# JunweiLiang/Object_Detection_Tracking

Hardware: AMD Instinct MI355X
Metric: detector FPS @1920x1080 b=8 per MI355X (higher is better)
Workload: dtype f32

## Files before the change

### include/odt.h

```cpp
#ifndef ODT_H_
#define ODT_H_

#include <stddef.h>
#include <stdint.h>

#ifdef __cplusplus
extern "C" {
#endif

typedef struct odt_model* odt_handle;

#define ODT_DTYPE_U8 0
#define ODT_DTYPE_F32 1

#define ODT_GRAPH_SINGLE 0
#define ODT_GRAPH_MULTI 1
#define ODT_GRAPH_EFFNET 2

typedef struct odt_config {
  int32_t graph;
  int32_t batch;
  int32_t height, width;
  int32_t num_class;
  int32_t num_blocks[4];
// ... 56 lines not shown
int odt_set_source_size(odt_handle h, int src_height, int src_width);

int odt_forward_serial(odt_handle h, int64_t* serial);

typedef struct odt_rle_result {
  int32_t n;
  int32_t height, width;
  const char* strings;
  const int64_t* offsets;
  const int32_t* lengths;
  const uint32_t* counts;
  const int64_t* count_offsets;
} odt_rle_result;
int odt_mask_rle(odt_handle h, int64_t serial, int height, int width, double scale, int want_counts, odt_rle_result* out);

#define ODT_WANT_FEATS  1
#define ODT_WANT_POOLED 2
#define ODT_WANT_MASKS  4
#define ODT_WANT_ALL    7
int odt_submit(odt_handle h, const void* frames, int dtype, int* ticket);
int odt_submit_ex(odt_handle h, const void* frames, int dtype, int want, int* ticket);
int odt_collect(odt_handle h, int ticket, odt_outputs* out);
int odt_ingest_buffer(odt_handle h, int dtype, void** buffer, size_t* bytes);

int odt_describe(odt_handle h, char* buf, int cap);

int odt_tap(odt_handle h, const char* name, float* dst, size_t cap_elems,
            int64_t* shape_out, int* rank_out);

int odt_range_health(odt_handle h, int rebase, double* worst_growth, char* tensor, int tensor_cap, double* tensor_amax,
                     long long* tensors_seen);

int odt_profile_enable(odt_handle h, int enable);
int odt_profile_read(odt_handle h, double* conv_ms, double* conv_flops,
                     int* conv_launches, double* total_ms);
int odt_profile_layer(odt_handle h, int index, char* name, int name_cap,
                      double* flops, double* ms, int64_t* mnk, int* count);

int odt_probe_mfma_bf16(int device, double warm_ms, double min_ms, int lds_reads, double* tflops_bf16,
                        double* clock_ghz, double* measured_ms, int* launches);

int odt_nn_cosine(int device, const float* gallery, const int32_t* seg_offsets,
                  int T, const float* dets, int N, int D, double* cost);

typedef struct odt_tracker* odt_tracker_handle;
int odt_tracker_create(double max_cosine_distance, int nn_budget, double max_iou_distance,
                       int max_age, int n_init, int device, odt_tracker_handle* out);
int odt_tracker_destroy(odt_tracker_handle t);
int odt_tracker_predict(odt_tracker_handle t);
int odt_tracker_update(odt_tracker_handle t, const double* tlwh, const double* conf,
                       const float* feats, int N, int D);
int odt_tracker_tracks(odt_tracker_handle t, int cap, int32_t* ids, int32_t* state,
                       int32_t* time_since_update, int32_t* hits, int32_t* age, double* mean,
                       double* covariance, int* n);
int odt_lsap(const double* cost, int nr, int nc, int32_t* rows, int32_t* cols, int* n);
int odt_tracker_nms(const double* boxes_xywh, const double* scores, const int32_t* order, int n, double max_overlap, int32_t* pick,
                    int* npick);

typedef struct odt_tmot* odt_tmot_handle;
int odt_tmot_create(double conf_thres, double track_max_second_lost, double emb_max_dist, double iou_max_dist1,
                    double iou_max_dist2, double emb_smooth_alpha, double frame_gap, double frame_rate,
                    odt_tmot_handle* out);
int odt_tmot_destroy(odt_tmot_handle t);
int odt_tmot_reset(odt_tmot_handle t);
int odt_tmot_update(odt_tmot_handle t, const double* tlwh, const double* conf, const float* feats, int n, int dim,
                    int* id_counter, int* n_out);
int odt_tmot_tracks(odt_tmot_handle t, int which, int cap, int32_t* ids, int32_t* state, int32_t* activated,
                    double* tlwh, double* det_tlwh, double* det_conf, double* score, int32_t* tracklet_len,
                    int32_t* start_frame, int32_t* frame_id, int* n);


int odt_op_conv2d(int device, const float* in, int B, int H, int W, int Cin,
                  const float* wt, const float* bias, int kh, int kw, int Cout,
                  int stride, int dil, int pad_t, int pad_l, int Ho, int Wo,
                  int oy, int ox, const float* res, int res_mode, int relu,
                  float* out);

int odt_op_conv2d_cat(int device, const float* a, int B, int Ho, int Wo, int Ca, const float* b2, int Hb,
                      int Wb, int Cb, int stride_b, const float* wa, const float* wb, const float* bias,
                      int Cout, int relu, float* out);
int odt_op_bottleneck_tail(int device, const float* in, int B, int H, int W, int C, const float* w2,
                           const float* b2, int dil, const float* w3, const float* b3, int C3,
                           const float* res, int relu3, int fuse, float* out);
int odt_op_stem(int device, const float* frame_pad, int B, int Hp, int Wp, const float* w_hwio, const float* bias,
                int fuse, int grid, float* out);
#define ODT_CONV_CHOICE_SHAPE 18
#define ODT_CONV_CHOICE_OUT 11
int odt_op_conv_choice(const int* shape, int conv_arith, int conv_split_family, int* out, char* name, int name_cap);
int odt_op_preprocess(int device, const void* frames, int dtype, int B, int H,
                      int W, int pad_t, int pad_l, int Hp, int Wp, float* out);
int odt_op_maxpool(int device, const float* in, int B, int H, int W, int C,
                   float* out);
int odt_op_topk(int device, const float* scores, int n, int k, int32_t* idx_out);
int odt_op_nms(int device, const float* boxes, const float* scores, int n,
               int max_out, float iou_thresh, int32_t* idx_out, int* n_out);
int odt_op_proposals(int device, int graph, int B, int L, const int* hs,
                     const int* ws, const int* fields, const float* const* rpn,
                     const float* const* anchors, int img_h, int img_w, int K,
                     float nms_thresh, float decode_clip, float* props,
                     int32_t* nprops);
int odt_op_roi_align(int device, int B, int C, const int* hs, const int* ws,
                     const float* const* feats, const float* strides,
                     const float* boxes, const int32_t* box_ind, int R,
                     float* out_nchw, float* pooled);
int odt_op_detections(int device, int graph, int B, int K, int C,
                      const float* cls_logits, const float* box_logits,
                      const float* props, const int32_t* nprops, int img_h,
                      int img_w, const float* reg_weights, float decode_clip,
                      float score_thresh, float nms_thresh, int per_im,
                      float* boxes, float* probs, int32_t* labels,
                      int32_t* valid);

int odt_op_class_nms(int device, int graph, int B, int N, int C, const float* boxes_in,
                     const float* scores_in, const int32_t* ncand, float score_thresh,
                     float nms_thresh, int per_im, float* boxes, float* scores,
                     int32_t* labels, int32_t* valid);


int odt_op_dwconv(int device, const float* in, int B, int H, int W, int ldc, const float* wt, const float* bias, int k,
                  int stride, int pad_t, int pad_l, int Ho, int Wo, int act, int nmaps, const int32_t* map_hw, int se,
                  int mid, const float* w1, const float* b1, const float* w2t, const float* b2, float* out, float* mean,
                  float* gate, int32_t* info);
int odt_op_se_gate(int device, const float* x, int B, int HW, int ldc, int mid, int se, const float* w1, const float* b1,
                   const float* w2t, const float* b2, float* mean, float* gate, float* scaled, int32_t* info);
int odt_op_rse_gate(int device, const float* t2, int B, int HW, int ch, int r, int cout, const float* w1, const float* b1,
                    const float* w2t, const float* b2, float* mean, float* gate);
int odt_op_rse_apply(int device, const float* y, const float* gate, const float* shortcut, int B, int HW, int C, int ldc,
                     int in_place, float* out, float* amax);
int odt_op_se_tail(int device, const float* t2, int B, int H, int W, int ch, const float* w3, const float* b3, const float* w1,
                   const float* b1, const float* w2t, const float* b2, const float* shortcut, float* out, float* gate,
                   float* amax);
int odt_op_bifpn_fuse(int device, int n, const float* const* ins, const int32_t* in_hw, const int32_t* mode,
                      const int32_t* pads, const float* wsm, int act, int B, int h, int w, int ldc, float* out);
int odt_op_mbconv_expand_dw(int device, const float* x, int B, int H, int W, int in_ldc, const float* e_wt,
                            const float* e_bias, int mid, int lmid, const float* dw_wt, const float* dw_bias, int k,
                            int stride, int pad_t, int pad_l, int Ho, int Wo, int se, const float* w1, const float* b1,
                            const float* w2t, const float* b2, float* out, float* mean, float* gate, int32_t* info);
int odt_op_effdet_post(int device, int B, int ncls, const int32_t* npix, int ldc_cls, int ldc_box,
                       const float* const* cls, const float* const* box, const float* anchors, int k, int max_out,
                       float score_thresh, float iou_thresh, float image_scale, int32_t* cand_idx, float* cand_boxes,
                       float* cand_scores, int32_t* cand_cls, int32_t* cand_lvl, float* boxes, float* scores,
                       int32_t* labels, int32_t* levels, int32_t* valid);
int odt_op_preprocess_rgb(int device, const void* frames, int dtype, int B, int Hs, int Ws, int Hr, int Wr, int pad_t,
                          int pad_l, int Hp, int Wp, int resize, float* out);

int odt_op_mask_rle(int device, const float* masks, const float* boxes, int n, int on_device, int height, int width,
                    double scale, int want_counts, odt_rle_result* out);

#ifdef __cplusplus
}
#endif
#endif
```

### object_detection_tracking_amd/_lib.py

```python
from __future__ import annotations

import copy
import ctypes as C
import json
import os

import numpy as np

HERE = os.path.dirname(os.path.abspath(__file__))
LIB_HIP_PATH = os.path.join(HERE, "libodt_hip.so")

c_float_p = C.POINTER(C.c_float)
c_int_p = C.POINTER(C.c_int32)
c_i64_p = C.POINTER(C.c_int64)
c_double_p = C.POINTER(C.c_double)

ODT_DTYPE_U8, ODT_DTYPE_F32 = 0, 1
ODT_ARITH_DEFAULT, ODT_ARITH_F32, ODT_ARITH_BF16X3 = 0, 1, 2
ODT_GRAPH_SINGLE, ODT_GRAPH_MULTI, ODT_GRAPH_EFFNET = 0, 1, 2
RPN_CH = 16


class OdtConfig(C.Structure):
  _fields_ = [
      ("graph", C.c_int32), ("batch", C.c_int32), ("height", C.c_int32),
      ("width", C.c_int32), ("num_class", C.c_int32),
      ("num_blocks", C.c_int32 * 4), ("use_dilations", C.c_int32),
      ("fpn_channels", C.c_int32), ("head_dim", C.c_int32),
      ("rpn_topk", C.c_int32), ("result_per_im", C.c_int32),
      ("anchor_field", C.c_int32), ("rpn_nms_thresh", C.c_float),
      ("rpn_decode_clip", C.c_float), ("head_decode_clip", C.c_float),
      ("bbox_reg_weights", C.c_float * 4), ("result_score_thresh", C.c_float),
      ("head_nms_thresh", C.c_float), ("add_mask", C.c_int32), ("mask_dim", C.c_int32),
      ("eff_backbone", C.c_int32), ("eff_det", C.c_int32), ("eff_topk", C.c_int32),
      ("eff_image_scale", C.c_float), ("conv_arith", C.c_int32), ("conv_split_family", C.c_int32),
      ("keep_taps", C.c_int32),
      ("tail_overlap", C.c_int32),
      ("use_se", C.c_int32),
  ]


class OdtOutputs(C.Structure):
  _fields_ = [("boxes", c_float_p), ("probs", c_float_p), ("labels", c_int_p),
              ("valid", c_int_p), ("feats", c_float_p), ("pooled", c_float_p),
              ("masks", c_float_p)]


class OdtRleResult(C.Structure):
  _fields_ = [("n", C.c_int32), ("height", C.c_int32), ("width", C.c_int32), ("strings", C.c_void_p),
              ("offsets", c_i64_p), ("lengths", c_int_p), ("counts", C.POINTER(C.c_uint32)), ("count_offsets", c_i64_p)]

  def rles(self):
    size = [int(self.height), int(self.width)]
    out = []
    for j in range(int(self.n)):
      s = C.string_at(self.strings + int(self.offsets[j]), int(self.lengths[j])) if self.lengths[j] else b""
      out.append({"size": list(size), "counts": s.decode("ascii")})
    return out

  def count_lists(self):
    if not self.counts:
      return None
    total = int(self.count_offsets[int(self.n)])
    flat = np.ctypeslib.as_array(self.counts, shape=(total,)).copy() if total else np.zeros(0, np.uint32)
    return [flat[int(self.count_offsets[j]):int(self.count_offsets[j + 1])] for j in range(int(self.n))]


def fptr(a):
  return a.ctypes.data_as(c_float_p)


def iptr(a):
  return a.ctypes.data_as(c_int_p)


def f32(a):
  return np.ascontiguousarray(a, dtype=np.float32)


def i32(a):
  return np.ascontiguousarray(a, dtype=np.int32)


class OdtError(RuntimeError):
  pass


class OdtLib(object):

  SYMBOLS = [
      "odt_last_error", "odt_device_count", "odt_create", "odt_destroy",
      "odt_load_tensor", "odt_finalize_weights", "odt_forward",
      "odt_forward_async", "odt_synchronize", "odt_read_outputs", "odt_describe", "odt_range_health", "odt_submit", "odt_submit_ex", "odt_collect",
      "odt_ingest_buffer", "odt_set_source_size", "odt_tap", "odt_profile_enable",
      "odt_profile_read", "odt_profile_layer", "odt_probe_mfma_bf16", "odt_nn_cosine", "odt_op_conv2d", "odt_op_conv2d_cat",
      "odt_op_bottleneck_tail", "odt_op_stem", "odt_op_conv_choice", "odt_op_preprocess",
      "odt_op_maxpool", "odt_op_topk", "odt_op_nms", "odt_op_proposals",
      "odt_op_roi_align", "odt_op_detections", "odt_op_class_nms",
      "odt_op_dwconv", "odt_op_se_gate", "odt_op_rse_gate", "odt_op_rse_apply", "odt_op_se_tail", "odt_op_bifpn_fuse", "odt_op_mbconv_expand_dw", "odt_op_effdet_post",
      "odt_op_preprocess_rgb", "odt_forward_serial", "odt_mask_rle", "odt_op_mask_rle", "odt_tracker_create", "odt_tracker_destroy",
      "odt_tracker_predict", "odt_tracker_update", "odt_tracker_tracks", "odt_lsap", "odt_tracker_nms",
      "odt_tmot_create", "odt_tmot_destroy", "odt_tmot_reset", "odt_tmot_update", "odt_tmot_tracks",
  ]

  def __init__(self, path):
    if not os.path.exists(path):
      raise OdtError("native library not found: %s (build it with "
                     "`python -m object_detection_tracking_amd.build`)" % path)
    self.path = path
    self.dll = C.CDLL(path)
    d = self.dll
    for s in self.SYMBOLS:
      if not hasattr(d, s):
        raise OdtError("%s does not export %s" % (path, s))
    d.odt_last_error.restype = C.c_char_p
    d.odt_create.argtypes = [C.POINTER(OdtConfig), C.c_int, C.POINTER(C.c_void_p)]
    d.odt_destroy.argtypes = [C.c_void_p]
    d.odt_load_tensor.argtypes = [C.c_void_p, C.c_char_p, c_float_p, c_i64_p, C.c_int]
    d.odt_finalize_weights.argtypes = [C.c_void_p]
    d.odt_forward.argtypes = [C.c_void_p, C.c_void_p, C.c_int, C.c_int, C.c_void_p,
                              C.POINTER(OdtOutputs)]
    d.odt_forward_async.argtypes = [C.c_void_p, C.c_void_p, C.c_int, C.c_int, C.c_void_p]
    d.odt_synchronize.argtypes = [C.c_void_p]
    d.odt_read_outputs.argtypes = [C.c_void_p, C.POINTER(OdtOutputs)]
    d.odt_submit.argtypes = [C.c_void_p, C.c_void_p, C.c_int, C.POINTER(C.c_int)]
    d.odt_describe.argtypes = [C.c_void_p, C.c_char_p, C.c_int]
    d.odt_range_health.argtypes = [C.c_void_p, C.c_int, C.POINTER(C.c_double), C.c_char_p, C.c_int, C.POINTER(C.c_double), C.POINTER(C.c_longlong)]
    d.odt_submit_ex.argtypes = [C.c_void_p, C.c_void_p, C.c_int, C.c_int, C.POINTER(C.c_int)]
    d.odt_collect.argtypes = [C.c_void_p, C.c_int, C.POINTER(OdtOutputs)]
    d.odt_set_source_size.argtypes = [C.c_void_p, C.c_int, C.c_int]
    d.odt_ingest_buffer.argtypes = [C.c_void_p, C.c_int, C.POINTER(C.c_void_p),
                                    C.POINTER(C.c_size_t)]
    d.odt_tap.argtypes = [C.c_void_p, C.c_char_p, c_float_p, C.c_size_t, c_i64_p,
                          C.POINTER(C.c_int)]
    d.odt_profile_enable.argtypes = [C.c_void_p, C.c_int]
    d.odt_profile_read.argtypes = [C.c_void_p, c_double_p, c_double_p,
                                   C.POINTER(C.c_int), c_double_p]
    d.odt_profile_layer.argtypes = [C.c_void_p, C.c_int, C.c_char_p, C.c_int, c_double_p,
                                    c_double_p, c_i64_p, C.POINTER(C.c_int)]
    d.odt_probe_mfma_bf16.argtypes = [C.c_int, C.c_double, C.c_double, C.c_int, c_double_p, c_double_p, c_double_p,
                                      C.POINTER(C.c_int)]
    d.odt_nn_cosine.argtypes = [C.c_int, c_float_p, c_int_p, C.c_int, c_float_p, C.c_int,
                                C.c_int, c_double_p]
    d.odt_op_conv2d.argtypes = [C.c_int, c_float_p] + [C.c_int] * 4 + [c_float_p, c_float_p] + \
        [C.c_int] * 11 + [c_float_p, C.c_int, C.c_int, c_float_p]
    d.odt_op_conv2d_cat.argtypes = [C.c_int, c_float_p] + [C.c_int] * 4 + [c_float_p] + [C.c_int] * 4 + \
        [c_float_p, c_float_p, c_float_p, C.c_int, C.c_int, c_float_p]
    d.odt_op_bottleneck_tail.argtypes = [C.c_int, c_float_p] + [C.c_int] * 4 + [c_float_p, c_float_p, C.c_int, c_float_p, c_float_p,
                                         C.c_int, c_float_p, C.c_int, C.c_int, c_float_p]
    d.odt_op_stem.argtypes = [C.c_int, c_float_p] + [C.c_int] * 3 + [c_float_p, c_float_p, C.c_int, C.c_int, c_float_p]
    d.odt_op_conv_choice.argtypes = [c_int_p, C.c_int, C.c_int, c_int_p, C.c_char_p, C.c_int]
    d.odt_op_preprocess.argtypes = [C.c_int, C.c_void_p] + [C.c_int] * 8 + [c_float_p]
    d.odt_op_maxpool.argtypes = [C.c_int, c_float_p] + [C.c_int] * 4 + [c_float_p]
    d.odt_op_topk.argtypes = [C.c_int, c_float_p, C.c_int, C.c_int, c_int_p]
    d.odt_op_nms.argtypes = [C.c_int, c_float_p, c_float_p, C.c_int, C.c_int, C.c_float,
                             c_int_p, C.POINTER(C.c_int)]
    d.odt_op_proposals.argtypes = [C.c_int, C.c_int, C.c_int, C.c_int, c_int_p, c_int_p, c_int_p,
                                   C.POINTER(c_float_p), C.POINTER(c_float_p), C.c_int, C.c_int,
                                   C.c_int, C.c_float, C.c_float, c_float_p, c_int_p]
    d.odt_op_roi_align.argtypes = [C.c_int, C.c_int, C.c_int, c_int_p, c_int_p,
                                   C.POINTER(c_float_p), c_float_p, c_float_p, c_int_p, C.c_int,
                                   c_float_p, c_float_p]
    d.odt_tracker_create.argtypes = [C.c_double, C.c_int, C.c_double, C.c_int, C.c_int, C.c_int,
                                     C.POINTER(C.c_void_p)]
    d.odt_tracker_destroy.argtypes = [C.c_void_p]
    d.odt_tracker_predict.argtypes = [C.c_void_p]
    d.odt_tracker_update.argtypes = [C.c_void_p, c_double_p, c_double_p, c_float_p, C.c_int, C.c_int]
    d.odt_tracker_tracks.argtypes = [C.c_void_p, C.c_int, c_int_p, c_int_p, c_int_p, c_int_p, c_int_p,
                                     c_double_p, c_double_p, C.POINTER(C.c_int)]
    d.odt_lsap.argtypes = [c_double_p, C.c_int, C.c_int, c_int_p, c_int_p, C.POINTER(C.c_int)]
    d.odt_tracker_nms.argtypes = [c_double_p, c_double_p, c_int_p, C.c_int, C.c_double, c_int_p, C.POINTER(C.c_int)]
    d.odt_tmot_create.argtypes = [C.c_double] * 8 + [C.POINTER(C.c_void_p)]
    d.odt_tmot_destroy.argtypes = [C.c_void_p]
    d.odt_tmot_reset.argtypes = [C.c_void_p]
    d.odt_tmot_update.argtypes = [C.c_void_p, c_double_p, c_double_p, c_float_p, C.c_int, C.c_int,
                                  C.POINTER(C.c_int), C.POINTER(C.c_int)]
    d.odt_tmot_tracks.argtypes = [C.c_void_p, C.c_int, C.c_int, c_int_p, c_int_p, c_int_p, c_double_p,
                                  c_double_p, c_double_p, c_double_p, c_int_p, c_int_p, c_int_p,
                                  C.POINTER(C.c_int)]
    d.odt_op_detections.argtypes = [C.c_int] * 5 + [c_float_p, c_float_p, c_float_p, c_int_p,
                                                    C.c_int, C.c_int, c_float_p, C.c_float,
                                                    C.c_float, C.c_float, C.c_int, c_float_p,
                                                    c_float_p, c_int_p, c_int_p]
    d.odt_op_class_nms.argtypes = [C.c_int] * 5 + [c_float_p, c_float_p, c_int_p, C.c_float, C.c_float, C.c_int,
                                                   c_float_p, c_float_p, c_int_p, c_int_p]

    d.odt_op_dwconv.argtypes = [C.c_int, c_float_p] + [C.c_int] * 4 + [c_float_p, c_float_p] + [C.c_int] * 8 + \
        [c_int_p, C.c_int, C.c_int] + [c_float_p] * 7 + [c_int_p]
    d.odt_op_se_gate.argtypes = [C.c_int, c_float_p] + [C.c_int] * 5 + [c_float_p] * 7 + [c_int_p]
    d.odt_op_rse_gate.argtypes = [C.c_int, c_float_p] + [C.c_int] * 5 + [c_float_p] * 6
    d.odt_op_rse_apply.argtypes = [C.c_int, c_float_p, c_float_p, c_float_p] + [C.c_int] * 5 + [c_float_p, c_float_p]
    d.odt_op_se_tail.argtypes = [C.c_int, c_float_p] + [C.c_int] * 4 + [c_float_p] * 10
    d.odt_op_bifpn_fuse.argtypes = [C.c_int, C.c_int, C.POINTER(c_float_p), c_int_p, c_int_p, c_int_p, c_float_p] + \
        [C.c_int] * 5 + [c_float_p]
    d.odt_op_mbconv_expand_dw.argtypes = [C.c_int, c_float_p] + [C.c_int] * 4 + [c_float_p] * 2 + [C.c_int] * 2 + \
        [c_float_p] * 2 + [C.c_int] * 7 + [c_float_p] * 7 + [c_int_p]
    d.odt_op_effdet_post.argtypes = [C.c_int] * 3 + [c_int_p, C.c_int, C.c_int, C.POINTER(c_float_p), C.POINTER(c_float_p),
                                     c_float_p, C.c_int, C.c_int, C.c_float, C.c_float, C.c_float, c_int_p, c_float_p,
                                     c_float_p, c_int_p, c_int_p, c_float_p, c_float_p, c_int_p, c_int_p, c_int_p]
    d.odt_op_preprocess_rgb.argtypes = [C.c_int, C.c_void_p] + [C.c_int] * 11 + [c_float_p]
    d.odt_forward_serial.argtypes = [C.c_void_p, c_i64_p]
    d.odt_mask_rle.argtypes = [C.c_void_p, C.c_int64, C.c_int, C.c_int, C.c_double, C.c_int, C.POINTER(OdtRleResult)]
    d.odt_op_mask_rle.argtypes = [C.c_int, C.c_void_p, C.c_void_p, C.c_int, C.c_int, C.c_int, C.c_int, C.c_double, C.c_int,
                                  C.POINTER(OdtRleResult)]

  def check(self, rc):
    if rc != 0:
      msg = self.dll.odt_last_error()
      raise OdtError(msg.decode("utf-8", "replace") if msg else "odt error %d" % rc)

  def device_count(self):
    n = C.c_int(0)
    self.check(self.dll.odt_device_count(C.byref(n)))
    return n.value


_LIB = None


def get_lib():
  global _LIB
  if _LIB is None:
    lib = OdtLib(LIB_HIP_PATH)
    if lib.device_count() < 1:
      raise OdtError("libodt_hip.so loaded but no HIP device is visible")
    _LIB = lib
  return _LIB


def as_frames(frames):
  fr = np.ascontiguousarray(frames)
  if fr.dtype == np.uint8:
# ... 94 lines not shown
```

### object_detection_tracking_amd/csrc/conv_h2.hip

```cpp
#include "conv_split_epilogue.hpp"

namespace odt {

namespace {

#define ODT_MFMA_F16(a, b, c) __builtin_amdgcn_mfma_f32_32x32x16_f16(a, b, c, 0, 0, 0)

template <int TN, int WM, int WN = 2>
struct H2Cfg {
  static constexpr int BM = 64 * WM, BN = 32 * TN * WN;
  static constexpr int NWV = WN * WM, NTHR = 64 * NWV;
  static constexpr int AKG = BM * 16 + 32, APL = 4 * AKG, ASTG = 2 * APL;
  static constexpr int BKG = BN * 16, BPL = 4 * BKG, STAGE_B = 2 * BPL;
  static constexpr int BOFF = 2 * ASTG;
  static constexpr int RING = BOFF + 2 * STAGE_B;
  static constexpr int CTILE = (BM < 128 ? BM : 128) * (BN + 4) * 4;
  static constexpr int LDS = RING > CTILE ? RING : CTILE;
  static constexpr int NW = STAGE_B / 1024 / NWV;
  static constexpr int RA = BM * 8 / NTHR;
  static_assert(LDS <= 160 * 1024 && STAGE_B % (1024 * NWV) == 0, "LDS ring");
};

template <int TN, int WM, bool TRACE = false, int WN = 2>
__global__ void __launch_bounds__(64 * WN * WM, 2) conv_h2_kernel(const ConvParams* __restrict__ pp) {
// ... 231 lines not shown
      }
      ODT_FENCE();
      ODT_MF(kst, 0, 0, j, bsel); ODT_FENCE();
    }
    { const int t = a_cur; a_cur = a_nxt; a_nxt = t; }
    { const int t = b_cur; b_cur = b_nxt; b_nxt = t; }
  };
  {
    int c = 0;
    for (; c + 2 < nsteps; ++c) step(std::true_type{}, std::true_type{});
    if (c + 1 < nsteps) { step(std::true_type{}, std::false_type{}); ++c; }
    step(std::false_type{}, std::false_type{});
  }
  stamp(2);
  split3_epilogue<WM, WN, TN, G::LDS, TRACE, G::NTHR>(p, acc, lds, m0, n0, M, HoWo, ks, splitk, tid, wm, wn, fr, fg, h2_inv);
  stamp(5);
}

#undef ODT_MF
#undef ODT_FENCE

__global__ void __launch_bounds__(256) h2_rowscale_kernel(const float* __restrict__ wt, int Cout, int K, float* __restrict__ chinv) {
  __shared__ float red[4];
  const int n = (int)blockIdx.x;
  float m = 0.f;
  if (n < Cout)
    for (int k = (int)threadIdx.x; k < K; k += 256) m = fmaxf(m, fabsf(wt[(size_t)n * K + k]));
#pragma unroll
  for (int d = 32; d >= 1; d >>= 1) m = fmaxf(m, __shfl_xor(m, d));
  if ((threadIdx.x & 63) == 0) red[threadIdx.x >> 6] = m;
  __syncthreads();
  if (threadIdx.x == 0) {
    m = fmaxf(fmaxf(red[0], red[1]), fmaxf(red[2], red[3]));
    chinv[n] = pow2f(-h2_scale_exp(__float_as_uint(m)));
  }
}

__global__ void split_weights_h2_kernel(const float* __restrict__ wt, int Cout, int K, int SBN, int ntaps, int Cin,
                                        unsigned short* __restrict__ img, const float* __restrict__ chinv) {
  const int nst = K >> 5, nst1 = ntaps * (Cin >> 5);
  const long idx = (long)blockIdx.x * blockDim.x + threadIdx.x;
  const long total = (long)cout_padded(Cout) * nst * 4;
  if (idx >= total) return;
  const int n = (int)(idx / (nst * 4)), rem = (int)(idx - (long)n * (nst * 4)), st = rem >> 2, kg = rem & 3;
  int k0;
  if (st < nst1) { const int cs = st / ntaps, tap = st - cs * ntaps; k0 = tap * Cin + cs * 32; }
  else k0 = ntaps * Cin + (st - nst1) * 32;
  k0 += kg * 8;
  const int tn = n / SBN, nn = n - tn * SBN;
  const float s = 1.0f / chinv[n];
  for (int e = 0; e < 8; e += 2) {
    unsigned piece[2];
    const float w0 = n < Cout ? wt[(size_t)n * K + k0 + e] : 0.f, w1 = n < Cout ? wt[(size_t)n * K + k0 + e + 1] : 0.f;
    split2h(w0, w1, s, piece[0], piece[1]);
    for (int q = 0; q < 2; ++q) {
      const size_t at = ((((size_t)(tn * nst + st) * 2 + q) * 4 + kg) * SBN + nn) * 8 + e;
      img[at] = (unsigned short)(piece[q] & 0xffffu);
      img[at + 1] = (unsigned short)(piece[q] >> 16);
    }
  }
}

__global__ void split_weights_h2f_kernel(const float* __restrict__ wt, int Cout, int K, unsigned short* __restrict__ img,
                                         const float* __restrict__ chinv) {
  const int KH = K >> 1, NS = KH >> 4;
  const long idx = (long)blockIdx.x * blockDim.x + threadIdx.x;
  const long total = (long)Cout * 2 * NS * 2;
  if (idx >= total) return;
  const int fg = (int)(idx & 1), s = (int)((idx >> 1) % NS), wn = (int)((idx / (2 * NS)) & 1), n = (int)(idx / (4 * NS));
  const int c = n >> 5, fr = n & 31;
  const float sc = 1.0f / chinv[n];
  for (int e = 0; e < 8; e += 2) {
    const int k0 = wn * KH + (s >> 1) * 32 + (s & 1) * 16 + (e & 3) + 8 * (e >> 2) + 4 * fg;
    unsigned piece[2];
    split2h(wt[(size_t)n * K + k0], wt[(size_t)n * K + k0 + 1], sc, piece[0], piece[1]);
    for (int q = 0; q < 2; ++q) {
      const size_t at = ((((((size_t)c * 2 + q) * 2 + wn) * NS + s) * 2 + fg) * 32 + fr) * 8 + e;
      img[at] = (unsigned short)(piece[q] & 0xffffu);
      img[at + 1] = (unsigned short)(piece[q] >> 16);
    }
  }
}

__global__ void __launch_bounds__(256) tensor_amax_kernel(const float* __restrict__ x, size_t n, unsigned* __restrict__ slot) {
  float m = 0.f;
  for (size_t i = (size_t)blockIdx.x * 256 + threadIdx.x; i < n; i += (size_t)gridDim.x * 256) m = fmaxf(m, fabsf(x[i]));
  publish_amax(slot, m, (int)threadIdx.x);
}

}

size_t conv_h2_weight_bytes(int Cout, int K) { return (size_t)cout_padded(Cout) * K * 4 + (size_t)cout_padded(Cout) * 4; }

const float* conv_h2_chinv(const void* img, int Cout, int K) {
  return reinterpret_cast<const float*>(reinterpret_cast<const char*>(img) + (size_t)cout_padded(Cout) * K * 4);
}

int conv_make_h2_weights(const ConvParams& p, void* img_dev, hipStream_t stream) {
  const int K = p.kh * p.kw * p.Cin + (p.in2 != nullptr ? p.Cin2 : 0);
  const int bn = conv_variant_row(p.variant).bn;
  ODT_CHECK((bn == 256 || bn == 128 || bn == 64) && p.Cin % 32 == 0 && (p.in2 == nullptr || p.Cin2 % 32 == 0) && cout_padded(p.Cout) % bn == 0,
            "conv_make_h2_weights: 256- / 128- / 64-wide n-tiles and 32-channel slices required");
  float* chinv = const_cast<float*>(conv_h2_chinv(img_dev, p.Cout, K));
  hipLaunchKernelGGL(h2_rowscale_kernel, dim3((unsigned)cout_padded(p.Cout)), dim3(256), 0, stream, p.wt, p.Cout, K, chinv);
  const long total = (long)cout_padded(p.Cout) * (K >> 5) * 4;
  hipLaunchKernelGGL(split_weights_h2_kernel, dim3((unsigned)((total + 255) / 256)), dim3(256), 0, stream, p.wt, p.Cout, K,
                     bn, p.kh * p.kw, p.Cin, (unsigned short*)img_dev, chinv);
  ODT_HIP(hipGetLastError());
  return 0;
}

size_t conv_h2f_weight_bytes(int Cout, int K) { return (size_t)Cout * K * 4 + (size_t)Cout * 4; }
const float* conv_h2f_chinv(const void* img, int Cout, int K) {
  return reinterpret_cast<const float*>(reinterpret_cast<const char*>(img) + (size_t)Cout * K * 4);
}
int conv_make_h2f_weights(const float* wt, int Cout, int K, void* img_dev, hipStream_t stream) {
  ODT_CHECK((K == 256 || K == 128 || K == 64) && Cout % 32 == 0 && Cout > 0, "conv_make_h2f_weights: K = 64 / 128 / 256 and Cout % 32 == 0 required");
  float* chinv = const_cast<float*>(conv_h2f_chinv(img_dev, Cout, K));
  hipLaunchKernelGGL(h2_rowscale_kernel, dim3((unsigned)Cout), dim3(256), 0, stream, wt, Cout, K, chinv);
  const long total = (long)Cout * (K >> 3);
  hipLaunchKernelGGL(split_weights_h2f_kernel, dim3((unsigned)((total + 255) / 256)), dim3(256), 0, stream, wt, Cout, K,
                     (unsigned short*)img_dev, chinv);
  ODT_HIP(hipGetLastError());
  return 0;
}

bool conv_h2f_fusable(const ConvParams& a, const ConvParams& b) {
  const ConvKernelRow& fa = conv_variant_row(conv_variant_fused_tail(a.variant));
  const bool a_ok = a.wt_split != nullptr && fa.launch != nullptr && fa.bn == a.Cout && a.splitk <= 1 && a.head_wt == nullptr &&
                    a.res_mode == 0 && a.in2 == nullptr && a.relu <= 1 && a.nlvl <= 1 && a.out_oy == 0 && a.out_ox == 0 &&
                    a.out_H == a.Ho && a.out_W == a.Wo && a.f_wt == nullptr;
  const bool b_ok = b.in == a.out && b.kh == 1 && b.kw == 1 && b.stride == 1 && b.pad_t == 0 && b.pad_l == 0 && b.Cin == a.Cout &&
                    b.in_ldc == a.out_ldc && b.in2 == nullptr && b.B == a.B && b.H == a.Ho && b.W == a.Wo && b.Ho == a.Ho &&
                    b.Wo == a.Wo && b.in_Ha == a.out_H && b.in_Wa == a.out_W && b.Cout % 32 == 0 && b.out_oy == 0 && b.out_ox == 0 &&
                    b.out_H == b.Ho && b.out_W == b.Wo && b.out_ldc % 4 == 0 && b.out_ldc >= b.Cout &&
                    (b.res_mode == 0 || (b.res_mode == 1 && b.res_H == b.Ho && b.res_W == b.Wo && b.res_ldc % 4 == 0)) &&
                    b.relu <= 1 && b.nlvl <= 1 && b.head_wt == nullptr && b.splitk <= 1 && b.wt_split != nullptr && conv_variant_row(b.variant).family == CF_H2 &&
                    b.f_wt == nullptr && (double)b.B * b.Ho * b.Wo * b.out_ldc * 4.0 < 2147483648.0;
  return a_ok && b_ok;
}

int launch_tensor_amax(const float* x, size_t n, unsigned* slot, hipStream_t stream) {
  const unsigned blocks = (unsigned)std::min<size_t>((n + 255) / 256, 2048);
  hipLaunchKernelGGL(tensor_amax_kernel, dim3(blocks ? blocks : 1), dim3(256), 0, stream, x, n, slot);
  ODT_HIP(hipGetLastError());
  return 0;
}

void conv_rows_h2(ConvKernelRow* t) {
  ODT_CONV_ROW(t, H2_64x64, CF_H2, 64, 64, 128, 0, (conv_h2_kernel<1, 1, false>));
  ODT_CONV_ROW(t, H2_64x128, CF_H2, 64, 128, 128, 0, (conv_h2_kernel<2, 1, false>));
  ODT_CONV_ROW(t, H2_512x64, CF_H2, 512, 64, 512, 0, (conv_h2_kernel<2, 8, false, 1>));
  ODT_CONV_ROW(t, H2_128x64, CF_H2, 128, 64, 256, 0, (conv_h2_kernel<1, 2, false>));
  ODT_CONV_ROW_T(t, H2_256x256, CF_H2, 256, 256, 512, 0, (conv_h2_kernel<4, 4, false>), (conv_h2_kernel<4, 4, true>));
  ODT_CONV_ROW(t, H2_256x128, CF_H2, 256, 128, 512, 0, (conv_h2_kernel<2, 4, false>));
  ODT_CONV_ROW_T(t, H2_128x128, CF_H2, 128, 128, 256, 0, (conv_h2_kernel<2, 2, false>), (conv_h2_kernel<2, 2, true>));
}

}
```

### object_detection_tracking_amd/csrc/conv_h2k.hip

```cpp
#include "conv_split_epilogue.hpp"

namespace odt {

namespace {

#define ODT_MFMA_F16(a, b, c) __builtin_amdgcn_mfma_f32_32x32x16_f16(a, b, c, 0, 0, 0)
#define ODT_MF(kst, qa, qb, j, bsel) { if constexpr (FUSE) {                                                   \
                                          acc[0][j] = ODT_MFMA_F16(fb[bsel][qb], fa[kst][qa][0], acc[0][j]);   \
                                          acc[1][j] = ODT_MFMA_F16(fb[bsel][qb], fa[kst][qa][1], acc[1][j]);   \
                                        } else {                                                                \
                                          acc[0][j] = ODT_MFMA_F16(fa[kst][qa][0], fb[bsel][qb], acc[0][j]);   \
                                          acc[1][j] = ODT_MFMA_F16(fa[kst][qa][1], fb[bsel][qb], acc[1][j]); } }
#define ODT_FENCE() __builtin_amdgcn_sched_barrier(0)

template <int TN, bool FUSE = false, int WN = 2>
struct H2kCfg {
  static constexpr int WM = 8 / WN;
  static constexpr int BM = 64 * WM, BN = 32 * TN * WN;
  static constexpr int PR = BM + 16;
  static constexpr int ZR = PR - 1;
  static constexpr int AKG = PR * 16 + 32, APL = 4 * AKG, ABUF = 2 * APL;
  static constexpr int BKG = BN * 16, BPL = 4 * BKG, STAGE_B = 2 * BPL;
  static constexpr int BOFF = 2 * ABUF;
  static constexpr int RING = BOFF + 2 * STAGE_B;
  static constexpr int CTILE = 128 * (BN + 4) * 4;
  static constexpr int F_WCH = 2 * 2 * (2 * TN) * 1024, F_CS = 36, F_COFF = 2 * F_WCH, F_CEND = F_COFF + 2 * 256 * F_CS * 4;
  static constexpr int LDS0 = RING > CTILE ? RING : CTILE;
  static constexpr int F_KOFF = F_CEND > LDS0 ? F_CEND : LDS0;
  static constexpr int F_K3OFF = F_KOFF + 2048;
  static constexpr int LDS = FUSE ? F_K3OFF + 8192 : LDS0;
  static constexpr int NW = STAGE_B / 1024 / 8;
  static constexpr int RA = (PR + 63) / 64;
  static_assert(LDS <= 160 * 1024 && STAGE_B % 8192 == 0 && (!FUSE || WN == 2), "LDS");
};

template <int TN, bool TRACE>
__device__ __forceinline__ void h2f_tail(const ConvParams& p, f32x16 (&acc)[2][TN], unsigned char* lds, int m0, int M,
                                         int wave, int wm, int wn, float h2_inv) {
  using G = H2kCfg<TN, true>;
  constexpr int NS = 2 * TN, WCH = G::F_WCH, CS = G::F_CS, COFF = G::F_COFF, CBUF = 256 * CS * 4;
  ODT_FENCE();
  const int lane = ODT_LANE_ID();
  const int tid = wave * 64 + lane, fr = lane & 31, fg = lane >> 5;
  const int nch = p.f_cout >> 5;

  const float* kc = reinterpret_cast<const float*>(lds + G::F_KOFF);
  const float act2_lo = p.relu == 1 ? 0.f : -__builtin_huge_valf();
  float mx[2] = {0.f, 0.f};
#pragma unroll
  for (int j = 0; j < TN; ++j)
#pragma unroll
    for (int g = 0; g < 4; ++g) {
      const int col = wn * 32 * TN + j * 32 + 8 * g + 4 * fg;
      const f32x4 sc = *reinterpret_cast<const f32x4*>(kc + col), bs = *reinterpret_cast<const f32x4*>(kc + 256 + col);
#pragma unroll
      for (int i = 0; i < 2; ++i)
#pragma unroll
        for (int e = 0; e < 4; ++e) {
          float v = acc[i][j][4 * g + e] * sc[e];
          v += bs[e];
          mx[i] = fmaxf(mx[i], fabsf(fmaxf(v, act2_lo)));
        }
      if (g & 1) ODT_FENCE();
    }
  ODT_PIN2(mx[0], mx[1]);
  asm volatile("" ::: "memory");
  constexpr int XS = 8 * 2 * NS * 1024;
  float* xs = reinterpret_cast<float*>(lds + XS);
#pragma unroll
  for (int i = 0; i < 2; ++i) {
    mx[i] = fmaxf(mx[i], __shfl_xor(mx[i], 32));
    xs[wave * 128 + i * 64 + lane] = mx[i];
  }
  ODT_BARRIER_LDS();
  float ys[2], yinv[2];
#pragma unroll
  for (int i = 0; i < 2; ++i) {
    const float m = fmaxf(mx[i], xs[(wave ^ 1) * 128 + i * 64 + lane]);
    const int be = (int)((__float_as_uint(m) >> 23) & 0xffu);
    int e = 14 - (be - 127);
    e = e > 100 ? 100 : (e < -100 ? -100 : e);
    e = (be == 0) | (be == 255) ? 0 : e;
    ys[i] = pow2f(e); yinv[i] = pow2f(-e);
  }
  ODT_PIN2(ys[0], ys[1]);
  u32x4 yq[2][2][NS];
#pragma unroll
  for (int j = 0; j < TN; ++j)
#pragma unroll
    for (int h = 0; h < 2; ++h) {
      const int col = wn * 32 * TN + j * 32 + 16 * h + 4 * fg;
      const f32x4 sc0 = *reinterpret_cast<const f32x4*>(kc + col), bs0 = *reinterpret_cast<const f32x4*>(kc + 256 + col);
      const f32x4 sc1 = *reinterpret_cast<const f32x4*>(kc + col + 8), bs1 = *reinterpret_cast<const f32x4*>(kc + 256 + col + 8);
#pragma unroll
      for (int i = 0; i < 2; ++i) {
        float v[8];
#pragma unroll
        for (int e = 0; e < 4; ++e) {
          float t0 = acc[i][j][8 * h + e] * sc0[e], t1 = acc[i][j][8 * h + 4 + e] * sc1[e];
          t0 += bs0[e]; t1 += bs1[e];
          v[e] = fmaxf(t0, act2_lo); v[4 + e] = fmaxf(t1, act2_lo);
        }
        u32x4 hq, lq;
#pragma unroll
        for (int t = 0; t < 4; ++t) {
          unsigned a, b;
          split2h(v[2 * t], v[2 * t + 1], ys[i], a, b);
          hq[t] = a; lq[t] = b;
        }
        ODT_PIN2(hq, lq);
        yq[i][0][2 * j + h] = hq; yq[i][1][2 * j + h] = lq;
      }
      ODT_FENCE();
    }
  ODT_STAMP(3);

  constexpr int XW = 2 * NS * 1024;
  static_assert(XS == 8 * XW && XS + 8 * 512 <= G::F_KOFF, "exchange area");
  u32x4 yo[2][NS], yr[2][NS];
  const float yinv_k = wn == 0 ? yinv[0] : yinv[1];
  {
    unsigned char* xw = lds + wave * XW + lane * 16;
    const unsigned char* xr = lds + (wave ^ 1) * XW + lane * 16;
    auto give = [&](auto IC) {
      constexpr int ig = decltype(IC)::value;
#pragma unroll
      for (int q = 0; q < 2; ++q)
#pragma unroll
        for (int t = 0; t < NS; ++t) {
          *reinterpret_cast<u32x4*>(xw + (q * NS + t) * 1024) = yq[ig][q][t];
          yo[q][t] = yq[1 - ig][q][t];
        }
    };
    if (wn == 0) give(std::integral_constant<int, 1>{}); else give(std::integral_constant<int, 0>{});
    ODT_BARRIER_LDS();
#pragma unroll
    for (int q = 0; q < 2; ++q)
#pragma unroll
      for (int t = 0; t < NS; ++t) yr[q][t] = *reinterpret_cast<const u32x4*>(xr + (q * NS + t) * 1024);
    ODT_BARRIER_LDS();
  }
  const __amdgpu_buffer_rsrc_t rs_w = __builtin_amdgcn_make_buffer_rsrc((void*)p.f_wt, 0, (int)((unsigned)nch * (unsigned)WCH), 0x00020000);
  const int rot = (p.debug & 0x100) == 0 ? (m0 / G::BM) % nch : 0;
  auto ce = [&](int c) { return c < nch ? (c + rot >= nch ? c + rot - nch : c + rot) : c; };
  auto dma_w = [&](int cs, int buf) {
    const int c = ce(cs);
#pragma unroll
    for (int i = 0; i < WCH / 8192; ++i)
      __builtin_amdgcn_raw_ptr_buffer_load_lds(rs_w, ODT_LDS_PTR(lds + buf * WCH + (i * 8 + wave) * 1024), 16,
                                               c < nch ? lane * 16 + (i * 8 + wave) * 1024 : (int)kOOB, c < nch ? c * WCH : 0, 0, 0);
  };
  dma_w(0, 0);
  dma_w(1, 1);

  const unsigned mrows = (unsigned)M;
  const __amdgpu_buffer_rsrc_t rs_res = __builtin_amdgcn_make_buffer_rsrc(
      (void*)(p.f_res != nullptr ? p.f_res : p.f_bias), 0, (int)(p.f_res != nullptr ? mrows * (unsigned)p.f_res_ldc * 4u : 0u), 0x00020000);
  const __amdgpu_buffer_rsrc_t rs_out = __builtin_amdgcn_make_buffer_rsrc((void*)p.f_out, 0, (int)(mrows * (unsigned)p.f_out_ldc * 4u), 0x00020000);
  const int c4 = tid & 7, row0 = tid >> 3;
  const unsigned m_first = (unsigned)(m0 + row0);
  const unsigned roff0 = (m_first * (unsigned)p.f_res_ldc + c4 * 4u) * 4u, rstep = 64u * (unsigned)p.f_res_ldc * 4u;
  const unsigned ooff0 = (m_first * (unsigned)p.f_out_ldc + c4 * 4u) * 4u, ostep = 64u * (unsigned)p.f_out_ldc * 4u;
  const bool has_res = p.f_res != nullptr;
  const float act_lo = p.f_relu == 1 ? 0.f : -__builtin_huge_valf();
  const float* k3 = reinterpret_cast<const float*>(lds + G::F_K3OFF);
  auto fetch_res = [&](int cs, int s2) -> f32x4 {
    const int c = ce(cs);
    const unsigned off = has_res && c < nch && m_first + 64u * s2 < mrows ? roff0 + s2 * rstep : kOOB;
    return (f32x4)__builtin_amdgcn_raw_buffer_load_b128(rs_res, (int)off, c * 128, 2);
  };
  f32x4 ra[4], rb[4];
#pragma unroll
  for (int s2 = 0; s2 < 4; ++s2) ra[s2] = fetch_res(0, s2);
#pragma unroll
  for (int s2 = 0; s2 < 4; ++s2) rb[s2] = fetch_res(1, s2);
  const unsigned char* wrd = lds + lane * 16;
  float* Cst = reinterpret_cast<float*>(lds + COFF);
  const int cw_at = (wm * 64 + wn * 32 + fr) * CS + 4 * fg;
  const int cr_at = row0 * CS + c4 * 4;
  float vmax = 0.f;
  auto row_item = [&](int cs, int s2, f32x4& rr) {
    const int c = ce(cs);
    const float* Cb = Cst + (cs & 1) * (CBUF / 4);
    f32x4 v = *reinterpret_cast<const f32x4*>(Cb + cr_at + 64 * s2 * CS);
    const f32x4 sc3 = *reinterpret_cast<const f32x4*>(k3 + c * 32 + c4 * 4), b3 = *reinterpret_cast<const f32x4*>(k3 + 1024 + c * 32 + c4 * 4);
    v = v * sc3;
    v += b3;
    v += rr;
#pragma unroll
    for (int e = 0; e < 4; ++e) v[e] = fmaxf(v[e], act_lo);
    const float vm = fmaxf(fmaxf(fabsf(v[0]), fabsf(v[1])), fmaxf(fabsf(v[2]), fabsf(v[3])));
    const bool ok = m_first + 64u * s2 < mrows;
    vmax = fmaxf(vmax, ok ? vm : 0.f);
    __builtin_amdgcn_raw_buffer_store_b128((u32x4)v, rs_out, (int)(ok ? ooff0 + s2 * ostep : kOOB), c * 128, 0);
    rr = fetch_res(cs + 2, s2);
  };
  ODT_WAIT_VM_LGKM0(8);
  __builtin_amdgcn_s_barrier();
  auto chunk = [&](int c, f32x4 (&rprev)[4], auto HP) {
    constexpr bool has_prev = decltype(HP)::value;
    const int buf = c & 1;
    const unsigned char* wo = wrd + buf * WCH + wn * NS * 1024;
    const unsigned char* wr = wrd + buf * WCH + (1 - wn) * NS * 1024;
    f32x16 co;
#pragma unroll
    for (int r = 0; r < 16; ++r) co[r] = 0.f;
    f16x8 wf[2][2];
    wf[0][0] = *reinterpret_cast<const f16x8*>(wo);
    wf[0][1] = *reinterpret_cast<const f16x8*>(wo + 2 * NS * 1024);
#pragma unroll
    for (int u = 0; u < 2 * NS; ++u) {
      if (u + 1 < 2 * NS) {
        const unsigned char* w = ((u + 1) & 1 ? wr : wo) + ((u + 1) >> 1) * 1024;
        wf[(u + 1) & 1][0] = *reinterpret_cast<const f16x8*>(w);
        wf[(u + 1) & 1][1] = *reinterpret_cast<const f16x8*>(w + 2 * NS * 1024);
      }
      f16x8 yhh, yll;
      if (u & 1) { __builtin_memcpy(&yhh, &yr[0][u >> 1], 16); __builtin_memcpy(&yll, &yr[1][u >> 1], 16); }
      else { __builtin_memcpy(&yhh, &yo[0][u >> 1], 16); __builtin_memcpy(&yll, &yo[1][u >> 1], 16); }
      ODT_FENCE();
      co = ODT_MFMA_F16(wf[u & 1][1], yhh, co);
      co = ODT_MFMA_F16(wf[u & 1][0], yll, co);
      co = ODT_MFMA_F16(wf[u & 1][0], yhh, co);
      ODT_FENCE();
      if constexpr (has_prev) {
        if constexpr (NS >= 4) { if ((u & 1) && u < 8) row_item(c - 1, u >> 1, rprev[u >> 1]); }
        else row_item(c - 1, u, rprev[u]);
      }
    }
    float* Cb = Cst + buf * (CBUF / 4) + cw_at;
#pragma unroll
    for (int g = 0; g < 4; ++g) {
      f32x4 a = {co[4 * g], co[4 * g + 1], co[4 * g + 2], co[4 * g + 3]};
      a = a * yinv_k;
      *reinterpret_cast<f32x4*>(Cb + 8 * g) = a;
    }
    if constexpr (has_prev) ODT_WAIT_VM_LGKM0(8); else ODT_WAIT_VM_LGKM0(0);
    __builtin_amdgcn_s_barrier();
    ODT_FENCE();
    dma_w(c + 2, buf);
    ODT_FENCE();
  };
  chunk(0, ra, std::false_type{});
  int c = 1;
#pragma unroll 1
  for (; c + 1 < nch; c += 2) {
    chunk(c, ra, std::true_type{});
    chunk(c + 1, rb, std::true_type{});
  }
  if (c < nch) {
    chunk(c, ra, std::true_type{});
#pragma unroll
    for (int s2 = 0; s2 < 4; ++s2) row_item(c, s2, rb[s2]);
  } else {
#pragma unroll
    for (int s2 = 0; s2 < 4; ++s2) row_item(c - 1, s2, ra[s2]);
  }
  publish_amax_wg<512>(p.f_out_amax, vmax, tid, lds);
}

template <int TN, bool TRACE = false, bool FUSE = false, int WN = 2>
__global__ void __launch_bounds__(512, 2) conv_h2k_kernel(const ConvParams* __restrict__ pp) {
  using G = H2kCfg<TN, FUSE, WN>;
  constexpr int WM = G::WM, KW = 3;
  constexpr int BM = G::BM, BN = G::BN, AKG = G::AKG, APL = G::APL, ABUF = G::ABUF, BKG = G::BKG, BPL = G::BPL;
  constexpr int STAGE_B = G::STAGE_B, BOFF = G::BOFF, NW = G::NW, ZR = G::ZR, RA = G::RA;
  const ConvParams p = *pp;
  __shared__ __attribute__((aligned(16))) unsigned char lds[G::LDS];

  const int tid = threadIdx.x, lane = tid & 63;
  const int wave = __builtin_amdgcn_readfirstlane(tid >> 6);
  const int wm = wave / WN, wn = wave % WN;
  auto stamp = [&](int i) {
    if constexpr (TRACE) {
      if (tid == 0) p.trace[(size_t)blockIdx.x * 16 + i] = wall_clock64();
    }
  };
  stamp(0);
  if constexpr (TRACE) {
    if (tid == 0) {
      p.trace[(size_t)blockIdx.x * 16 + 8] = __builtin_amdgcn_s_getreg((31 << 11) | 4);
      p.trace[(size_t)blockIdx.x * 16 + 9] = __builtin_amdgcn_s_getreg((31 << 11) | 20);
    }
  }
  const int ntn = cout_padded(p.Cout) / BN;
  int wg = (int)blockIdx.x;
  {
    const int nwg = (int)gridDim.x, xcd = wg & 7, q = nwg >> 3, r = nwg & 7;
    wg = (xcd < r ? xcd * (q + 1) : r * (q + 1) + (xcd - r) * q) + (wg >> 3);
  }
  const int splitk = p.splitk > 1 ? p.splitk : 1;
  const int ks = wg % splitk;
  wg /= splitk;
  const int mt = wg / ntn, nt = wg - mt * ntn;
  const int m0 = mt * BM, n0 = nt * BN;
  const int HoWo = p.Ho * p.Wo;
  const int M = p.B * HoWo;
  const int cpt = p.Cin >> 5;
  const int nsteps = p.kh * KW * cpt, ngroups_all = p.kh * cpt;
  const int g_begin = (int)(((long)ngroups_all * ks) / splitk);
  const int ngroups = (int)(((long)ngroups_all * (ks + 1)) / splitk) - g_begin;
  const int halo = (KW - 1) * p.dil;
  const int sexp = h2_in_scale_exp(p);
  const float a_scale = pow2f(sexp), h2_inv = pow2f(-sexp);

  const __amdgpu_buffer_rsrc_t rs_in = __builtin_amdgcn_make_buffer_rsrc(
      (void*)p.in, 0, (int)((unsigned)p.B * p.in_Ha * p.in_Wa * p.in_ldc * 4u), 0x00020000);
  const __amdgpu_buffer_rsrc_t rs_wt = __builtin_amdgcn_make_buffer_rsrc(
      (void*)p.wt_split, 0, (int)((unsigned)ntn * nsteps * (unsigned)STAGE_B), 0x00020000);

  unsigned l_b = ((unsigned)nt * (unsigned)nsteps + (unsigned)(g_begin * KW)) * (unsigned)STAGE_B;
  auto dma_b = [&](int boff) {
#pragma unroll
    for (int i = 0; i < NW; ++i)
      __builtin_amdgcn_raw_ptr_buffer_load_lds(rs_wt, ODT_LDS_PTR(lds + boff + (i * 8 + wave) * 1024), 16,
                                               lane * 16 + (i * 8 + wave) * 1024, (int)l_b, 0, 0);
    l_b += (unsigned)STAGE_B;
  };
  dma_b(BOFF);

  const int pix_bytes = p.in_ldc * 4;
  const int n_first = sfast_div(m0, p.div_howo_mul, p.div_howo_sh), r_img = m0 - n_first * HoWo;
  const int len0 = HoWo - r_img < BM ? HoWo - r_img : BM;
  const int pix0 = (n_first * p.in_Ha - p.pad_t) * p.in_Wa + r_img - p.pad_l;
  const int pix1 = ((n_first + 1) * p.in_Ha - p.pad_t) * p.in_Wa - p.pad_l;
  const int a_c = tid & 7, a_r = tid >> 3;
  int a_base[RA];
#pragma unroll
  for (int j = 0; j < RA; ++j) {
    const int pr = a_r + 64 * j;
    const int pix = pr < len0 + halo ? pix0 + pr : pix1 + (pr - len0 - halo);
    a_base[j] = pr < BM + 2 * halo ? pix * pix_bytes + a_c * 16 : (int)kOOB;
  }
  int l_cs = g_begin / p.kh, l_kh = g_begin - (g_begin / p.kh) * p.kh;
  f32x4 ga[RA];
  auto load_group = [&]() {
    const int khoff = l_kh * p.dil * p.in_Wa * pix_bytes;
#pragma unroll
    for (int j = 0; j < RA; ++j) {
      const unsigned v = (unsigned)a_base[j] == kOOB ? kOOB : (unsigned)(a_base[j] + khoff);
      ga[j] = (f32x4)__builtin_amdgcn_raw_buffer_load_b128(rs_in, (int)v, l_cs * 128, 0);
    }
    if (++l_kh == p.kh) { l_kh = 0; ++l_cs; }
  };
  auto store_slot = [&](int abuf, int j) {
    const int pr = a_r + 64 * j;
    if (pr < BM + 2 * halo) {
      unsigned h0, l0, h1, l1;
      split2h(ga[j][0], ga[j][1], a_scale, h0, l0);
      split2h(ga[j][2], ga[j][3], a_scale, h1, l1);
      unsigned char* d = lds + abuf + (a_c >> 1) * AKG + pr * 16 + (a_c & 1) * 8;
// ... 80 lines not shown
    for (int t = 0; t < 2; ++t) fa[kst][q][t] = *reinterpret_cast<const f16x8*>(lds + q * APL + kst * 2 * AKG + fa_addr[t]);
  };
  auto rdA_n = [&](int q) {
#pragma unroll
    for (int t = 0; t < 2; ++t) fa[0][q][t] = *reinterpret_cast<const f16x8*>(lds + q * APL + fa_addr_n[t]);
  };
  auto rdB = [&](int bbuf, int kst, int j, int dst) {
#pragma unroll
    for (int q = 0; q < 2; ++q) fb[dst][q] = *reinterpret_cast<const f16x8*>(lds + bbuf + q * BPL + kst * 2 * BKG + b_rd + j * 512);
  };
  int a_cur = 0, a_nxt = ABUF;
  int b_cur = BOFF, b_nxt = BOFF + STAGE_B;
  tap_addr(a_cur, c_kh, 0);
  rdA(0, 1); rdA(0, 0);
  rdB(b_cur, 0, 0, 0);

  auto step = [&](auto KWIC, auto NEXT, auto PRE, auto GNC) {
    constexpr int KWI = decltype(KWIC)::value;
    constexpr bool next = decltype(NEXT)::value, pre = decltype(PRE)::value, gn = decltype(GNC)::value;
    constexpr int NG = 2 * TN;
    ODT_FENCE();
#pragma unroll
    for (int g = 0; g < NG; ++g) {
      const int kst = g / TN, j = g % TN, bsel = g & 1;
      const bool last = g == NG - 1;
      if (last) {
        if constexpr (KWI == 0 && gn) ODT_WAIT_VM_LGKM0(RA); else ODT_WAIT_VM_LGKM0(0);
        __builtin_amdgcn_s_barrier();
        ODT_FENCE();
        if constexpr (pre) dma_b(b_cur);
        if constexpr (next) {
          if constexpr (KWI + 1 < KW) tap_addr_n(a_cur, c_kh, KWI + 1);
          else tap_addr_n(a_nxt, c_kh + 1 == p.kh ? 0 : c_kh + 1, 0);
          rdB(b_nxt, 0, 0, bsel ^ 1);
        }
      } else {
        rdB(b_cur, (g + 1) / TN, (g + 1) % TN, bsel ^ 1);
        if (TN == 1) { rdA(1, 1); rdA(1, 0); }
      }
      ODT_FENCE();
      ODT_MF(kst, 1, 0, j, bsel); ODT_FENCE();
      if (last) {
        if constexpr (next) rdA_n(1);
      } else {
        if constexpr (gn && KWI == 2) {
          if (TN > 1) {
            constexpr int SPG = (RA + NG - 2) / (NG - 1);
#pragma unroll
            for (int q = 0; q < SPG; ++q)
              if (g * SPG + q < RA) store_slot(a_nxt, g * SPG + q);
          } else { store_slot(a_nxt, 0); store_slot(a_nxt, 1); store_slot(a_nxt, 2); }
        }
        if constexpr (gn && KWI == 0) { if (g == (TN == 1 ? 0 : 1)) load_group(); }
      }
      ODT_FENCE();
      ODT_MF(kst, 0, 1, j, bsel); ODT_FENCE();
      if (last) {
        if constexpr (next) rdA_n(0);
      } else {
        if (TN > 1 && g == TN - 2) rdA(1, 1);
        if (TN > 1 && g == TN - 1) rdA(1, 0);
        if constexpr (gn && KWI == 2) { if (TN == 1) { store_slot(a_nxt, 3); store_slot(a_nxt, 4); } }
      }
      ODT_FENCE();
      ODT_MF(kst, 0, 0, j, bsel); ODT_FENCE();
    }
    fa_addr[0] = fa_addr_n[0]; fa_addr[1] = fa_addr_n[1];
    { const int t = b_cur; b_cur = b_nxt; b_nxt = t; }
    if constexpr (KWI == KW - 1) {
      const int u = a_cur; a_cur = a_nxt; a_nxt = u;
      if (++c_kh == p.kh) c_kh = 0;
    }
  };
  {
    using T = std::true_type; using F = std::false_type;
    using K0 = std::integral_constant<int, 0>; using K1 = std::integral_constant<int, 1>; using K2 = std::integral_constant<int, 2>;
    for (int g = 0; g + 1 < ngroups; ++g) { step(K0{}, T{}, T{}, T{}); step(K1{}, T{}, T{}, T{}); step(K2{}, T{}, T{}, T{}); }
    step(K0{}, T{}, T{}, F{});
    step(K1{}, T{}, F{}, F{});
    step(K2{}, F{}, F{}, F{});
  }
#undef ODT_MF
  stamp(2);
  if constexpr (FUSE) h2f_tail<TN, TRACE>(p, acc, lds, m0, M, wave, wm, wn, h2_inv);
  else split3_epilogue<WM, WN, TN, G::LDS, TRACE>(p, acc, lds, m0, n0, M, HoWo, ks, splitk, tid, wm, wn, fr, fg, h2_inv);
  stamp(5);
}
#undef ODT_FENCE

}

void conv_rows_h2k(ConvKernelRow* t) {
  ODT_CONV_ROW(t, H2KF_256x64, CF_H2, 256, 64, 512, CVF_KWR | CVF_FTAIL, (conv_h2k_kernel<1, false, true>));
  ODT_CONV_ROW(t, H2KF_256x128, CF_H2, 256, 128, 512, CVF_KWR | CVF_FTAIL, (conv_h2k_kernel<2, false, true>));
  ODT_CONV_ROW_T(t, H2KF_256x256, CF_H2, 256, 256, 512, CVF_KWR | CVF_FTAIL, (conv_h2k_kernel<4, false, true>), (conv_h2k_kernel<4, true, true>));
  ODT_CONV_ROW_T(t, H2K_256x256, CF_H2, 256, 256, 512, CVF_KWR, (conv_h2k_kernel<4, false>), (conv_h2k_kernel<4, true>));
  ODT_CONV_ROW(t, H2K_256x128, CF_H2, 256, 128, 512, CVF_KWR, (conv_h2k_kernel<2, false>));
  ODT_CONV_ROW(t, H2K_512x64, CF_H2, 512, 64, 512, CVF_KWR, (conv_h2k_kernel<2, false, false, 1>));
  ODT_CONV_ROW(t, H2K_256x64, CF_H2, 256, 64, 512, CVF_KWR, (conv_h2k_kernel<1, false>));
}

}
```

### object_detection_tracking_amd/csrc/conv_igemm.hip

```cpp
#include <cstdlib>
#include <type_traits>

#include "odt_common.hpp"

namespace odt {

namespace {

constexpr int LS = 36;

typedef unsigned int u32x4 __attribute__((vector_size(16)));

__device__ __forceinline__ int fast_div(int n, unsigned mul, unsigned sh) {
  return mul ? (int)(__umulhi((unsigned)n, mul) >> sh) : n;
}
constexpr unsigned kOOB = 0x80000000u;

template <int WM, int WN, int TM, int TN, int ST, bool FINE>
__global__ void __launch_bounds__(256, ST == 1 ? 3 : 2) conv_igemm_kernel(const ConvParams* __restrict__ pp) {
  const ConvParams p = *pp;
  constexpr int BM = WM * TM * 32, BN = WN * TN * 32;
  constexpr int RA = BM / 32, RB = BN / 32;
  static_assert(WM * WN == 4, "4 waves");
  __shared__ __attribute__((aligned(16))) float lds[ST][(BM + BN) * LS];
// ... 428 lines not shown
        if (pass == 0) stamp(4);
      }
    };
    if (p.relu == 1) run(std::integral_constant<int, 1>{});
    else if (p.relu == 2) run(std::integral_constant<int, 2>{});
    else if (p.relu == 3) run(std::integral_constant<int, 3>{});
    else run(std::integral_constant<int, 0>{});
  } else {
    for (int pass = 0; pass < PASSES; ++pass) {
      stage_pass(pass);
      for (int s2 = 0; s2 < NCH; ++s2) {
        const int rl = row0 + s2 * (256 / C4);
        const int m = m0 + pass * RP + rl;
        int nv = p.Cout - col;
        nv = nv > 4 ? 4 : nv;
        if (m >= M || nv <= 0) continue;
        size_t opix, rpix = 0;
        if (dense_io) {
          opix = (size_t)m;
          rpix = (size_t)m;
        } else {
          const int n = fast_div(m, p.div_howo_mul, p.div_howo_sh), rr = m - n * HoWo;
          const int ho = fast_div(rr, p.div_wo_mul, p.div_wo_sh), wo = rr - ho * p.Wo;
          opix = ((size_t)n * p.out_H + ho + p.out_oy) * p.out_W + wo + p.out_ox;
          if (p.res_mode != 0)
            rpix = p.res_mode == 1 ? ((size_t)n * p.res_H + ho) * p.res_W + wo
                                   : ((size_t)n * p.res_H + (ho >> 1)) * p.res_W + (wo >> 1);
        }
        f32x4 v = *reinterpret_cast<const f32x4*>(&Ct[rl * CS + c4 * 4]);
        v += bias4;
        if (p.res_mode != 0) {
          const float* rp = p.res + rpix * p.res_ldc + col;
          for (int e = 0; e < nv; ++e) v[e] += rp[e];
        }
#pragma unroll
        for (int e = 0; e < 4; ++e) {
          if (p.relu == 1) v[e] = fmaxf(v[e], 0.f);
          else if (p.relu == 2) v[e] = v[e] * (1.0f / (1.0f + expf(-v[e])));
          else if (p.relu == 3) v[e] = 1.0f / (1.0f + expf(-v[e]));
        }
        float* op = p.out + opix * p.out_ldc + col;
        for (int e = 0; e < nv; ++e) op[e] = v[e];
      }
    }
  }
  stamp(5);
}

}

void conv_rows_f32(ConvKernelRow* t) {
  ODT_CONV_ROW(t, F32_128x64_S1_FINE, CF_F32, 128, 64, 256, CVF_FINE, (conv_igemm_kernel<4, 1, 1, 2, 1, true>));
  ODT_CONV_ROW(t, F32_128x64_S1, CF_F32, 128, 64, 256, 0, (conv_igemm_kernel<4, 1, 1, 2, 1, false>));
  ODT_CONV_ROW(t, F32_64x64_S1_FINE, CF_F32, 64, 64, 256, CVF_FINE, (conv_igemm_kernel<2, 2, 1, 1, 1, true>));
  ODT_CONV_ROW(t, F32_64x64_S1, CF_F32, 64, 64, 256, 0, (conv_igemm_kernel<2, 2, 1, 1, 1, false>));
  ODT_CONV_ROW(t, F32_128x128_S1_FINE, CF_F32, 128, 128, 256, CVF_FINE, (conv_igemm_kernel<2, 2, 2, 2, 1, true>));
  ODT_CONV_ROW(t, F32_128x128_S1, CF_F32, 128, 128, 256, 0, (conv_igemm_kernel<2, 2, 2, 2, 1, false>));
  ODT_CONV_ROW(t, F32_128x64_S2_FINE, CF_F32, 128, 64, 256, CVF_ST2 | CVF_FINE, (conv_igemm_kernel<4, 1, 1, 2, 2, true>));
  ODT_CONV_ROW(t, F32_128x64_S2, CF_F32, 128, 64, 256, CVF_ST2, (conv_igemm_kernel<4, 1, 1, 2, 2, false>));
  ODT_CONV_ROW(t, F32_64x64_S2_FINE, CF_F32, 64, 64, 256, CVF_ST2 | CVF_FINE, (conv_igemm_kernel<2, 2, 1, 1, 2, true>));
  ODT_CONV_ROW(t, F32_64x64_S2, CF_F32, 64, 64, 256, CVF_ST2, (conv_igemm_kernel<2, 2, 1, 1, 2, false>));
  ODT_CONV_ROW(t, F32_128x128_S2_FINE, CF_F32, 128, 128, 256, CVF_ST2 | CVF_FINE, (conv_igemm_kernel<2, 2, 2, 2, 2, true>));
  ODT_CONV_ROW(t, F32_128x128_S2, CF_F32, 128, 128, 256, CVF_ST2, (conv_igemm_kernel<2, 2, 2, 2, 2, false>));
}

static void make_div(unsigned d, unsigned* mul, unsigned* sh) {
  if (d <= 1) { *mul = 0; *sh = 0; return; }
  unsigned l = 0;
  while ((1ull << l) < d) ++l;
  const unsigned pbits = 31 + l;
  *mul = (unsigned)(((1ull << pbits) + d - 1) / d);
  *sh = pbits - 32;
}

void conv_prepare(ConvParams& p) {
  make_div((unsigned)(p.Ho * p.Wo), &p.div_howo_mul, &p.div_howo_sh);
  make_div((unsigned)p.Wo, &p.div_wo_mul, &p.div_wo_sh);
}

double conv_flops(const ConvParams& p) {
  return 2.0 * (double)p.B * p.Ho * p.Wo * (double)p.Cout *
             (double)(p.kh * p.kw * p.Cin + (p.in2 != nullptr ? p.Cin2 : 0)) +
         (p.head_wt != nullptr ? 2.0 * (double)p.B * p.Ho * p.Wo * (double)p.Cout * 15.0 : 0.0) +
         (p.f_wt != nullptr ? 2.0 * (double)p.B * p.Ho * p.Wo * (double)p.Cout * (double)p.f_cout : 0.0);
}

int conv_check(const ConvParams& p) {
  ODT_CHECK(p.Cin % 32 == 0, "conv: Cin must be a multiple of 32");
  ODT_CHECK(p.in_ldc % 4 == 0, "conv: input pixel stride must be a multiple of 4 floats");
  ODT_CHECK(p.B > 0 && p.Ho > 0 && p.Wo > 0 && p.Cout > 0, "conv: empty problem");
  ODT_CHECK(p.in2 == nullptr || (p.kh == 1 && p.kw == 1 && p.Cin2 % 32 == 0 && p.in2_ldc % 4 == 0 &&
                                 (double)p.B * p.in2_Ha * p.in2_Wa * p.in2_ldc * 4.0 < 2147483648.0),
            "conv: a second A source needs a 1x1 conv, Cin2 % 32 == 0 and a tensor below 2 GiB");
  ODT_CHECK((long)p.Ho * p.stride + (long)p.kh * p.dil < 32000 && (long)p.Wo * p.stride + (long)p.kw * p.dil < 32000 &&
            p.pad_t < 32000 && p.pad_l < 32000, "conv: spatial extent must fit 16-bit tap coordinates");
  ODT_CHECK((double)p.B * p.in_Ha * p.in_Wa * p.in_ldc * 4.0 < 2147483648.0 &&
            (double)p.Cout * (p.kh * p.kw * p.Cin + p.Cin2) * 4.0 < 2147483648.0,
            "conv: operand tensors must be smaller than 2 GiB (32-bit buffer offsets)");
  ODT_CHECK((double)p.B * p.out_H * p.out_W * p.out_ldc * 4.0 < 2147483648.0 &&
            (p.res_mode == 0 || (double)p.B * p.res_H * p.res_W * p.res_ldc * 4.0 < 2147483648.0),
            "conv: output / residual tensors must be smaller than 2 GiB (32-bit buffer offsets)");
  return conv_check_variant(p);
}

}
```

### object_detection_tracking_amd/csrc/conv_split.hip

```cpp
#include <array>

#include "conv_split_common.hpp"

namespace odt {

namespace {

__global__ void split_weights_kernel(const float* __restrict__ wt, int Cout, int K, int SBN, int bk, unsigned short* __restrict__ img,
                                     const float* __restrict__ kscale) {
  const int nsl = K / bk, kgs = bk >> 3;
  const long idx = (long)blockIdx.x * blockDim.x + threadIdx.x;
  const long total = (long)cout_padded(Cout) * (K >> 3);
  if (idx >= total) return;
  const int n = (int)(idx / (K >> 3)), k8 = (int)(idx - (long)n * (K >> 3));
  const int tn = n / SBN, nn = n - tn * SBN, sl = k8 / kgs, kg = k8 - sl * kgs;
  for (int e = 0; e < 8; e += 2) {
    unsigned piece[3];
    float w0 = n < Cout ? wt[(size_t)n * K + k8 * 8 + e] : 0.f, w1 = n < Cout ? wt[(size_t)n * K + k8 * 8 + e + 1] : 0.f;
    if (kscale != nullptr) { w0 = w0 * kscale[k8 * 8 + e]; w1 = w1 * kscale[k8 * 8 + e + 1]; }
    split2(w0, w1, piece[0], piece[1], piece[2]);
    for (int q = 0; q < 3; ++q) {
      const size_t at = ((((size_t)(tn * nsl + sl) * 3 + q) * kgs + kg) * SBN + nn) * 8 + e;
      img[at] = (unsigned short)(piece[q] & 0xffffu);
      img[at + 1] = (unsigned short)(piece[q] >> 16);
// ... 243 lines not shown
      conv_tiles(p, 128, 64) < q.min_tiles) return false;
  return TILE(CF_H2, s.np == 64 && q.h2_n64_bm512 == 2 ? 512 : 128, 64, 0, 1);
}
bool rule_split1(const Sel& s, Tile& t) { return TILE(CF_SPLIT1, conv_split_bm(s.p.Cout), s.bn0, 0, 1); }
#undef TILE

const Rule kRules[] = {rule_exact_f32_outside_policy, rule_exact_f32_too_few_tiles, rule_h2_n64_forced,     rule_h2_256_rows,
                       rule_h2k_few_rows,             rule_h2_dense_few_rows,       rule_h2_64_rows,        rule_h2_128_rows,
                       rule_split3,                   rule_h2_n64_small_tiles,      rule_split1};

int select_exact_f32(const ConvParams& p, const Knobs& k) {
  const long M = (long)p.B * p.Ho * p.Wo;
  const long tiles128 = ((M + 127) / 128) * ((p.Cout + 127) / 128);
  int tile = (int)k.get_long(K_CONV_TILE, 0);
  const bool smallk = !k.off(K_CONV_SMALLK);
  const int Kfull = conv_k(p);
  if (tile == 0) tile = p.Cout <= 64 ? 1 : ((tiles128 < 384 || (smallk && Kfull <= 384)) ? 2 : 3);
  int stages = (tile == 3 && p.kh * p.kw == 1 && p.Cin >= 1024) ? 2 : 1;
  if (k.get(K_CONV_STAGES).i == 1 || k.get(K_CONV_STAGES).i == 2) stages = (int)k.get(K_CONV_STAGES).i;
  const int BMt = tile == 2 ? 64 : 128, BNt = tile == 3 ? 128 : 64;
  const long tiles = ((M + BMt - 1) / BMt) * ((p.Cout + BNt - 1) / BNt);
  const long slots = 256L * (stages == 2 ? 2 : (tile == 3 ? 3 : 4));
  bool fine = stages == 2 || (tile != 2 && (tiles <= slots || tile == 1 || (Kfull >= 1024 && tiles >= 2 * slots)));
  if (tile == 2) fine = tiles >= 384 && tiles <= slots;
  if (k.get(K_CONV_FINE).c0 == '0' || k.get(K_CONV_FINE).c0 == '1') fine = k.get(K_CONV_FINE).c0 == '1';
  return conv_variant_find(CF_F32, BMt, BNt, (stages == 2 ? CVF_ST2 : 0u) | (fine ? CVF_FINE : 0u));
}

}

ConvChoice conv_select(const ConvParams& p, const ConvPolicy& q, const Knobs& k) {
  Sel s{p, q, (long)p.B * p.Ho * p.Wo, conv_k(p), cout_padded(p.Cout), conv_split_bn(p.Cout), false, 0, 0, 1, false, false};
  split3_fit(s);
  s.kwr3 = s.fit && q.kw_reuse && s.b3 == 256 && s.k3 == 1 && (s.n3 >= 128 || q.kwr_n64) && conv_kwr_pays(p);
  s.h2 = s.fit && q.family == 2 && (s.n3 >= 128 || q.h2_n64) && conv_h2_sources_ok(p) && p.lvl_scale == nullptr && p.head_wt == nullptr;
  Tile t{CF_F32, 0, 0, 0, 0};
  for (const Rule rule : kRules)
    if (rule(s, t)) break;
  if (t.family == CF_F32) return ConvChoice{select_exact_f32(p, k), 0, 0};
  if (t.family == CF_H2 && t.bm == 64 && t.splitk == 1 && conv_h2d_fits(p) && !k.off(K_CONV_H2_BK64)) t.flags |= CVF_DSTAGE;
  const long capv = k.get_long(K_SPLIT_REDUCE_BLOCKS, 512L);
  return ConvChoice{conv_variant_find(t.family, t.bm, t.bn, t.flags), t.splitk, capv > 0 ? (int)capv : 512};
}

int conv_finish(ConvParams& p, const Knobs& k) {
  conv_prepare(p);
  if (k.get(K_CONV_DEBUG).i != 0) p.debug = (int)k.get(K_CONV_DEBUG).i;
  if (p.wt_split == nullptr) conv_use_variant(p, select_exact_f32(p, k), 0);
  return conv_check(p);
}

int conv_check_variant(const ConvParams& p) {
  const ConvKernelRow& r = conv_variant_row(p.variant);
  const bool split3 = p.wt_split != nullptr && r.family == CF_SPLIT3;
  ODT_CHECK(p.nlvl <= 1 || (split3 && p.splitk <= 1 && p.nlvl <= 5 && p.head_wt == nullptr),
            "conv: per-row-range epilogue constants need a conv_split3 kernel without split-K");
  if (p.wt_split == nullptr) {
    ODT_CHECK(p.variant == CV_NONE || r.family == CF_F32, "conv: a split-kernel row without a weight image");
    return 0;
  }
  ODT_CHECK(r.launch != nullptr && r.family != CF_F32, "conv: the record's variant names no split-kernel row of the table");
  ODT_CHECK(cout_padded(p.Cout) % r.bn == 0, "conv: the row's n-tile does not divide the padded channel count");
  const long M = (long)p.B * p.Ho * p.Wo;
  const int sk = p.splitk > 1 ? p.splitk : 1;
  const bool kwr = (r.flags & CVF_KWR) != 0;
  ODT_CHECK(sk == 1 || p.reduce_blocks > 0, "conv: split-K without a combine-pass grid");
  if (r.flags & CVF_STEM) {
    ODT_CHECK(conv_stem_fits(p) && p.out != nullptr && p.out_H == (p.Ho + 1 - 3) / 2 + 1 && p.out_W == (p.Wo + 1 - 3) / 2 + 1 &&
              p.out_oy == 0 && p.out_ox == 0, "conv stem: unsupported shape");
  } else if (r.family == CF_H2) {
    ODT_CHECK((r.bm != 512 || !kwr || p.Ho * p.Wo >= 512) && conv_h2_sources_ok(p) && p.h2_chinv != nullptr &&
              (!(r.flags & CVF_DSTAGE) || (sk == 1 && conv_h2d_fits(p))),
              "conv h2: unsupported tile / shape, or no recorded input range");
    ODT_CHECK(sk == 1 || (p.partial != nullptr && p.in2 == nullptr && p.head_wt == nullptr && (p.kh * p.kw * p.Cin >> 5) >= sk),
              "conv h2: split-K needs a partial buffer, a single source and at least one stage per range");
    ODT_CHECK((p.f_wt != nullptr) == ((r.flags & CVF_FTAIL) != 0), "conv h2: a fused 1x1 tail needs the kw-reuse kernel");
    if (kwr) {
      ODT_CHECK(conv_kwr_fits(p) && (sk == 1 || (r.bm == 256 && r.bn >= 128 && p.f_wt == nullptr && p.kh * (p.Cin >> 5) >= sk)), "conv h2k: unsupported shape");
      ODT_CHECK(p.f_wt == nullptr || (r.bn == p.Cout && p.head_wt == nullptr && p.res_mode == 0 && p.relu <= 1 && p.f_cout % 32 == 0 &&
                                      p.f_cout > 0 && p.f_cout <= 1024 && p.f_out != nullptr && p.f_chinv != nullptr && p.f_bias != nullptr && p.f_out_ldc % 4 == 0 &&
                                      (p.f_res == nullptr || p.f_res_ldc % 4 == 0) && (double)M * p.f_out_ldc * 4.0 < 2147483648.0 &&
                                      (p.f_res == nullptr || (double)M * p.f_res_ldc * 4.0 < 2147483648.0)),
                "conv h2k: unsupported fused 1x1 tail");
    }
  } else if (r.family == CF_SPLIT3) {
    ODT_CHECK(p.Cin % 16 == 0 && p.kh * p.kw <= 32, "conv split3: unsupported tile / shape");
    ODT_CHECK(sk == 1 || (p.partial != nullptr && p.in2 == nullptr && (p.kh * p.kw * p.Cin >> 4) >= sk),
              "conv split3: split-K needs a partial buffer, a single source and at least one stage per range");
    ODT_CHECK(!kwr || (sk == 1 && conv_kwr_fits(p)), "conv split3k: unsupported shape");
  } else {
    ODT_CHECK(sk == 1 && r.bm == conv_split_bm(p.Cout) && r.bn == conv_split_bn(p.Cout), "conv split1: the tile follows from the channel count");
  }
  return 0;
}

int launch_conv(const ConvParams& p, const ConvParams* dev, hipStream_t stream) {
  const ConvKernelRow& r = conv_variant_row(p.variant);
  ODT_CHECK(r.launch != nullptr, "conv: launch of a record without a kernel variant");
  const int sk = p.splitk > 1 ? p.splitk : 1;
  unsigned grid;
  if (r.flags & CVF_STEM) {
    if (conv_stem_grid(p, &grid)) return 1;
  } else {
    const long M = (long)p.B * p.Ho * p.Wo;
    const int ntiles = r.family == CF_F32 ? (p.Cout + r.bn - 1) / r.bn : cout_padded(p.Cout) / r.bn;
    grid = (unsigned)(((M + r.bm - 1) / r.bm) * ntiles * sk);
  }
  (p.trace != nullptr && r.launch_traced != nullptr ? r.launch_traced : r.launch)(dev, grid, stream);
  if (sk > 1) launch_split_reduce(p, dev, stream);
  ODT_HIP(hipGetLastError());
  return 0;
}

size_t conv_split_partial_bytes(const ConvParams& p) {
  const int fam = conv_variant_row(p.variant).family;
  return (fam == CF_SPLIT3 || fam == CF_H2) && p.splitk > 1 ? (size_t)p.splitk * p.B * p.Ho * p.Wo * cout_padded(p.Cout) * sizeof(float) : 0;
}

__global__ void __launch_bounds__(256) scale_weights_kernel(const float* __restrict__ wt, const float* __restrict__ kscale, long total, int K,
                                                            float* __restrict__ out) {
  const long i = (long)blockIdx.x * blockDim.x + threadIdx.x;
  if (i < total) out[i] = wt[i] * kscale[(int)(i % K)];
}

int conv_scale_weights(const float* wt, const float* kscale, int Cout, int K, float* out, hipStream_t stream) {
  const long total = (long)Cout * K;
  hipLaunchKernelGGL(scale_weights_kernel, dim3((unsigned)((total + 255) / 256)), dim3(256), 0, stream, wt, kscale, total, K, out);
  ODT_HIP(hipGetLastError());
  return 0;
}

int conv_make_split_weights(const ConvParams& p, void* img_dev, hipStream_t stream, const float* wt_src, const float* kscale) {
  const float* src = wt_src != nullptr ? wt_src : p.wt;
  ODT_CHECK(kscale == nullptr || (p.kh == 1 && p.kw == 1 && p.in2 == nullptr), "conv_make_split_weights: a folded gate belongs to a single-source 1x1 conv");
  const ConvKernelRow& r = conv_variant_row(p.variant);
  const int bn = r.bn;
  const int K = p.kh * p.kw * p.Cin + (p.in2 != nullptr ? p.Cin2 : 0);
  ODT_CHECK(r.launch != nullptr && r.family != CF_F32 && K % 32 == 0,
            "conv_make_split_weights: Cout % 64 == 0, K % 32 == 0 and a chosen kernel family required");
  if (r.family == CF_H2) {
    ODT_CHECK(kscale == nullptr && wt_src == nullptr, "conv_make_split_weights: the fp16x2 image takes the conv's own weights");
    return conv_make_h2_weights(p, img_dev, stream);
  }
  if (r.family == CF_SPLIT3) {
    const long total = (long)cout_padded(p.Cout) * (K >> 4) * 2;
    hipLaunchKernelGGL(split_weights3_kernel, dim3((unsigned)((total + 255) / 256)), dim3(256), 0, stream, src, p.Cout, K,
                       bn, p.kh * p.kw, p.Cin, (unsigned short*)img_dev, kscale);
  } else {
    const long total = (long)cout_padded(p.Cout) * (K >> 3);
    hipLaunchKernelGGL(split_weights_kernel, dim3((unsigned)((total + 255) / 256)), dim3(256), 0, stream, src, p.Cout, K,
                       bn, 32, (unsigned short*)img_dev, kscale);
  }
  ODT_HIP(hipGetLastError());
  return 0;
}

}
```

### object_detection_tracking_amd/csrc/knobs.hpp

```cpp
#pragma once
#include <string>
#include <vector>

namespace odt {

#define ODT_KNOB_LIST(X)                                                                                                          \
  X(CONV_SPLIT) X(CONV_SPLIT_PIPE) X(CONV_SPLIT_MINTILES) X(CONV_SPLIT3_MINTILES) X(CONV_SPLIT_MINK) X(CONV_SPLIT_MINBN)          \
  X(CONV_H2S_MAXK) X(CONV_H2_FEW_TILES) X(CONV_H2_N64) X(CONV_H2_N64_BM512) X(CONV_H2_BM64) X(CONV_H2K_SPLITK) X(CONV_H2K_FEWROWS) X(CONV_H2_BK64)    \
  X(CONV_H2_ROT) X(CONV_SPLIT3_FILLDIV) X(CONV_SPLIT3_BM) X(CONV_SPLIT3_SPLITK) X(CONV_SPLIT3_KWR) X(CONV_SPLIT3_KWR_N64)         \
  X(CONV_SPLIT3_FORCE_SPLITK) X(CONV_SPLIT_SRC2) X(CONV_SPLIT_RES2) X(SPLIT_REDUCE_BLOCKS) X(CONV_NT) X(AMAX_PER_WAVE) X(ROI_AMAX)            \
  X(CONV_CHUNK_BYTES) X(CONV_TILE) X(CONV_DEBUG) X(CONV_SMALLK) X(CONV_STAGES) X(CONV_FINE) X(CONV_TRACE)                         \
  X(FUSE_SHORTCUT) X(FUSE_RPN_HEAD) X(FUSE_BOTTLENECK) X(FUSE_ROT) X(FUSE_STEM) X(STEM_GRID) X(TAIL_OVERLAP)                      \
  X(SIDE_STREAM_PRIORITY) X(COSINE_STREAM_PRIORITY) X(TRACKER_TIMING)                                                             \
  X(EFFDET_SPLIT) X(EFFDET_FUSE_MB) X(EFFDET_FUSE_MB_MIN) X(EFFDET_WSCALE) X(EFFDET_MERGE_LEVELS) X(DW_PX) X(DW_SUMCAP) X(DW_XCD)

enum Knob : int {
#define ODT_KNOB_ENUM(n) K_##n,
  ODT_KNOB_LIST(ODT_KNOB_ENUM)
#undef ODT_KNOB_ENUM
  K_COUNT
};

struct KnobVal {
  bool set = false;
  long i = 0;
  double d = 0.0;
  char c0 = 0;
};

struct Knobs {
  KnobVal v[K_COUNT];
  std::string text[K_COUNT];
  const KnobVal& get(Knob k) const { return v[k]; }
  bool off(Knob k) const { return v[k].set && v[k].c0 == '0'; }
  long get_long(Knob k, long dflt) const { return v[k].set ? v[k].i : dflt; }
  std::vector<std::string> active() const;
};
Knobs knobs_read();

}
```

### object_detection_tracking_amd/csrc/odt_common.hpp

```cpp
#pragma once
#include <hip/hip_runtime.h>
#include <vector>

#include <cstddef>
#include <cstdint>
#include <cstdio>
#include <functional>
#include <string>

#include "knobs.hpp"

namespace odt {

void set_error(const std::string& msg);

#define ODT_HIP(expr)                                                          \
  do {                                                                         \
    hipError_t odt_e_ = (expr);                                                \
    if (odt_e_ != hipSuccess) {                                                \
      ::odt::set_error(std::string(#expr) + ": " + hipGetErrorString(odt_e_)); \
      return 1;                                                                \
    }                                                                          \
  } while (0)

#define ODT_CHECK(cond, msg)                 \
  do {                                       \
    if (!(cond)) {                           \
      ::odt::set_error(std::string(msg));    \
      return 1;                              \
    }                                        \
  } while (0)

typedef float f32x4 __attribute__((vector_size(16)));
typedef float f32x16 __attribute__((vector_size(64)));

constexpr int kMaxTopK = 1024;
constexpr int kMaxTopKBig = 4096;
#ifndef ODT_AMAX_WAYS
#define ODT_AMAX_WAYS 1
#endif
constexpr int kAmaxWays = ODT_AMAX_WAYS;
constexpr int kRangeSlots = 1024;
constexpr int kRoiOut = 7;
constexpr int kRpnCh = 16;
constexpr int kSelChunk = 32768;
int proposal_total_chunks(const struct ProposalParams& p);

struct ConvParams {
  const float* in;
  const float* wt;
  const float* bias;
  const float* res;
  float* out;
  int B, H, W, Cin, in_ldc;
  int in_Ha, in_Wa;
  int Ho, Wo, Cout;
  int kh, kw, stride, dil, pad_t, pad_l;
  int out_H, out_W, out_oy, out_ox, out_ldc;
  int res_mode;
  int res_H, res_W, res_ldc;
  int relu;
  const float* in2;
  int Cin2, in2_ldc, in2_Ha, in2_Wa, in2_stride;
  unsigned div_howo_mul, div_howo_sh, div_wo_mul, div_wo_sh;
  int debug;
  unsigned long long* trace;
  const void* wt_split;
  int variant;
  int host_unused0_[3];
  int splitk;
  float* partial;
  int nlvl;
  int lvl_start[5];
  int lvl_stride;
  const float* lvl_scale;
  const unsigned* in_amax;
  const unsigned* in2_amax;
  unsigned* out_amax;
  const float* h2_chinv;
  const float* head_wt;
  const float* head_bias;
  float* head_out;
  int head_ldc;
  const void* f_wt;
  const float* f_chinv;
  const float* f_bias;
  const float* f_res;
  float* f_out;
  unsigned* f_out_amax;
  int f_cout, f_out_ldc, f_res_ldc, f_relu;
  int host_unused1_[5];
  int reduce_blocks;
};
static_assert(sizeof(ConvParams) == 432 && offsetof(ConvParams, variant) == 208 && offsetof(ConvParams, splitk) == 224 &&
              offsetof(ConvParams, nlvl) == 240 && offsetof(ConvParams, reduce_blocks) == 428, "ConvParams layout");
void conv_prepare(ConvParams& p);
double conv_flops(const ConvParams& p);

enum ConvFamily : int { CF_F32 = 0, CF_SPLIT1 = 1, CF_H2 = 2, CF_SPLIT3 = 3 };
enum ConvVariantFlag : unsigned {
  CVF_KWR = 1u,
  CVF_DSTAGE = 2u,
  CVF_FTAIL = 4u,
  CVF_STEM = 8u,
  CVF_ST2 = 16u,
  CVF_FINE = 32u,
};
#define ODT_CONV_VARIANT_LIST(X)                                                                                                   \
  X(F32_128x64_S1) X(F32_128x64_S1_FINE) X(F32_128x64_S2) X(F32_128x64_S2_FINE) X(F32_64x64_S1) X(F32_64x64_S1_FINE)              \
  X(F32_64x64_S2) X(F32_64x64_S2_FINE) X(F32_128x128_S1) X(F32_128x128_S1_FINE) X(F32_128x128_S2) X(F32_128x128_S2_FINE)          \
  X(SPLIT1_128x256) X(SPLIT1_256x128) X(SPLIT1_256x64)                                                                            \
  X(SPLIT3_256x256) X(SPLIT3_256x128) X(SPLIT3_256x64) X(SPLIT3_128x256) X(SPLIT3_128x128)                                        \
  X(SPLIT3K_256x256) X(SPLIT3K_256x128) X(SPLIT3K_256x64)                                                                         \
  X(H2_64x64) X(H2_64x128) X(H2_512x64) X(H2_128x64) X(H2_256x256) X(H2_256x128) X(H2_128x128) X(H2D_64x64) X(H2D_64x128)         \
  X(H2K_256x256) X(H2K_256x128) X(H2K_512x64) X(H2K_256x64) X(H2KF_256x64) X(H2KF_256x128) X(H2KF_256x256) X(H2_STEM)
enum ConvVariant : int {
  CV_NONE = 0,
#define ODT_CONV_VARIANT_ENUM(n) CV_##n,
  ODT_CONV_VARIANT_LIST(ODT_CONV_VARIANT_ENUM)
#undef ODT_CONV_VARIANT_ENUM
  CV_COUNT
};
typedef void (*ConvLaunchFn)(const ConvParams* dev, unsigned grid, hipStream_t stream);
struct ConvKernelRow {
  const char* name;
  int family;
  int bm, bn, threads;
  unsigned flags;
  ConvLaunchFn launch;
  ConvLaunchFn launch_traced;
};
#define ODT_CONV_THUNK(threads, kern) \
  [](const ConvParams* dev, unsigned grid, hipStream_t st) { hipLaunchKernelGGL(kern, dim3(grid), dim3(threads), 0, st, dev); }
#define ODT_CONV_ROW(t, id, fam, bm, bn, threads, flags, kern) \
  t[CV_##id] = ConvKernelRow{#id, fam, bm, bn, threads, flags, ODT_CONV_THUNK(threads, kern), nullptr}
#define ODT_CONV_ROW_T(t, id, fam, bm, bn, threads, flags, kern, kern_traced) \
  t[CV_##id] = ConvKernelRow{#id, fam, bm, bn, threads, flags, ODT_CONV_THUNK(threads, kern), ODT_CONV_THUNK(threads, kern_traced)}
const ConvKernelRow& conv_variant_row(int variant);
int conv_variant_find(int family, int bm, int bn, unsigned flags);
int conv_variant_fused_tail(int variant);
void conv_use_variant(ConvParams& p, int variant, int splitk = 1, int reduce_blocks = 0);
void conv_rows_f32(ConvKernelRow* t);
void conv_rows_split1(ConvKernelRow* t);
void conv_rows_split3(ConvKernelRow* t);
void conv_rows_h2(ConvKernelRow* t);
void conv_rows_h2d(ConvKernelRow* t);
void conv_rows_h2k(ConvKernelRow* t);
void conv_rows_stem(ConvKernelRow* t);

struct ConvPolicy {
  int arith;
  int family;
  long min_tiles;
  long min_tiles3;
  int min_k, min_bn;
  int h2s_maxk;
  bool h2_few_tiles;
  bool h2_n64;
  bool h2k_splitk;
  int h2k_fewrows;
  int fill_div;
  int h2_bm64;
  int h2_n64_bm512;
  int force_bm3;
  int splitk_max;
  bool kw_reuse;
  bool kwr_n64;
  int force_splitk;
  bool src2, res2;
};
ConvPolicy conv_policy_default();
ConvPolicy conv_policy_with_knobs(ConvPolicy q, const Knobs& k);
bool conv_split_supported(const ConvParams& p);
struct ConvChoice {
  int variant, splitk, reduce_blocks;
};
ConvChoice conv_select(const ConvParams& p, const ConvPolicy& q, const Knobs& k);
int conv_finish(ConvParams& p, const Knobs& k);
int conv_check(const ConvParams& p);
int conv_check_variant(const ConvParams& p);
int launch_conv(const ConvParams& p, const ConvParams* dev, hipStream_t stream);
bool conv_kwr_fits(const ConvParams& p);
bool conv_h2_sources_ok(const ConvParams& p);
bool conv_h2d_fits(const ConvParams& p);
bool conv_stem_fits(const ConvParams& p);
int conv_stem_grid(const ConvParams& p, unsigned* grid);
size_t conv_split_weight_bytes(int Cout, int K);
int conv_split_bn(int Cout);
int conv_split_bm(int Cout);
int conv_make_split_weights(const ConvParams& p, void* img_dev, hipStream_t stream, const float* wt_src = nullptr,
                            const float* kscale = nullptr);
int conv_scale_weights(const float* wt, const float* kscale, int Cout, int K, float* out, hipStream_t stream);
const float* conv_h2_chinv(const void* img, int Cout, int K);
int conv_make_h2_weights(const ConvParams& p, void* img_dev, hipStream_t stream);
int launch_tensor_amax(const float* x, size_t n, unsigned* slot, hipStream_t stream);
size_t conv_h2f_weight_bytes(int Cout, int K);
const float* conv_h2f_chinv(const void* img, int Cout, int K);
int conv_make_h2f_weights(const float* wt, int Cout, int K, void* img_dev, hipStream_t stream);
bool conv_h2f_fusable(const ConvParams& a, const ConvParams& b);
size_t conv_split_partial_bytes(const ConvParams& p);

int launch_preprocess(const void* frames, int dtype, int B, int H, int W, int pad_t, int pad_l,
                      int Hp, int Wp, float* out, hipStream_t stream, unsigned* amax = nullptr);
int launch_preprocess_resize(const void* frames, int dtype, int B, int Hs, int Ws, int H, int W, int pad_t,
                             int pad_l, int Hp, int Wp, float* out, hipStream_t stream, unsigned* amax = nullptr);
int launch_maxpool3x3s2(const float* in, int B, int H, int W, int C, float* out, int Ho, int Wo,
                        hipStream_t stream);

struct DwConvParams {
  const float* in;
  const float* wt;
  const float* bias;
  float* out;
  int B, H, W, Ho, Wo, ldc, k, stride, pad_t, pad_l;
  int act;
  float* sum_part;
  int cqn, nsplit;
  int xcd_bands;
  int nlvl;
  const float* lin[5];
  float* lout[5];
  int lH[5], lW[5];
  int px;
};
int dwconv_plan(DwConvParams& p, bool squeeze, const Knobs& k);
int launch_dwconv(const DwConvParams& p, hipStream_t stream);
struct MbExpandDwParams {
  const float* x;
  int B, H, W, in_ldc;
  const void* w_img;
  const float* e_bias;
  int mid, lmid;
  const float* dw_wt;
  const float* dw_bias;
  float* out;
  int Ho, Wo, k, stride, pad_t, pad_l;
  float* sum_part;
  int nsplit;
  int tiles_y, tiles_x;
};
int launch_mbconv_expand_dw(const MbExpandDwParams& p, hipStream_t stream);
int mbconv_expand_dw_splits(const MbExpandDwParams& p);
size_t mbconv_expand_weight_bytes(int lmid, int in_ldc);
struct FuseParams {
  const float* in[3];
  int ih[3], iw[3], mode[3];
  float sy[3], sx[3];
  int pt[3], pl[3];
  float wgt[3], denom;
  int n, weighted, act;
  int B, h, w, ldc;
  float* out;
};
int launch_bifpn_fuse(const FuseParams& p, hipStream_t stream);
int launch_preprocess_rgb(const void* frames, int dtype, int B, int H, int W, int pad_t, int pad_l, int Hp, int Wp,
                          float* out, hipStream_t stream);
int channel_mean_splits(int HW, int ldc, int B);
int launch_preprocess_rgb_resize(const void* frames, int dtype, int B, int Hs, int Ws, int Hr, int Wr, int pad_t,
                                 int pad_l, int Hp, int Wp, float* out, hipStream_t stream);
int launch_channel_mean(const float* in, int B, int HW, int ldc, float* scratch, float* out, hipStream_t stream);
int launch_channel_scale(float* x, const float* s, int B, int HW, int ldc, hipStream_t stream);
struct SeGateParams {
  const float* part; int nsplit;
  int HW, ldc, mid, se;
  const float* w1;
  const float* b1;
  const float* w2t;
  const float* b2;
  float* gate;
  float* r;
  float* mean;
};
int launch_se_gate(const float* in, const SeGateParams& p, int B, float* scratch, hipStream_t stream);
int launch_se_gate_from_parts(const SeGateParams& p, int B, hipStream_t stream);

struct ResSeParams {
  const float* t2;
  int B, HW, ch, r, cout;
  const float* w1;
  const float* b1;
  const float* w2t;
  const float* b2;
// ... 163 lines not shown
```

### object_detection_tracking_amd/csrc/odt_model.hpp

```cpp
#pragma once
#include "../../include/odt.h"

#include <algorithm>
#include <cmath>
#include <cstdlib>
#include <cstring>
#include <map>
#include <memory>
#include <mutex>
#include <set>
#include <string>
#include <type_traits>
#include <vector>

#include "odt_common.hpp"

namespace odt {

std::string& last_error();
int launch_subsample2(const float* in, int B, int H, int W, int C, float* out, int Ho, int Wo,
                      hipStream_t stream);

struct DevBuf {
  void* p = nullptr;
  size_t bytes = 0;
  int alloc(size_t n) {
    bytes = n;
    if (n == 0) n = 256;
    ODT_HIP(hipMalloc(&p, n));
    return 0;
  }
  void release() { if (p) (void)hipFree(p); p = nullptr; bytes = 0; }
  ~DevBuf() { release(); }
  DevBuf() = default;
  DevBuf(const DevBuf&) = delete;
  DevBuf& operator=(const DevBuf&) = delete;
};

struct Tensor {
  float* d = nullptr;
  int B = 0, H = 0, W = 0, C = 0;
  int h = 0, w = 0, c = 0;
  size_t elems() const { return (size_t)B * H * W * C; }
};

struct HostTensor {
  std::vector<float> data;
  std::vector<int64_t> shape;
};

struct ConvOp {
  ConvParams p;
  std::string name;
};

enum OpKind { OP_PRE, OP_CONV, OP_POOL, OP_SUB2, OP_PROPOSALS, OP_ROI_HEAD, OP_DETECT, OP_ROI_FINAL,
              OP_ROI_MASK, OP_MASK_SELECT, OP_PRE_RGB, OP_DW, OP_CMEAN, OP_CSCALE, OP_FUSE, OP_EFF_POST, OP_ROI_EFF, OP_SE_GATE,
              OP_SE_GATE_MEAN, OP_WSCALE, OP_MB_EXPAND_DW, OP_RSE_GATE, OP_RSE_APPLY };
struct Op {
  OpKind kind;
  int conv = -1;
  Tensor in, out;
  DwConvParams dw{};
  MbExpandDwParams mb{};
  FuseParams fuse{};
  SeGateParams se{};
  ResSeParams rse{};
  ResSeApplyParams rsa{};
  float* aux = nullptr;
  const float* wt0 = nullptr;
  float* aux2 = nullptr;
  int pad_t = 0, pad_l = 0;
  bool skip = false;
};

}

using namespace odt;

struct odt_model {
  odt_config cfg;
  Knobs knobs;
  int device = 0;
  hipStream_t own_stream = nullptr;
  bool finalized = false;
  std::map<std::string, HostTensor> host_w;
  std::vector<std::unique_ptr<DevBuf>> bufs;
  std::map<std::string, Tensor> taps;
  std::vector<ConvOp> convs;
  std::vector<char> conv_fused;
  ConvParams* convs_dev = nullptr;
  std::vector<ConvParams> conv_recs;
  std::vector<int> conv_rec0, conv_nrec;
  int chunked_convs = 0;
  static constexpr int kAmaxSlots = 512;
  unsigned* amax_dev = nullptr;
  int amax_used[2] = {0, 0};
  unsigned* range_host = nullptr;
  std::vector<float> range_baseline;
  unsigned* range_host_dev = nullptr;
  std::vector<std::string> range_slot_name;
  int convs_h2 = 0;
  int stem_fused = 0;
  int convs_h2f = 0;
  unsigned* pre_amax = nullptr;
  std::vector<Op> ops;
  int Hp = 0, Wp = 0;
  ProposalParams prop{};
  RoiAlignParams roi_head{}, roi_final{}, roi_mask{};
  MaskSelectParams mask_sel{};
  EffPostParams eff_post{};
  RoiAlignParams roi_eff{};
  int eff_filters = 0;
  struct Slot;
  Slot* d2h_slot = nullptr; int d2h_want = 0;
  ConvPolicy policy{};
  int se_blocks = 0;
  int mb_fused = 0;
  int tail_overlap = -1;
  size_t op_first_fpn = 0, op_tail = 0;
  hipStream_t tail_stream = nullptr, done_stream = nullptr;
  hipEvent_t trunk_done = nullptr, tail_done = nullptr;
  bool tail_pending = false;
  unsigned long long forwards_enqueued = 0;
  int eff_scaled_h = 0, eff_scaled_w = 0;
  float* final_masks = nullptr;
  std::map<std::string, std::unique_ptr<DevBuf>> rle_bufs;
  MaskRleHost rle_host;
  DetectParams det{};
  Tensor image_pad, frames_dev;
  int src_h = 0, src_w = 0;
  DevBuf frames_src;
  float* anchors_dev[5] = {nullptr, nullptr, nullptr, nullptr, nullptr};
  float* final_feat = nullptr;
  float* final_pooled = nullptr;
  size_t frames_bytes = 0;
  struct Slot {
    void* pin_in = nullptr; size_t pin_in_bytes = 0;
    void* dev_in = nullptr; size_t dev_in_bytes = 0;
    float *pin_boxes = nullptr, *pin_probs = nullptr, *pin_feats = nullptr, *pin_pooled = nullptr;
    float* pin_masks = nullptr;
    int *pin_labels = nullptr, *pin_valid = nullptr;
    hipEvent_t h2d_done = nullptr, fwd_done = nullptr, d2h_done = nullptr;
    int ticket = -1;
    int ingest_armed = -1;
    int ingest_dtype = 0;
    int want = 0;
  } slot[2];
  hipStream_t copy_in = nullptr, copy_out = nullptr;
  int next_ticket = 0;
  hipEvent_t wait_before_detect = nullptr;
  bool profile = false;
  std::vector<hipEvent_t> ev;
  hipEvent_t ev_total[2] = {nullptr, nullptr};
  double prof_conv_ms = 0, prof_conv_flops = 0, prof_total_ms = 0;
  std::vector<double> prof_layer_ms;
  int prof_launches = 0;

  struct VTensor { size_t bytes = 0, voff = 0, off = 0; int first = 1 << 30, last = -1, region = 0; };
  static constexpr uintptr_t kVirtBase = 0x400000000000ull;
  bool arena_on = false;
  std::set<std::string> transient_taps;
  std::vector<VTensor> vt;
  size_t vnext = 0;
  float* arena[2] = {nullptr, nullptr};
  size_t arena_bytes[2] = {0, 0};
  size_t dedicated_tensor_bytes = 0, virtual_tensor_bytes = 0;
  bool is_virtual(const void* p) const {
    const uintptr_t a = (uintptr_t)p;
    return a >= kVirtBase && a < kVirtBase + vnext;
  }
  int vt_index(const void* p) const {
    const size_t o = (size_t)((uintptr_t)p - kVirtBase);
    size_t lo = 0, hi = vt.size();
    while (hi - lo > 1) { const size_t mid = (lo + hi) / 2; if (vt[mid].voff <= o) lo = mid; else hi = mid; }
    return (int)lo;
  }

  float* alloc_f(size_t elems, bool zero) {
    bufs.emplace_back(new DevBuf());
    if (bufs.back()->alloc(elems * sizeof(float))) return nullptr;
    if (zero && hipMemset(bufs.back()->p, 0, elems * sizeof(float)) != hipSuccess) return nullptr;
    return (float*)bufs.back()->p;
  }
};

namespace odt {

int ceil_div(int a, int b);
int make_tensor(odt_model* m, const std::string& name, int B, int H, int W, int C, Tensor* t, bool zero = false);
const HostTensor* find_w(odt_model* m, const std::string& name);
int upload_conv(odt_model* m, const std::string& scope, int kh, int kw, int cin, int cout, bool has_bn, const float** wt_out,
                const float** bias_out);
int upload_conv_cat(odt_model* m, const std::string& sa, int cin_a, const std::string& sb, int cin_b, int cout,
                    const float** wt_out, const float** bias_out);
int upload_raw(odt_model* m, const std::vector<float>& v, const float** out);
int upload_se_gate(odt_model* m, const std::string& pre, int ch, const float** w1, const float** b1, const float** w2t,
                   const float** b2);
int add_conv(odt_model* m, const std::string& name, const Tensor& in, int cin, const float* wt, const float* bias, int kh,
             int kw, int cout, int stride, int dil, int pad_t, int pad_l, int Ho, int Wo, int oy, int ox, const Tensor* res,
             int res_mode, bool relu, int out_ldc, Tensor* out, const std::string& tap);
int create_side_stream(hipStream_t* s, const Knobs& k);
ConvPolicy resolve_conv_policy(const odt_model* m);
int attach_split_weights(odt_model* m);
int fuse_rpn_heads(odt_model* m);
int fuse_bottleneck_tails(odt_model* m);
int fuse_stem(odt_model* m);
void find_overlap_points(odt_model* m);
int plan_arena(odt_model* m);
int upload_conv_records(odt_model* m);
int build_plan(odt_model* m);
int build_plan_effnet(odt_model* m);
int run_plan(odt_model* m, const void* frames, int dtype, int on_device, hipStream_t st);

inline void rle_fill(const MaskRleHost& h, odt_rle_result* r) {
  r->n = h.n; r->height = h.H0; r->width = h.W0;
  r->strings = h.str.data(); r->offsets = h.off.data(); r->lengths = h.len.data();
  r->counts = h.counts.empty() ? nullptr : h.counts.data();
  r->count_offsets = h.coff.data();
}

template <typename F>
void visit_op_ptrs(odt_model* m, size_t oi, F&& f) {
  Op& op = m->ops[oi];
  if (op.skip) return;
  auto roi = [&](RoiAlignParams& r) {
    for (auto& p : r.feat) f(p);
    f(r.boxes); f(r.out_nhwc); f(r.out_nchw); f(r.pooled);
  };
  f(op.in.d); f(op.out.d);
  switch (op.kind) {
    case OP_PRE: case OP_PRE_RGB: f(m->image_pad.d); break;
    case OP_CONV: { ConvParams& c = m->convs[op.conv].p; f(c.in); f(c.res); f(c.out); f(c.in2); f(c.head_out); f(c.f_res); f(c.f_out); break; }
    case OP_PROPOSALS: for (auto& l : m->prop.lvl) f(l.rpn); f(m->prop.props); break;
    case OP_ROI_HEAD: roi(m->roi_head); break;
    case OP_ROI_FINAL: roi(m->roi_final); break;
    case OP_ROI_MASK: roi(m->roi_mask); break;
    case OP_ROI_EFF: roi(m->roi_eff); break;
    case OP_DETECT: f(m->det.head_out); f(m->det.props); break;
    case OP_MASK_SELECT: f(m->mask_sel.logits); break;
    case OP_DW: f(op.dw.in); f(op.dw.out); for (auto& p : op.dw.lin) f(p); for (auto& p : op.dw.lout) f(p); break;
    case OP_MB_EXPAND_DW: f(op.mb.x); f(op.mb.out); break;
    case OP_RSE_GATE: f(op.rse.t2); f(op.rse.part); f(op.rse.mean); f(op.rse.rvec); f(op.rse.gate); break;
    case OP_RSE_APPLY: f(op.rsa.y); f(op.rsa.sc); f(op.rsa.gate); f(op.rsa.out); break;
    case OP_FUSE: for (auto& p : op.fuse.in) f(p); f(op.fuse.out); break;
    case OP_EFF_POST: for (auto& p : m->eff_post.cls) f(p); for (auto& p : m->eff_post.box) f(p); break;
    case OP_CMEAN: case OP_CSCALE: case OP_SE_GATE: case OP_SE_GATE_MEAN: case OP_WSCALE: case OP_POOL: case OP_SUB2: break;
  }
}

}
```

### object_detection_tracking_amd/csrc/op_shims.hip

```cpp
#include <functional>

#include "odt_model.hpp"

using namespace odt;
#define g_err (::odt::last_error())

namespace {

template <typename T>
struct Tmp {
  T* d = nullptr;
  size_t n = 0;
  int alloc(size_t count) { n = count; ODT_HIP(hipMalloc((void**)&d, (count ? count : 1) * sizeof(T))); return 0; }
  int put(const T* h) { ODT_HIP(hipMemcpy(d, h, n * sizeof(T), hipMemcpyHostToDevice)); return 0; }
  int get(T* h, size_t count) { ODT_HIP(hipMemcpy(h, d, count * sizeof(T), hipMemcpyDeviceToHost)); return 0; }
  int zero() { ODT_HIP(hipMemset(d, 0, (n ? n : 1) * sizeof(T))); return 0; }
  ~Tmp() { if (d) (void)hipFree(d); }
};

int set_dev(int device) {
  int n = 0;
  ODT_HIP(hipGetDeviceCount(&n));
  ODT_CHECK(device >= 0 && device < n, "no such device");
  ODT_HIP(hipSetDevice(device));
// ... 181 lines not shown
      double pa = 0, pb = 0, ma = 0, mb = 0; int na = 0, nb2 = 0;
      for (int b = 0; b < max_blocks; ++b) {
        const unsigned long long* q = &t[(size_t)b * 16];
        if (q[0] == 0) continue;
        double* sx = (q[0] - t0 < 500) ? sa : sb;
        sx[0] += (double)(q[6] - q[0]); sx[1] += (double)(q[7] - q[6]); sx[2] += (double)(q[1] - q[7]);
        if (q[0] - t0 < 500) { pa += (double)(q[1] - q[0]); ma += (double)(q[2] - q[1]); ++na; }
        else { pb += (double)(q[1] - q[0]); mb += (double)(q[2] - q[1]); ++nb2; }
      }
      printf("[conv trace] first wave (%d blocks): prologue %.2f us, mainloop %.2f us | later (%d blocks): prologue %.2f us, mainloop %.2f us\n",
             na, na ? pa / na / 100 : 0.0, na ? ma / na / 100 : 0.0, nb2, nb2 ? pb / nb2 / 100 : 0.0, nb2 ? mb / nb2 / 100 : 0.0);
      if (na && nb2)
        printf("[conv trace] prologue split (setup / first loads+lds / barrier): first wave %.2f / %.2f / %.2f us, later %.2f / %.2f / %.2f us\n",
               sa[0] / na / 100, sa[1] / na / 100, sa[2] / na / 100, sb[0] / nb2 / 100, sb[1] / nb2 / 100, sb[2] / nb2 / 100);
    }
    printf("[conv trace] at mid-launch: %d blocks in prologue, %d in main loop, %d in epilogue\n", in_pro, in_main, in_epi);
    {
      std::map<unsigned, std::vector<int>> cu_blocks;
      for (int b = 0; b < max_blocks; ++b) {
        const unsigned long long* q = &t[(size_t)b * 16];
        if (q[0] == 0) continue;
        const unsigned hw = (unsigned)q[8], xcc = (unsigned)q[9] & 0xf;
        const unsigned cu = (hw >> 8) & 0xf, sh = (hw >> 12) & 1, se = (hw >> 13) & 0x7;
        cu_blocks[(xcc << 12) | (se << 8) | (sh << 4) | cu].push_back(b);
      }
      double frac[4] = {0, 0, 0, 0}; double busy = 0;
      for (auto& kv : cu_blocks) {
        std::vector<std::pair<unsigned long long, int>> ev;
        unsigned long long lo = ~0ull, hi = 0;
        for (int b : kv.second) {
          const unsigned long long* q = &t[(size_t)b * 16];
          ev.push_back({q[1], +1}); ev.push_back({q[2], -1});
          if (q[0] < lo) lo = q[0]; if (q[5] > hi) hi = q[5];
        }
        std::sort(ev.begin(), ev.end());
        unsigned long long prev = lo; int n = 0;
        for (auto& e : ev) {
          frac[n > 3 ? 3 : n] += (double)(e.first - prev); prev = e.first; n += e.second;
        }
        frac[0] += (double)(hi - prev); busy += (double)(hi - lo);
      }
      printf("[conv trace] %zu CUs seen; time share per CU with k workgroups in the main loop: k=0 %.3f  k=1 %.3f  k=2 %.3f  k>=3 %.3f\n",
             cu_blocks.size(), frac[0] / busy, frac[1] / busy, frac[2] / busy, frac[3] / busy);
      printf("[conv trace] XCD0 first blocks -> (se,cu,tg): ");
      for (int b = 0; b < 8 * 40 && b < max_blocks; b += 8) {
        const unsigned long long* q = &t[(size_t)b * 16];
        if (q[0] == 0) break;
        const unsigned hw = (unsigned)q[8];
        printf("%u.%u.%u ", (hw >> 13) & 7, (hw >> 8) & 0xf, (hw >> 16) & 0xf);
      }
      printf("\n");
    }
    fflush(stdout);
  }
  return dout.get(out, nout);
}

int odt_op_conv2d_cat(int device, const float* a, int B, int Ho, int Wo, int Ca, const float* b2, int Hb,
                      int Wb, int Cb, int stride_b, const float* wa, const float* wb, const float* bias,
                      int Cout, int relu, float* out) {
  ODT_CHECK(a && b2 && wa && wb && out, "odt_op_conv2d_cat: null argument");
  ODT_CHECK((Ho - 1) * stride_b < Hb && (Wo - 1) * stride_b < Wb, "odt_op_conv2d_cat: second input too small");
  if (set_dev(device)) return 1;
  std::vector<float> w((size_t)Cout * (Ca + Cb)), bz(Cout, 0.f);
  for (int o = 0; o < Cout; ++o) {
    for (int i = 0; i < Ca; ++i) w[(size_t)o * (Ca + Cb) + i] = wa[(size_t)i * Cout + o];
    for (int i = 0; i < Cb; ++i) w[(size_t)o * (Ca + Cb) + Ca + i] = wb[(size_t)i * Cout + o];
  }
  Tmp<float> da, db2, dw, dbias, dout;
  const size_t na = (size_t)B * Ho * Wo * Ca, nb = (size_t)B * Hb * Wb * Cb, nout = (size_t)B * Ho * Wo * Cout;
  if (da.alloc(na) || db2.alloc(nb) || dw.alloc(w.size()) || dbias.alloc(Cout) || dout.alloc(nout) || dout.zero()) return 1;
  if (da.put(a) || db2.put(b2) || dw.put(w.data()) || dbias.put(bias ? bias : bz.data())) return 1;
  ConvParams p; std::memset(&p, 0, sizeof(p));
  p.in = da.d; p.wt = dw.d; p.bias = dbias.d; p.out = dout.d;
  p.B = B; p.H = Ho; p.W = Wo; p.Cin = Ca; p.in_ldc = Ca; p.in_Ha = Ho; p.in_Wa = Wo;
  p.Ho = Ho; p.Wo = Wo; p.Cout = Cout; p.kh = 1; p.kw = 1; p.stride = 1; p.dil = 1;
  p.out_H = Ho; p.out_W = Wo; p.out_ldc = Cout; p.relu = relu;
  p.in2 = db2.d; p.Cin2 = Cb; p.in2_ldc = Cb; p.in2_Ha = Hb; p.in2_Wa = Wb; p.in2_stride = stride_b;
  if (run_conv(p, knobs_read())) return 1;
  ODT_HIP(hipDeviceSynchronize());
  return dout.get(out, nout);
}

int odt_op_bottleneck_tail(int device, const float* in, int B, int H, int W, int C, const float* w2_hwio, const float* b2,
                           int dil, const float* w3_io, const float* b3, int C3, const float* res, int relu3, int fuse,
                           float* out) {
  ODT_CHECK(in && w2_hwio && b2 && w3_io && b3 && out, "odt_op_bottleneck_tail: null argument");
  ODT_CHECK((C == 256 || C == 128 || C == 64) && C3 % 64 == 0 && C3 > 0 && (dil == 1 || dil == 2), "odt_op_bottleneck_tail: C = 64 / 128 / 256, C3 % 64 == 0, dil 1 or 2");
  if (set_dev(device)) return 1;
  const size_t M = (size_t)B * H * W;
  std::vector<float> w2((size_t)C * 9 * C), w3((size_t)C3 * C);
  for (int y = 0; y < 3; ++y) for (int x = 0; x < 3; ++x) for (int i = 0; i < C; ++i) for (int o = 0; o < C; ++o)
    w2[(((size_t)o * 3 + y) * 3 + x) * C + i] = w2_hwio[(((size_t)y * 3 + x) * C + i) * C + o];
  for (int i = 0; i < C; ++i) for (int o = 0; o < C3; ++o) w3[(size_t)o * C + i] = w3_io[(size_t)i * C3 + o];
  Tmp<float> di, dw2, db2, dw3, db3, dres, dmid, dout, img2, img3, imgf;
  Tmp<unsigned> amax;
  if (di.alloc(M * C) || dw2.alloc(w2.size()) || db2.alloc(C) || dw3.alloc(w3.size()) || db3.alloc(C3) || dmid.alloc(M * C) ||
      dout.alloc(M * C3) || dout.zero() || amax.alloc(4 * kAmaxWays) || amax.zero()) return 1;
  if (di.put(in) || dw2.put(w2.data()) || db2.put(b2) || dw3.put(w3.data()) || db3.put(b3)) return 1;
  if (res) { if (dres.alloc(M * C3) || dres.put(res)) return 1; }
  if (launch_tensor_amax(di.d, M * C, amax.d, nullptr)) return 1;
  ConvParams a; std::memset(&a, 0, sizeof(a));
  a.in = di.d; a.wt = dw2.d; a.bias = db2.d; a.out = dmid.d;
  a.B = B; a.H = H; a.W = W; a.Cin = C; a.in_ldc = C; a.in_Ha = H; a.in_Wa = W; a.Ho = H; a.Wo = W; a.Cout = C;
  a.kh = 3; a.kw = 3; a.stride = 1; a.dil = dil; a.pad_t = dil; a.pad_l = dil;
  a.out_H = H; a.out_W = W; a.out_ldc = C; a.relu = 1;
  conv_use_variant(a, conv_variant_find(CF_H2, 256, C, CVF_KWR));
  a.in_amax = amax.d; a.out_amax = amax.d + kAmaxWays; a.debug = 0x400;
  conv_prepare(a);
  if (img2.alloc((conv_split_weight_bytes(C, 9 * C) + 3) / 4) || conv_make_split_weights(a, img2.d, nullptr)) return 1;
  a.wt_split = img2.d; a.h2_chinv = conv_h2_chinv(img2.d, C, 9 * C);
  ConvParams b; std::memset(&b, 0, sizeof(b));
  b.in = dmid.d; b.wt = dw3.d; b.bias = db3.d; b.out = dout.d; b.res = res ? dres.d : nullptr;
  b.B = B; b.H = H; b.W = W; b.Cin = C; b.in_ldc = C; b.in_Ha = H; b.in_Wa = W; b.Ho = H; b.Wo = W; b.Cout = C3;
  b.kh = 1; b.kw = 1; b.stride = 1; b.dil = 1;
  b.out_H = H; b.out_W = W; b.out_ldc = C3; b.relu = relu3 ? 1 : 0;
  b.res_mode = res ? 1 : 0; b.res_H = H; b.res_W = W; b.res_ldc = C3;
  conv_use_variant(b, C3 % 256 == 0 ? CV_H2_256x256 : (C3 % 128 == 0 ? CV_H2_256x128 : CV_H2_128x64));
  b.in_amax = amax.d + kAmaxWays; b.out_amax = amax.d + 2 * kAmaxWays; b.debug = 0x400;
  conv_prepare(b);
  if (img3.alloc((conv_split_weight_bytes(C3, C) + 3) / 4) || conv_make_split_weights(b, img3.d, nullptr)) return 1;
  b.wt_split = img3.d; b.h2_chinv = conv_h2_chinv(img3.d, C3, C);
  Tmp<ConvParams> rec;
  if (rec.alloc(2)) return 1;
  if (fuse) {
    ODT_CHECK(conv_h2f_fusable(a, b), "odt_op_bottleneck_tail: this pair is not fusable");
    conv_use_variant(a, conv_variant_fused_tail(a.variant));
    if (imgf.alloc((conv_h2f_weight_bytes(C3, C) + 3) / 4) || conv_make_h2f_weights(dw3.d, C3, C, imgf.d, nullptr)) return 1;
    a.f_wt = imgf.d; a.f_chinv = conv_h2f_chinv(imgf.d, C3, C); a.f_bias = db3.d; a.f_res = b.res; a.f_res_ldc = C3;
    a.f_out = dout.d; a.f_out_ldc = C3; a.f_cout = C3; a.f_relu = b.relu; a.f_out_amax = amax.d + 2 * kAmaxWays;
    a.out = nullptr; a.out_amax = nullptr;
    ConvParams recs[2] = {a, b};
    if (conv_check(a) || rec.put(recs)) return 1;
    if (launch_conv(a, rec.d, nullptr)) return 1;
  } else {
    ConvParams recs[2] = {a, b};
    if (conv_check(a) || conv_check(b) || rec.put(recs)) return 1;
    if (launch_conv(a, rec.d, nullptr) || launch_conv(b, rec.d + 1, nullptr)) return 1;
  }
  ODT_HIP(hipDeviceSynchronize());
  return dout.get(out, M * C3);
}

int odt_op_stem(int device, const float* frame_pad, int B, int Hp, int Wp, const float* w_hwio, const float* bias, int fuse,
                int grid, float* out) {
  ODT_CHECK(frame_pad && w_hwio && bias && out && B > 0 && Hp >= 11 && Wp >= 11, "odt_op_stem: null argument / frame too small");
  if (set_dev(device)) return 1;
  const int Ho0 = (Hp - 7) / 2 + 1, Wo0 = (Wp - 7) / 2 + 1, Wa = 2 * Wo0 + 8;
  const int Hq = (Ho0 + 1 - 3) / 2 + 1, Wq = (Wo0 + 1 - 3) / 2 + 1;
  std::vector<float> x((size_t)B * Hp * Wa * 4, 0.f), wv((size_t)64 * 7 * 32, 0.f);
  for (int b = 0; b < B; ++b) for (int y = 0; y < Hp; ++y) for (int xx = 0; xx < Wp; ++xx) for (int c = 0; c < 3; ++c)
    x[(((size_t)b * Hp + y) * Wa + xx) * 4 + c] = frame_pad[(((size_t)b * Hp + y) * Wp + xx) * 3 + c];
  for (int y = 0; y < 7; ++y) for (int xx = 0; xx < 7; ++xx) for (int c = 0; c < 3; ++c) for (int o = 0; o < 64; ++o)
    wv[((size_t)o * 7 + y) * 32 + xx * 4 + c] = w_hwio[(((size_t)y * 7 + xx) * 3 + c) * 64 + o];
  Tmp<float> di, dw, db, dmap, dout, img;
  Tmp<unsigned> amax;
  Tmp<ConvParams> rec;
  const size_t nmap = (size_t)B * Ho0 * Wo0 * 64, nout = (size_t)B * Hq * Wq * 64;
  if (di.alloc(x.size()) || dw.alloc(wv.size()) || db.alloc(64) || dmap.alloc(nmap) || dout.alloc(nout) || dout.zero() ||
      amax.alloc(4 * kAmaxWays) || amax.zero() || rec.alloc(1)) return 1;
  if (di.put(x.data()) || dw.put(wv.data()) || db.put(bias)) return 1;
  if (launch_tensor_amax(di.d, x.size(), amax.d, nullptr)) return 1;
  ConvParams p; std::memset(&p, 0, sizeof(p));
  p.in = di.d; p.wt = dw.d; p.bias = db.d; p.out = dmap.d;
  p.B = B; p.H = Hp; p.W = Wa; p.Cin = 32; p.in_ldc = 4; p.in_Ha = Hp; p.in_Wa = Wa; p.Ho = Ho0; p.Wo = Wo0; p.Cout = 64;
  p.kh = 7; p.kw = 1; p.stride = 2; p.dil = 1; p.out_H = Ho0; p.out_W = Wo0; p.out_ldc = 64; p.relu = 1;
  conv_use_variant(p, CV_H2_128x64);
  p.in_amax = amax.d; p.out_amax = amax.d + kAmaxWays;
  conv_prepare(p);
  if (img.alloc((conv_split_weight_bytes(64, 224) + 3) / 4) || conv_make_split_weights(p, img.d, nullptr)) return 1;
  p.wt_split = img.d; p.h2_chinv = conv_h2_chinv(img.d, 64, 224);
  if (fuse) {
    ODT_CHECK(conv_stem_fits(p), "odt_op_stem: shape not taken by the stem kernel");
    p.out = dout.d; p.out_H = Hq; p.out_W = Wq; conv_use_variant(p, CV_H2_STEM);
    if (grid > 0) p.debug |= (grid & 0x3ff) << 20;
    if (conv_check(p) || rec.put(&p) || launch_conv(p, rec.d, nullptr)) return 1;
  } else {
    if (conv_check(p) || rec.put(&p) || launch_conv(p, rec.d, nullptr)) return 1;
    if (launch_maxpool3x3s2(dmap.d, B, Ho0, Wo0, 64, dout.d, Hq, Wq, nullptr)) return 1;
  }
  ODT_HIP(hipDeviceSynchronize());
  return dout.get(out, nout);
}

int odt_op_conv_choice(const int* shape, int conv_arith, int conv_split_family, int* out, char* name, int name_cap) {
  ODT_CHECK(shape && out, "odt_op_conv_choice: null argument");
  static float ph_f[4]; static unsigned ph_u[4];
  for (int i = 0; i < ODT_CONV_CHOICE_OUT; ++i) out[i] = 0;
  if (name && name_cap > 0) name[0] = 0;
  const int* s = shape;
  ConvParams q; std::memset(&q, 0, sizeof(q));
  q.in = ph_f; q.wt = ph_f; q.bias = ph_f; q.out = ph_f;
  q.B = s[0]; q.H = s[1]; q.W = s[2]; q.Cin = s[3]; q.Cout = s[4]; q.kh = s[5]; q.kw = s[6]; q.stride = s[7]; q.dil = s[8];
  q.pad_t = s[9]; q.pad_l = s[9]; q.Ho = s[10]; q.Wo = s[11]; q.in_Wa = s[12]; q.in_Ha = q.H;
  q.in_ldc = s[16] > 0 ? s[16] : q.Cin; q.out_ldc = s[17] > 0 ? s[17] : q.Cout;
  q.out_H = q.Ho; q.out_W = q.Wo;
  if (s[13] > 0) { q.in2 = ph_f; q.Cin2 = s[13]; q.in2_ldc = s[13]; q.in2_Ha = q.Ho; q.in2_Wa = q.Wo; q.in2_stride = 1; }
  q.res_mode = s[14];
  if (q.res_mode != 0) {
    q.res = ph_f; q.res_ldc = q.out_ldc;
    q.res_H = q.res_mode == 2 ? (q.Ho + 1) / 2 : q.Ho; q.res_W = q.res_mode == 2 ? (q.Wo + 1) / 2 : q.Wo;
  }
  if (s[15]) { q.in_amax = ph_u; if (q.in2 != nullptr) q.in2_amax = ph_u; }
  const Knobs kn = knobs_read();
  if (conv_check(q)) { out[0] = 2; return 0; }
  ConvPolicy pol = conv_policy_default();
  if (conv_arith == ODT_ARITH_F32) pol.arith = 0;
  else if (conv_arith == ODT_ARITH_BF16X3) pol.arith = 1;
  if (conv_split_family >= 1 && conv_split_family <= 3) pol.family = conv_split_family;
  pol = conv_policy_with_knobs(pol, kn);
  const ConvChoice ch = conv_select(q, pol, kn);
  if (conv_variant_row(ch.variant).family != CF_F32) {
    conv_use_variant(q, ch.variant, ch.splitk, ch.reduce_blocks);
    q.wt_split = ph_f;
    if (conv_variant_row(q.variant).family == CF_H2) q.h2_chinv = ph_f;
    if (conv_split_partial_bytes(q) > 0) q.partial = ph_f;
  }
  if (conv_finish(q, kn)) { out[0] = 2; return 0; }
  const ConvKernelRow& r = conv_variant_row(q.variant);
  if (name && name_cap > 0) { std::strncpy(name, r.name, name_cap - 1); name[name_cap - 1] = 0; }
  if (r.family != CF_F32) {
    out[0] = 1; out[1] = r.family; out[2] = r.bm; out[3] = r.bn; out[4] = (r.flags & CVF_KWR) ? 1 : 0; out[5] = q.splitk;
    out[6] = (r.flags & CVF_DSTAGE) ? 1 : 0; out[10] = q.reduce_blocks;
  } else {
// ... 506 lines not shown
```

### object_detection_tracking_amd/csrc/plan_common.hip

```cpp
#include "odt_model.hpp"

#define g_err (::odt::last_error())

namespace odt {

int ceil_div(int a, int b) { return (a + b - 1) / b; }

int make_tensor(odt_model* m, const std::string& name, int B, int H, int W, int C, Tensor* t, bool zero) {
  t->B = B; t->H = H; t->W = W; t->C = C; t->h = H; t->w = W; t->c = C;
  if (m->arena_on && !zero) {
    odt_model::VTensor v;
    v.bytes = (t->elems() * sizeof(float) + 255) & ~(size_t)255;
    v.voff = m->vnext;
    m->vnext += v.bytes;
    m->vt.push_back(v);
    m->virtual_tensor_bytes += v.bytes;
    t->d = reinterpret_cast<float*>(odt_model::kVirtBase + v.voff);
    if (!name.empty()) m->taps[name] = *t;
    return 0;
  }
  t->d = m->alloc_f(t->elems(), zero);
  ODT_CHECK(t->d != nullptr, "device allocation failed for " + name + ": " + g_err);
  m->dedicated_tensor_bytes += t->elems() * sizeof(float);
  if (!name.empty()) m->taps[name] = *t;
// ... 313 lines not shown

int fuse_rpn_heads(odt_model* m) {
  m->conv_fused.assign(m->convs.size(), 0);
  if (m->knobs.off(K_FUSE_RPN_HEAD)) return 0;
  const HostTensor* W = find_w(m, "__rpnhead/W");
  const HostTensor* Bv = find_w(m, "__rpnhead/b");
  if (W == nullptr || Bv == nullptr) return 0;
  const float *hw = nullptr, *hb = nullptr;
  for (size_t oi = 0; oi + 1 < m->ops.size(); ++oi) {
    Op& oa = m->ops[oi]; Op& ob = m->ops[oi + 1];
    if (oa.kind != OP_CONV || ob.kind != OP_CONV) continue;
    ConvOp& a = m->convs[oa.conv]; ConvOp& b = m->convs[ob.conv];
    if (a.name.compare(0, 10, "rpn/conv0@") != 0 || b.name.compare(0, 9, "rpn/head@") != 0) continue;
    const ConvParams& bp = b.p;
    ConvParams& ap = a.p;
    const ConvKernelRow& ar = conv_variant_row(ap.variant);
    const bool ok = ap.wt_split != nullptr && (ar.family == CF_SPLIT3 || ar.family == CF_H2) && ar.bn == 256 && ap.Cout == 256 && ap.splitk <= 1 &&
                    ap.res_mode == 0 && ap.in2 == nullptr && ap.relu <= 1 && bp.in == ap.out && bp.kh == 1 && bp.kw == 1 &&
                    bp.Cin == 256 && bp.Cout == 15 && bp.out_ldc == 16 && bp.stride == 1 && bp.res_mode == 0 && bp.relu == 0 &&
                    bp.out_oy == 0 && bp.out_ox == 0 && bp.out_H == bp.Ho && bp.out_W == bp.Wo && bp.Ho == ap.Ho && bp.Wo == ap.Wo &&
                    ap.out_oy == 0 && ap.out_ox == 0 && ap.out_H == ap.Ho && ap.out_W == ap.Wo && (int)W->data.size() == 256 * 15;
    if (!ok) continue;
    if (hw == nullptr) {
      std::vector<float> v((size_t)256 * 16, 0.f), vb(16, 0.f);
      for (int c = 0; c < 256; ++c)
        for (int j = 0; j < 15; ++j) v[(size_t)c * 16 + j] = W->data[(size_t)c * 15 + j];
      for (int j = 0; j < 15; ++j) vb[j] = Bv->data[j];
      if (upload_raw(m, v, &hw) || upload_raw(m, vb, &hb)) return 1;
    }
    ap.head_wt = hw; ap.head_bias = hb; ap.head_out = bp.out; ap.head_ldc = bp.out_ldc;
    ap.out = nullptr;
    ap.out_amax = nullptr;
    ob.skip = true;
    m->conv_fused[ob.conv] = 1;
  }
  return 0;
}

int fuse_bottleneck_tails(odt_model* m) {
  if (m->conv_fused.size() < m->convs.size()) m->conv_fused.resize(m->convs.size(), 0);
  const char e0 = m->knobs.get(K_FUSE_BOTTLENECK).c0;
  if (e0 == '0') return 0;
  const int min_cout = e0 == '1' ? 256 : (e0 == '2' ? 128 : 64);
  if (m->policy.arith == 0 || m->policy.family != 2) return 0;
  if (m->cfg.use_se) return 0;
  std::map<const float*, const void*> made;
  for (size_t oi = 0; oi + 1 < m->ops.size(); ++oi) {
    Op& oa = m->ops[oi]; Op& ob = m->ops[oi + 1];
    if (oa.kind != OP_CONV || ob.kind != OP_CONV || oa.skip || ob.skip) continue;
    ConvOp& a = m->convs[oa.conv]; ConvOp& b = m->convs[ob.conv];
    if (a.p.Cout < min_cout) continue;
    if (!conv_h2f_fusable(a.p, b.p)) continue;
    bool other = false;
    for (size_t k = 0; k < m->ops.size() && !other; ++k) {
      if (k == oi || k == oi + 1) continue;
      visit_op_ptrs(m, k, [&](auto& ptr) { if ((const void*)ptr == (const void*)a.p.out) other = true; });
    }
    for (const auto& kv : m->taps) if (kv.second.d == a.p.out) other = true;
    if (other) continue;
    const int K = b.p.Cin;
    auto it = made.find(b.p.wt);
    if (it == made.end()) {
      float* img = m->alloc_f((conv_h2f_weight_bytes(b.p.Cout, K) + 3) / 4, false);
      ODT_CHECK(img != nullptr, "device allocation failed (fused 1x1 weights of " + b.name + ")");
      if (conv_make_h2f_weights(b.p.wt, b.p.Cout, K, img, 0)) return 1;
      it = made.emplace(b.p.wt, img).first;
    }
    ConvParams& ap = a.p;
    conv_use_variant(ap, conv_variant_fused_tail(ap.variant), ap.splitk, ap.reduce_blocks);
    ap.f_wt = it->second; ap.f_chinv = conv_h2f_chinv(it->second, b.p.Cout, K); ap.f_bias = b.p.bias;
    ap.f_res = b.p.res_mode != 0 ? b.p.res : nullptr; ap.f_res_ldc = b.p.res_ldc;
    ap.f_out = b.p.out; ap.f_out_ldc = b.p.out_ldc; ap.f_cout = b.p.Cout; ap.f_relu = b.p.relu; ap.f_out_amax = b.p.out_amax;
    ap.debug |= b.p.debug & 0x400;
    if (m->knobs.off(K_FUSE_ROT)) ap.debug |= 0x100;
    ap.out = nullptr; ap.out_amax = nullptr;
    ob.skip = true;
    m->conv_fused[ob.conv] = 2;
    ++m->convs_h2f;
  }
  ODT_HIP(hipDeviceSynchronize());
  return 0;
}

int fuse_stem(odt_model* m) {
  if (m->knobs.off(K_FUSE_STEM)) return 0;
  if (m->policy.arith == 0 || m->policy.family != 2) return 0;
  for (size_t oi = 0; oi + 1 < m->ops.size(); ++oi) {
    Op& oa = m->ops[oi]; Op& ob = m->ops[oi + 1];
    if (oa.kind != OP_CONV || ob.kind != OP_POOL || oa.skip || ob.skip) continue;
    ConvParams& ap = m->convs[oa.conv].p;
    if (ob.in.d != ap.out || ap.out == nullptr || !conv_stem_fits(ap) || ap.out_oy != 0 || ap.out_ox != 0 || ap.out_H != ap.Ho || ap.out_W != ap.Wo ||
        ob.in.h != ap.Ho || ob.in.w != ap.Wo || ob.in.C != 64 || ob.out.H != (ap.Ho + 1 - 3) / 2 + 1 || ob.out.W != (ap.Wo + 1 - 3) / 2 + 1 ||
        ob.out.C < 64 || (double)ap.B * ob.out.H * ob.out.W * ob.out.C * 4.0 >= 2147483648.0) continue;
    bool other = false;
    for (size_t k = 0; k < m->ops.size() && !other; ++k) {
      if (k == oi || k == oi + 1) continue;
      visit_op_ptrs(m, k, [&](auto& ptr) { if ((const void*)ptr == (const void*)ap.out) other = true; });
    }
    if (!m->arena_on) for (const auto& kv : m->taps) if (kv.second.d == ap.out) other = true;
    if (other) continue;
    for (auto it = m->taps.begin(); it != m->taps.end();) { if (it->second.d == ap.out) it = m->taps.erase(it); else ++it; }
    ap.out = ob.out.d; ap.out_H = ob.out.H; ap.out_W = ob.out.W; ap.out_ldc = ob.out.C;
    conv_use_variant(ap, CV_H2_STEM, ap.splitk, ap.reduce_blocks);
    if (m->knobs.get(K_STEM_GRID).set) ap.debug |= ((int)m->knobs.get(K_STEM_GRID).i & 0x3ff) << 20;
    ob.skip = true;
    m->stem_fused = 1;
  }
  return 0;
}

void find_overlap_points(odt_model* m) {
  m->op_first_fpn = m->op_tail = 0;
  if (m->cfg.graph == ODT_GRAPH_EFFNET) return;
  for (size_t i = 0; i < m->ops.size(); ++i) {
    if (m->ops[i].kind == OP_PROPOSALS) { m->op_tail = i; break; }
    if (m->op_first_fpn == 0 && m->ops[i].kind == OP_CONV && m->convs[m->ops[i].conv].name.compare(0, 4, "fpn/") == 0)
      m->op_first_fpn = i;
  }
  if (m->op_tail == 0 || m->op_first_fpn == 0 || m->op_first_fpn >= m->op_tail) m->op_first_fpn = m->op_tail = 0;
}

int plan_arena(odt_model* m) {
  if (!m->arena_on || m->vt.empty()) return 0;
  find_overlap_points(m);
  const int nops = (int)m->ops.size();
  for (int oi = 0; oi < nops; ++oi)
    visit_op_ptrs(m, (size_t)oi, [&](auto& p) {
      if (p == nullptr || !m->is_virtual((const void*)p)) return;
      odt_model::VTensor& v = m->vt[m->vt_index((const void*)p)];
      v.first = std::min(v.first, oi); v.last = std::max(v.last, oi);
    });
  const bool split = m->op_tail > 0;
  std::vector<char> tapped(m->vt.size(), 0);
  for (const auto& kv : m->taps)
    if (kv.second.d != nullptr && m->is_virtual(kv.second.d)) tapped[m->vt_index(kv.second.d)] = 1;
  for (size_t i = 0; i < m->vt.size(); ++i) {
    auto& v = m->vt[i];
    if (v.last < 0 && !tapped[i]) { v.bytes = 0; v.first = v.last = 0; }
    if (v.last < 0) { v.first = 0; v.last = nops - 1; }
    v.region = split && v.last >= (int)m->op_tail ? 1 : 0;
    ODT_CHECK(v.region == 0 || v.bytes == 0 || v.first >= (int)m->op_first_fpn || tapped[i],
              "activation arena: a tensor the tail ops read is produced before the FPN stage (tail overlap would race)");
    if (v.region == 1) v.last = nops - 1;
  }
  std::vector<int> order(m->vt.size());
  for (size_t i = 0; i < order.size(); ++i) order[i] = (int)i;
  std::sort(order.begin(), order.end(), [&](int a, int b) {
    return m->vt[a].bytes != m->vt[b].bytes ? m->vt[a].bytes > m->vt[b].bytes : a < b;
  });
  std::vector<int> placed;
  for (int id : order) {
    odt_model::VTensor& v = m->vt[id];
    std::vector<std::pair<size_t, size_t>> busy;
    for (int q : placed) {
      const odt_model::VTensor& u = m->vt[q];
      if (u.region == v.region && u.first <= v.last && v.first <= u.last) busy.emplace_back(u.off, u.off + u.bytes);
    }
    std::sort(busy.begin(), busy.end());
    size_t off = 0;
    for (const auto& b : busy) {
      if (off + v.bytes <= b.first) break;
      off = std::max(off, b.second);
    }
    v.off = off;
    m->arena_bytes[v.region] = std::max(m->arena_bytes[v.region], off + v.bytes);
    placed.push_back(id);
  }
  for (int r = 0; r < 2; ++r) {
    if (m->arena_bytes[r] == 0) continue;
    m->arena[r] = m->alloc_f(m->arena_bytes[r] / sizeof(float), false);
    ODT_CHECK(m->arena[r] != nullptr, "device allocation failed (activation arena): " + g_err);
  }
  auto fix = [&](auto& p) {
    if (p == nullptr || !m->is_virtual((const void*)p)) return;
    const odt_model::VTensor& v = m->vt[m->vt_index((const void*)p)];
    const size_t within = (size_t)((uintptr_t)p - odt_model::kVirtBase) - v.voff;
    p = reinterpret_cast<std::remove_reference_t<decltype(p)>>(reinterpret_cast<char*>(m->arena[v.region]) + v.off + within);
  };
  for (auto& kv : m->taps) {
    if (kv.second.d != nullptr && m->is_virtual(kv.second.d)) {
      const odt_model::VTensor& v = m->vt[m->vt_index(kv.second.d)];
      if (v.region == 0 && !(v.first == 0 && v.last == nops - 1)) m->transient_taps.insert(kv.first);
    }
    fix(kv.second.d);
  }
  for (size_t oi = 0; oi < m->ops.size(); ++oi) visit_op_ptrs(m, oi, fix);
  fix(m->image_pad.d);
  for (size_t oi = 0; oi < m->ops.size(); ++oi) {
    const Op& op = m->ops[oi];
    if (op.kind != OP_CONV || op.skip) continue;
    const ConvParams& c = m->convs[op.conv].p;
    for (const void* q : {(const void*)c.in, (const void*)c.res, (const void*)c.out, (const void*)c.in2, (const void*)c.head_out,
                          (const void*)c.f_res, (const void*)c.f_out})
      ODT_CHECK(q == nullptr || !m->is_virtual(q), "activation arena: unmapped pointer left in " + m->convs[op.conv].name);
  }
  return 0;
}

static int conv_batch_chunks(const ConvParams& p, double limit) {
  auto fits = [&](int n) {
    const double b = (double)(p.B / n);
    return b * p.in_Ha * p.in_Wa * p.in_ldc * 4.0 < limit && b * p.out_H * p.out_W * p.out_ldc * 4.0 < limit &&
           (p.res_mode == 0 || b * p.res_H * p.res_W * p.res_ldc * 4.0 < limit) &&
           (p.in2 == nullptr || b * p.in2_Ha * p.in2_Wa * p.in2_ldc * 4.0 < limit) &&
           (p.f_wt == nullptr || (b * p.Ho * p.Wo * p.f_out_ldc * 4.0 < limit && (p.f_res == nullptr || b * p.Ho * p.Wo * p.f_res_ldc * 4.0 < limit)));
  };
  for (int n = 1; n <= p.B; ++n)
    if (p.B % n == 0 && fits(n)) return n;
  return p.B;
}

int upload_conv_records(odt_model* m) {
  double limit = 2147483648.0;
  if (m->knobs.get(K_CONV_CHUNK_BYTES).d > 0) limit = m->knobs.get(K_CONV_CHUNK_BYTES).d;
  m->conv_recs.clear(); m->conv_rec0.clear(); m->conv_nrec.clear();
  std::vector<char> launched(m->convs.size(), 0);
  for (const Op& op : m->ops)
    if (op.kind == OP_CONV && !op.skip) launched[op.conv] = 1;
  for (size_t ci = 0; ci < m->convs.size(); ++ci) {
    const ConvOp& c = m->convs[ci];
    const ConvParams& p = c.p;
    const int n = conv_batch_chunks(p, limit), bc = p.B / n;
    m->conv_rec0.push_back((int)m->conv_recs.size());
    m->conv_nrec.push_back(n);
    for (int k = 0; k < n; ++k) {
      ConvParams q = p;
      const size_t b0 = (size_t)k * bc;
      q.B = bc;
      q.in = p.in + b0 * p.in_Ha * p.in_Wa * p.in_ldc;
      if (p.out != nullptr) q.out = p.out + b0 * p.out_H * p.out_W * p.out_ldc;
      if (p.res != nullptr) q.res = p.res + b0 * p.res_H * p.res_W * p.res_ldc;
      if (p.in2 != nullptr) q.in2 = p.in2 + b0 * p.in2_Ha * p.in2_Wa * p.in2_ldc;
      if (p.head_out != nullptr) q.head_out = p.head_out + b0 * p.Ho * p.Wo * p.head_ldc;
      if (p.f_out != nullptr) q.f_out = p.f_out + b0 * p.Ho * p.Wo * p.f_out_ldc;
      if (p.f_res != nullptr) q.f_res = p.f_res + b0 * p.Ho * p.Wo * p.f_res_ldc;
      if (launched[ci] && conv_finish(q, m->knobs)) { g_err = c.name + ": " + g_err; return 1; }
      m->conv_recs.push_back(q);
    }
    if (n > 1) ++m->chunked_convs;
  }
  m->bufs.emplace_back(new DevBuf());
  if (m->bufs.back()->alloc(m->conv_recs.size() * sizeof(ConvParams))) return 1;
  m->convs_dev = (ConvParams*)m->bufs.back()->p;
  ODT_HIP(hipMemcpy(m->convs_dev, m->conv_recs.data(), m->conv_recs.size() * sizeof(ConvParams), hipMemcpyHostToDevice));
  return 0;
}

}
```

### object_detection_tracking_amd/csrc/plan_fpn.hip

```cpp
#include "odt_model.hpp"

#define g_err (::odt::last_error())

namespace odt {

int build_plan(odt_model* m) {
  const odt_config& cfg = m->cfg;
  m->arena_on = cfg.keep_taps == 0;
  if (cfg.graph == ODT_GRAPH_EFFNET) return build_plan_effnet(m);
  const int B = cfg.batch, H = cfg.height, W = cfg.width;
  const int FC = cfg.fpn_channels;
  const int ph = ceil_div(H, 32) * 32 - H, pw = ceil_div(W, 32) * 32 - W;
  const int Hp = 3 + H + 2 + ph, Wpl = 3 + W + 2 + pw;
  const int Ho0 = (Hp - 7) / 2 + 1, Wo0 = (Wpl - 7) / 2 + 1;
  const int Wp = 2 * Wo0 + 8;
  m->Hp = Hp; m->Wp = Wp;
  if (make_tensor(m, "image_pad", B, Hp, Wp, 4, &m->image_pad)) return 1;
  m->frames_bytes = (size_t)B * H * W * 3 * sizeof(float);
  m->src_h = H; m->src_w = W;
  { m->bufs.emplace_back(new DevBuf()); if (m->bufs.back()->alloc(m->frames_bytes)) return 1;
    m->frames_dev.d = (float*)m->bufs.back()->p; }
  { Op op; op.kind = OP_PRE; m->ops.push_back(op); }

  const float *wt = nullptr, *bias = nullptr;
// ... 265 lines not shown
  dp.props = props.d; dp.nprops = pp.nprops; dp.img_h = H; dp.img_w = W;
  for (int i = 0; i < 4; ++i) dp.reg_w[i] = cfg.bbox_reg_weights[i];
  dp.decode_clip = cfg.head_decode_clip; dp.score_thresh = cfg.result_score_thresh;
  dp.nms_thresh = cfg.head_nms_thresh; dp.per_im = cfg.result_per_im;
  const int per_im = cfg.result_per_im;
  Tensor dec{}, prb{};
  if (make_tensor(m, "decoded_boxes", 1, B * K, C - 1, 4, &dec, true)) return 1;
  if (make_tensor(m, "label_probs", 1, 1, B * K, C, &prb, true)) return 1;
  dp.dec_boxes = dec.d; dp.probs = prb.d;
  dp.cls_keep = (int*)m->alloc_f((size_t)B * (C - 1) * per_im, true);
  dp.cls_count = (int*)m->alloc_f((size_t)B * (C - 1), true);
  dp.out_boxes = m->alloc_f((size_t)B * per_im * 4, true);
  dp.out_probs = m->alloc_f((size_t)B * per_im, true);
  dp.out_labels = (int*)m->alloc_f((size_t)B * per_im, true);
  dp.out_valid = (int*)m->alloc_f(B, true);
  ODT_CHECK(dp.cls_keep && dp.cls_count && dp.out_boxes && dp.out_probs && dp.out_labels && dp.out_valid,
            "device allocation failed (detections)");
  { Op op; op.kind = OP_DETECT; m->ops.push_back(op); }

  m->final_feat = m->alloc_f((size_t)B * per_im * FC * 49, true);
  m->final_pooled = m->alloc_f((size_t)B * per_im * FC, true);
  ODT_CHECK(m->final_feat && m->final_pooled, "device allocation failed (features)");
  RoiAlignParams& rf = m->roi_final;
  rf.boxes = dp.out_boxes; rf.per_image = per_im; rf.count = dp.out_valid; rf.R_cap = B * per_im;
  rf.out_nhwc = nullptr; rf.out_nchw = m->final_feat; rf.pooled = m->final_pooled;
  rf.pack_rows = 1;
  { Op op; op.kind = OP_ROI_FINAL; m->ops.push_back(op); }

  if (cfg.add_mask) {
    ODT_CHECK(cfg.graph == ODT_GRAPH_SINGLE, "add_mask: built for the single-image graph only");
    const int MD = cfg.mask_dim > 0 ? cfg.mask_dim : 256;
    ODT_CHECK(MD % 32 == 0, "add_mask: mrcnn_head_dim must be a multiple of 32");
    const int R = B * per_im;
    Tensor mroi{};
    if (make_tensor(m, "mask_roi", R, 14, 14, FC, &mroi, true)) return 1;
    m->roi_mask = m->roi_final;
    m->roi_mask.out_nhwc = mroi.d; m->roi_mask.out_nchw = nullptr; m->roi_mask.pooled = nullptr;
    m->roi_mask.out_size = 14;
    { Op op; op.kind = OP_ROI_MASK; m->ops.push_back(op); }
    Tensor cur = mroi;
    int cin = FC;
    for (int k = 0; k < 4; ++k) {
      const std::string sc = "maskrcnn/fcn" + std::to_string(k);
      if (upload_conv(m, sc, 3, 3, cin, MD, false, &wt, &bias)) return 1;
      Tensor nx{};
      if (add_conv(m, sc, cur, cin, wt, bias, 3, 3, MD, 1, 1, 1, 1, 14, 14, 0, 0, nullptr, 0, true, MD, &nx,
                   "mask_fcn" + std::to_string(k))) return 1;
      cur = nx; cin = MD;
    }
    {
      const HostTensor* wd = find_w(m, "maskrcnn/deconv/W"); const HostTensor* bd = find_w(m, "maskrcnn/deconv/b");
      ODT_CHECK(wd && bd, "missing maskrcnn/deconv variables");
      ODT_CHECK(wd->data.size() == (size_t)4 * MD * MD && bd->data.size() == (size_t)MD, "bad maskrcnn/deconv shapes");
      HostTensor v, vb; v.data.resize((size_t)MD * 4 * MD); vb.data.resize((size_t)4 * MD);
      for (int q = 0; q < 4; ++q)
        for (int co = 0; co < MD; ++co) {
          vb.data[(size_t)q * MD + co] = bd->data[co];
          for (int ci = 0; ci < MD; ++ci)
            v.data[(size_t)ci * 4 * MD + (size_t)q * MD + co] = wd->data[((size_t)q * MD + co) * MD + ci];
        }
      m->host_w["__maskdeconv/W"] = v; m->host_w["__maskdeconv/b"] = vb;
      if (upload_conv(m, "__maskdeconv", 1, 1, MD, 4 * MD, false, &wt, &bias)) return 1;
    }
    Tensor dc{};
    if (add_conv(m, "maskrcnn/deconv", cur, MD, wt, bias, 1, 1, 4 * MD, 1, 1, 0, 0, 14, 14, 0, 0, nullptr, 0, true,
                 4 * MD, &dc, "mask_deconv")) return 1;
    Tensor dv = dc;
    dv.W = dv.w = 56; dv.C = MD; dv.c = MD;
    if (upload_conv(m, "maskrcnn/conv", 1, 1, MD, C - 1, false, &wt, &bias)) return 1;
    Tensor ml{};
    const int mld = (C - 1 + 3) / 4 * 4;
    if (add_conv(m, "maskrcnn/conv", dv, MD, wt, bias, 1, 1, C - 1, 1, 1, 0, 0, 14, 56, 0, 0, nullptr, 0, false, mld,
                 &ml, "mask_logits")) return 1;
    m->final_masks = m->alloc_f((size_t)R * 784, true);
    ODT_CHECK(m->final_masks != nullptr, "device allocation failed (masks)");
    MaskSelectParams& ms = m->mask_sel;
    ms.logits = ml.d; ms.ld = ml.C; ms.labels = dp.out_labels; ms.valid = dp.out_valid; ms.B = B;
    ms.per_image = per_im; ms.masks = m->final_masks;
    { Op op; op.kind = OP_MASK_SELECT; m->ops.push_back(op); }
  }
  if (attach_split_weights(m)) return 1;
  if (fuse_rpn_heads(m)) return 1;
  if (fuse_bottleneck_tails(m)) return 1;
  if (fuse_stem(m)) return 1;
  if (plan_arena(m)) return 1;
  if (upload_conv_records(m)) return 1;
  return 0;
}

}
```

### object_detection_tracking_amd/csrc/runtime.hip

```cpp
#include <cmath>
#include <thread>

#include "odt_model.hpp"

namespace odt {

std::string& last_error() {
  static thread_local std::string err;
  return err;
}
void set_error(const std::string& msg) { last_error() = msg; }

}

using namespace odt;
#define g_err (::odt::last_error())

namespace odt {

static int run_ops(odt_model* m, const void* src, int dtype, hipStream_t st, size_t* ev_io, size_t begin = 0,
                   size_t end = (size_t)-1) {
  const odt_config& cfg = m->cfg;
  size_t ev_i = *ev_io;
  for (size_t oi = begin; oi < end && oi < m->ops.size(); ++oi) {
// ... 545 lines not shown
  if (want & ODT_WANT_POOLED)
    ODT_HIP(hipMemcpyAsync(sl.pin_pooled, h->final_pooled, B * per * FC * sizeof(float), hipMemcpyDeviceToHost, co));
  if ((want & ODT_WANT_MASKS) && h->final_masks)
    ODT_HIP(hipMemcpyAsync(sl.pin_masks, h->final_masks, B * per * 784 * sizeof(float), hipMemcpyDeviceToHost, co));
  ODT_HIP(hipEventRecord(sl.d2h_done, co));
  sl.ticket = t;
  *ticket = t;
  h->next_ticket = t + 1;
  return 0;
}

int odt_collect(odt_handle h, int ticket, odt_outputs* out) {
  ODT_CHECK(h && out, "odt_collect: null argument");
  odt_model::Slot& sl = h->slot[ticket & 1];
  ODT_CHECK(ticket >= 0 && sl.ticket == ticket, "odt_collect: unknown or already collected ticket");
  ODT_HIP(hipSetDevice(h->device));
  ODT_HIP(hipEventSynchronize(sl.d2h_done));
  const odt_config& cfg = h->cfg;
  const size_t B = cfg.batch, per = cfg.result_per_im, FC = cfg.fpn_channels;
  size_t total = 0;
  for (size_t b = 0; b < B; ++b) total += (size_t)sl.pin_valid[b];
  if (out->valid) std::memcpy(out->valid, sl.pin_valid, B * sizeof(int));
  if (out->boxes) std::memcpy(out->boxes, sl.pin_boxes, B * per * 4 * sizeof(float));
  if (out->probs) std::memcpy(out->probs, sl.pin_probs, B * per * sizeof(float));
  if (out->labels) std::memcpy(out->labels, sl.pin_labels, B * per * sizeof(int));
  ODT_CHECK(!out->feats || (sl.want & ODT_WANT_FEATS), "odt_collect: feats requested but the ticket was submitted without ODT_WANT_FEATS");
  ODT_CHECK(!out->pooled || (sl.want & ODT_WANT_POOLED), "odt_collect: pooled requested but the ticket was submitted without ODT_WANT_POOLED");
  ODT_CHECK(!out->masks || (sl.want & ODT_WANT_MASKS), "odt_collect: masks requested but the ticket was submitted without ODT_WANT_MASKS");
  if (out->feats) std::memcpy(out->feats, sl.pin_feats, total * FC * 49 * sizeof(float));
  if (out->pooled) std::memcpy(out->pooled, sl.pin_pooled, total * FC * sizeof(float));
  if (out->masks) {
    ODT_CHECK(sl.pin_masks != nullptr, "odt_collect: masks requested but the model was built without add_mask");
    std::memcpy(out->masks, sl.pin_masks, (size_t)h->cfg.batch * h->cfg.result_per_im * 784 * sizeof(float));
  }
  sl.ticket = -1;
  return 0;
}

int odt_tap(odt_handle h, const char* name, float* dst, size_t cap_elems, int64_t* shape_out, int* rank_out) {
  ODT_CHECK(h && name && shape_out && rank_out, "odt_tap: null argument");
  ODT_HIP(hipSetDevice(h->device));
  if (std::string(name) == "nproposals") {
    shape_out[0] = h->cfg.batch; *rank_out = 1;
    if (dst) {
      ODT_CHECK(cap_elems >= (size_t)h->cfg.batch, "odt_tap: buffer too small");
      std::vector<int> v(h->cfg.batch);
      ODT_HIP(hipDeviceSynchronize());
      ODT_HIP(hipMemcpy(v.data(), h->prop.nprops, v.size() * sizeof(int), hipMemcpyDeviceToHost));
      for (size_t i = 0; i < v.size(); ++i) dst[i] = (float)v[i];
    }
    return 0;
  }
  auto it = h->taps.find(name);
  ODT_CHECK(it != h->taps.end(), std::string("odt_tap: unknown stage ") + name);
  ODT_CHECK(h->transient_taps.count(name) == 0, std::string("odt_tap: stage tensor ") + name + " is not kept after a forward "
            "(its memory is reused inside the activation arena): create the handle with odt_config.keep_taps = 1");
  const Tensor& t = it->second;
  shape_out[0] = t.B; shape_out[1] = t.H; shape_out[2] = t.W; shape_out[3] = t.C; *rank_out = 4;
  if (dst) {
    ODT_CHECK(cap_elems >= t.elems(), "odt_tap: buffer too small");
    ODT_HIP(hipDeviceSynchronize());
    ODT_HIP(hipMemcpy(dst, t.d, t.elems() * sizeof(float), hipMemcpyDeviceToHost));
  }
  return 0;
}

int odt_profile_enable(odt_handle h, int enable) {
  ODT_CHECK(h != nullptr, "null handle");
  h->profile = enable != 0;
  h->prof_conv_ms = h->prof_conv_flops = h->prof_total_ms = 0; h->prof_launches = 0;
  h->prof_layer_ms.assign(h->convs.size(), 0.0);
  return 0;
}

int odt_profile_layer(odt_handle h, int index, char* name, int name_cap, double* flops, double* ms,
                      int64_t* mnk, int* count) {
  ODT_CHECK(h != nullptr, "null handle");
  if (count) *count = (int)h->convs.size();
  if (index < 0 || index >= (int)h->convs.size()) return 0;
  const ConvOp& c = h->convs[index];
  if (name && name_cap > 0) {
    const bool fused = index < (int)h->conv_fused.size() && h->conv_fused[index];
    const ConvKernelRow& row = conv_variant_row(c.p.variant);
    const std::string nm = c.name + (fused ? "[fused into the producer's epilogue]" : (c.p.head_wt != nullptr ? "+head" : ((row.flags & CVF_FTAIL) ? "+conv3" : ((row.flags & CVF_STEM) ? "+pool0" : "")))) +
                           (!fused && c.p.wt_split != nullptr ? (row.family == CF_H2 ? "[fp16x2]" : "[bf16x3]") : "");
    std::strncpy(name, nm.c_str(), name_cap - 1); name[name_cap - 1] = 0;
  }
  if (flops) *flops = (index < (int)h->conv_fused.size() && h->conv_fused[index]) ? 0.0 : conv_flops(c.p);
  if (ms) *ms = index < (int)h->prof_layer_ms.size() ? h->prof_layer_ms[index] : 0.0;
  if (mnk) { mnk[0] = (int64_t)c.p.B * c.p.Ho * c.p.Wo; mnk[1] = c.p.Cout; mnk[2] = (int64_t)c.p.kh * c.p.kw * c.p.Cin; }
  return 0;
}

int odt_describe(odt_handle h, char* buf, int cap) {
  ODT_CHECK(h != nullptr && buf != nullptr && cap > 0, "odt_describe: null argument");
  int fam[4] = {0, 0, 0, 0}, nsk = 0, nfused = 0;
  for (size_t i = 0; i < h->convs.size(); ++i) {
    const ConvOp& c = h->convs[i];
    if (i < h->conv_fused.size() && h->conv_fused[i]) { ++nfused; continue; }
    fam[c.p.wt_split != nullptr ? conv_variant_row(c.p.variant).family : CF_F32] += 1;
    if (c.p.wt_split != nullptr && c.p.splitk > 1) ++nsk;
  }
  int se_conv1_h2 = 0;
  if (h->se_blocks > 0)
    for (const ConvOp& c : h->convs) {
      const size_t n = c.name.size();
      if (n > 6 && c.name.compare(n - 6, 6, "/conv1") == 0 && c.p.wt_split != nullptr && conv_variant_row(c.p.variant).family == CF_H2)
        ++se_conv1_h2;
    }
  size_t dev_bytes = 0;
  for (const auto& b : h->bufs) dev_bytes += b->bytes;
  dev_bytes += h->frames_src.bytes;
  for (const auto& sl : h->slot) dev_bytes += sl.dev_in_bytes;
  const std::vector<std::string> active = h->knobs.active();
  std::string envs;
  for (size_t i = 0; i < active.size(); ++i) {
    std::string e = active[i];
    for (char& ch : e) if (ch == '"' || ch == '\\' || (unsigned char)ch < 0x20) ch = '?';
    envs += (i ? ", \"" : "\"") + e + "\"";
  }
  char tmp[8192];
  std::snprintf(tmp, sizeof(tmp),
                "{\"conv_arith\": \"%s\", \"conv_launches\": %d, \"convs_fused_into_epilogues\": %d, \"exact_f32_mfma_launches\": %d, "
                "\"bf16x3_split_launches\": %d, \"fp16x2_split_launches\": %d, \"bottleneck_tails_fused\": %d, \"stem_fused\": %d, \"mbconv_expand_dw_fused\": %d, \"split_launches_by_family\": {\"split3_8wave_lds_dma\": %d, "
                "\"one_stage_bk32\": %d, \"h2_8wave_lds_dma\": %d, \"of_split3_with_split_k\": %d}, \"policy\": {\"family\": %d, \"min_tiles\": %ld, "
                "\"min_tiles3\": %ld, \"min_k\": %d}, \"env_overrides_applied\": %d, \"env_overrides\": [%s], "
                "\"memory\": {\"device_bytes\": %zu, \"activation_arena_bytes\": [%zu, %zu], \"arena_tensors\": %zu, "
                "\"arena_tensor_bytes_unshared\": %zu, \"dedicated_tensor_bytes\": %zu, \"keep_taps\": %d}, \"convs_cut_into_batch_ranges\": %d, "
                "\"use_se\": %d, \"se_blocks\": %d, \"se_blocks_conv1_on_fp16x2\": %d}",
                h->policy.arith != 0 && fam[2] > 0 ? "f32 through fp16x2 / bf16x3 split products"
                    : (h->policy.arith != 0 && fam[1] + fam[3] > 0 ? "f32 through bf16x3 split products" : "exact f32 MFMA"),
                (int)h->convs.size() - nfused, nfused, fam[0], fam[1] + fam[3], fam[2], h->convs_h2f, h->stem_fused, h->mb_fused, fam[3], fam[1], fam[2], nsk, h->policy.family,
                h->policy.min_tiles, h->policy.min_tiles3, h->policy.min_k, (int)active.size(), envs.c_str(),
                dev_bytes, h->arena_bytes[0], h->arena_bytes[1], h->vt.size(), h->virtual_tensor_bytes,
                h->dedicated_tensor_bytes, h->cfg.keep_taps, h->chunked_convs, h->cfg.use_se != 0 ? 1 : 0, h->se_blocks, se_conv1_h2);
  ODT_CHECK((int)std::strlen(tmp) < cap, "odt_describe: buffer too small");
  std::strncpy(buf, tmp, cap - 1); buf[cap - 1] = 0;
  return 0;
}

int odt_range_health(odt_handle h, int rebase, double* worst_growth, char* tensor, int tensor_cap, double* tensor_amax, long long* tensors_seen) {
  ODT_CHECK(h != nullptr && worst_growth != nullptr, "odt_range_health: null argument");
  double worst = 0.0, wamax = 0.0;
  int wslot = -1;
  long long seen = 0;
  if (h->range_host != nullptr && !h->range_baseline.empty()) {
    const volatile unsigned* r = h->range_host;
    for (int g = 0; g < 2; ++g)
      for (int i = g * odt_model::kAmaxSlots; i < g * odt_model::kAmaxSlots + h->amax_used[g]; ++i) {
        const unsigned bits = r[i];
        float a; std::memcpy(&a, &bits, 4);
        if (!(a > 0.f) || !std::isfinite(a)) continue;
        ++seen;
        float& base = h->range_baseline[i];
        if (!(base > 0.f)) { base = a; continue; }
        const double f = (double)a / (double)base;
        if (f > worst) { worst = f; wslot = i; wamax = a; }
        if (rebase) base = a;
      }
  }
  *worst_growth = worst;
  if (tensor_amax) *tensor_amax = wamax;
  if (tensors_seen) *tensors_seen = seen;
  if (tensor != nullptr && tensor_cap > 0) {
    const std::string nm = wslot >= 0 && wslot < (int)h->range_slot_name.size() ? h->range_slot_name[wslot] : std::string();
    std::strncpy(tensor, nm.c_str(), tensor_cap - 1); tensor[tensor_cap - 1] = 0;
  }
  return 0;
}

int odt_profile_read(odt_handle h, double* conv_ms, double* conv_flops, int* conv_launches, double* total_ms) {
  ODT_CHECK(h != nullptr, "null handle");
  if (conv_ms) *conv_ms = h->prof_conv_ms;
  if (conv_flops) *conv_flops = h->prof_conv_flops;
  if (conv_launches) *conv_launches = h->prof_launches;
  if (total_ms) *total_ms = h->prof_total_ms;
  return 0;
}

}
```

### object_detection_tracking_amd/ops.py

```python
from __future__ import annotations

import ctypes as C

import numpy as np

from . import _lib
from ._lib import RPN_CH, c_float_p, f32, fptr, i32, iptr


def _L(lib):
  return lib if lib is not None else _lib.get_lib()


def conv2d(x_nhwc, w_hwio, bias=None, stride=1, dil=1, pad_t=0, pad_l=0, out_hw=None,
           out_off=(0, 0), res=None, res_mode=0, relu=False, lib=None, device=0):
  lib = _L(lib)
  x = f32(x_nhwc); w = f32(w_hwio)
  B, H, W, Cin = x.shape
  kh, kw, _, Cout = w.shape
  if out_hw is None:
    ke_h, ke_w = (kh - 1) * dil + 1, (kw - 1) * dil + 1
    out_hw = ((H + 2 * pad_t - ke_h) // stride + 1, (W + 2 * pad_l - ke_w) // stride + 1)
  Ho, Wo = out_hw
  oy, ox = out_off
  out = np.zeros((B, Ho + oy, Wo + ox, Cout), np.float32)
  b = f32(bias) if bias is not None else None
  r = f32(res) if res is not None else None
  lib.check(lib.dll.odt_op_conv2d(device, fptr(x), B, H, W, Cin, fptr(w),
                                  fptr(b) if b is not None else None, kh, kw, Cout, stride, dil,
                                  pad_t, pad_l, Ho, Wo, oy, ox,
                                  fptr(r) if r is not None else None, res_mode, int(relu),
                                  fptr(out)))
  return out


def conv2d_cat(a, b2, wa, wb, bias=None, stride_b=1, relu=False, lib=None, device=0):
  lib = _L(lib)
  a = f32(a); b2 = f32(b2); wa = f32(wa); wb = f32(wb)
  B, Ho, Wo, Ca = a.shape
  _, Hb, Wb, Cb = b2.shape
  Cout = wa.shape[1]
  out = np.zeros((B, Ho, Wo, Cout), np.float32)
  bb = f32(bias) if bias is not None else None
  lib.check(lib.dll.odt_op_conv2d_cat(device, fptr(a), B, Ho, Wo, Ca, fptr(b2), Hb, Wb, Cb, stride_b,
                                      fptr(wa), fptr(wb), fptr(bb) if bb is not None else None, Cout,
                                      int(relu), fptr(out)))
  return out


def bottleneck_tail(x, w2, b2, w3, b3, res=None, dil=1, relu3=True, fuse=True, lib=None, device=0):
  lib = _L(lib)
  x = f32(x); w2 = f32(w2); b2 = f32(b2); w3 = f32(w3); b3 = f32(b3)
  B, H, W, Cc = x.shape
  C3 = w3.shape[1]
  r = f32(res) if res is not None else None
  out = np.zeros((B, H, W, C3), np.float32)
  lib.check(lib.dll.odt_op_bottleneck_tail(device, fptr(x), B, H, W, Cc, fptr(w2), fptr(b2), dil, fptr(w3), fptr(b3), C3,
                                           fptr(r) if r is not None else None, int(relu3), int(fuse), fptr(out)))
  return out


def stem(frame_pad, w_hwio, bias, fuse=True, grid=0, lib=None, device=0):
  lib = _L(lib)
  x = f32(frame_pad); w = f32(w_hwio); b = f32(bias)
  B, Hp, Wp, _ = x.shape
  Ho0, Wo0 = (Hp - 7) // 2 + 1, (Wp - 7) // 2 + 1
  Hq, Wq = (Ho0 + 1 - 3) // 2 + 1, (Wo0 + 1 - 3) // 2 + 1
  out = np.zeros((B, Hq, Wq, 64), np.float32)
  lib.check(lib.dll.odt_op_stem(device, fptr(x), B, Hp, Wp, fptr(w), fptr(b), int(fuse), int(grid), fptr(out)))
  return out


CONV_CHOICE_SHAPE = ("B", "H", "W", "Cin", "Cout", "kh", "kw", "stride", "dil", "pad", "Ho", "Wo", "in_Wa", "Cin2", "res_mode", "ranges",
                     "in_ldc", "out_ldc")
CONV_CHOICE_OUT = ("status", "kind", "bm", "bn", "kwr", "splitk", "dstage", "f32_tile", "f32_stages", "f32_fine", "reduce_blocks")


def conv_choice(shape, conv_arith=0, conv_split_family=0, lib=None):
  lib = lib if lib is not None else _lib.OdtLib(_lib.LIB_HIP_PATH)
  s = i32(list(shape)); out = np.zeros(len(CONV_CHOICE_OUT), np.int32)
  assert s.shape == (len(CONV_CHOICE_SHAPE),)
  name = C.create_string_buffer(64)
  lib.check(lib.dll.odt_op_conv_choice(iptr(s), int(conv_arith), int(conv_split_family), iptr(out), name, 64))
  d = dict(zip(CONV_CHOICE_OUT, (int(v) for v in out)))
  d["name"] = name.value.decode()
  return d


def preprocess(frames, pad_t, pad_l, Hp, Wp, lib=None, device=0):
  lib = _L(lib)
  fr = np.ascontiguousarray(frames)
  assert fr.dtype in (np.uint8, np.float32)
  B, H, W, _ = fr.shape
  out = np.zeros((B, Hp, Wp, 4), np.float32)
  lib.check(lib.dll.odt_op_preprocess(device, fr.ctypes.data_as(C.c_void_p),
                                      0 if fr.dtype == np.uint8 else 1, B, H, W, pad_t, pad_l,
                                      Hp, Wp, fptr(out)))
  return out


def maxpool3x3s2(x_nhwc, lib=None, device=0):
  lib = _L(lib)
  x = f32(x_nhwc)
  B, H, W, Cc = x.shape
  out = np.zeros((B, (H + 1 - 3) // 2 + 1, (W + 1 - 3) // 2 + 1, Cc), np.float32)
  lib.check(lib.dll.odt_op_maxpool(device, fptr(x), B, H, W, Cc, fptr(out)))
  return out


def top_k(scores, k, lib=None, device=0):
  lib = _L(lib)
  s = f32(scores).reshape(-1)
  idx = np.zeros((k,), np.int32)
  lib.check(lib.dll.odt_op_topk(device, fptr(s), s.size, k, iptr(idx)))
  return idx


def nms(boxes, scores, max_out, iou_thresh, lib=None, device=0):
  lib = _L(lib)
  b = f32(boxes).reshape(-1, 4); s = f32(scores).reshape(-1)
  idx = np.zeros((max(1, s.size),), np.int32)
  n = C.c_int(0)
  lib.check(lib.dll.odt_op_nms(device, fptr(b), fptr(s), s.size, max_out, iou_thresh, iptr(idx),
                               C.byref(n)))
  return idx[:n.value].copy()


def pack_rpn(logits, deltas):
  B, h, w, A = logits.shape
  out = np.zeros((B, h, w, RPN_CH), np.float32)
  out[..., :A] = logits
  out[..., A:A + 4 * A] = np.asarray(deltas, np.float32).reshape(B, h, w, 4 * A)
  return out


def proposals(graph, rpn_levels, anchors, img_hw, K, nms_thresh, decode_clip, lib=None, device=0):
  lib = _L(lib)
  L = len(rpn_levels)
  rp = [f32(r) for r in rpn_levels]; an = [f32(a) for a in anchors]
  B = rp[0].shape[0]
  hs = i32([r.shape[1] for r in rp]); ws = i32([r.shape[2] for r in rp])
  fs = i32([a.shape[0] for a in an])
# ... 259 lines not shown
```

Measured before the change: 312.4.

## Fuse next bottleneck's 1x1 conv1 into previous block's fused conv3 tail

```diff
diff --git a/include/odt.h b/include/odt.h
--- a/include/odt.h
+++ b/include/odt.h
@@ -162,6 +162,10 @@
 int odt_op_bottleneck_tail(int device, const float* in, int B, int H, int W, int C, const float* w2,
                            const float* b2, int dil, const float* w3, const float* b3, int C3,
                            const float* res, int relu3, int fuse, float* out);
+int odt_op_bottleneck_tail_next(int device, const float* in, int B, int H, int W, int C, const float* w2,
+                                const float* b2, int dil, const float* w3, const float* b3, int C3,
+                                const float* res, int relu3, const float* w1, const float* b1, int N1,
+                                float* out, float* out1);
 int odt_op_stem(int device, const float* frame_pad, int B, int Hp, int Wp, const float* w_hwio, const float* bias,
                 int fuse, int grid, float* out);
 #define ODT_CONV_CHOICE_SHAPE 18
diff --git a/object_detection_tracking_amd/_lib.py b/object_detection_tracking_amd/_lib.py
--- a/object_detection_tracking_amd/_lib.py
+++ b/object_detection_tracking_amd/_lib.py
@@ -94,7 +94,7 @@
       "odt_forward_async", "odt_synchronize", "odt_read_outputs", "odt_describe", "odt_range_health", "odt_submit", "odt_submit_ex", "odt_collect",
       "odt_ingest_buffer", "odt_set_source_size", "odt_tap", "odt_profile_enable",
       "odt_profile_read", "odt_profile_layer", "odt_probe_mfma_bf16", "odt_nn_cosine", "odt_op_conv2d", "odt_op_conv2d_cat",
-      "odt_op_bottleneck_tail", "odt_op_stem", "odt_op_conv_choice", "odt_op_preprocess",
+      "odt_op_bottleneck_tail", "odt_op_bottleneck_tail_next", "odt_op_stem", "odt_op_conv_choice", "odt_op_preprocess",
       "odt_op_maxpool", "odt_op_topk", "odt_op_nms", "odt_op_proposals",
       "odt_op_roi_align", "odt_op_detections", "odt_op_class_nms",
       "odt_op_dwconv", "odt_op_se_gate", "odt_op_rse_gate", "odt_op_rse_apply", "odt_op_se_tail", "odt_op_bifpn_fuse", "odt_op_mbconv_expand_dw", "odt_op_effdet_post",
@@ -148,6 +148,8 @@
         [c_float_p, c_float_p, c_float_p, C.c_int, C.c_int, c_float_p]
     d.odt_op_bottleneck_tail.argtypes = [C.c_int, c_float_p] + [C.c_int] * 4 + [c_float_p, c_float_p, C.c_int, c_float_p, c_float_p,
                                          C.c_int, c_float_p, C.c_int, C.c_int, c_float_p]
+    d.odt_op_bottleneck_tail_next.argtypes = [C.c_int, c_float_p] + [C.c_int] * 4 + [c_float_p, c_float_p, C.c_int, c_float_p, c_float_p,
+                                              C.c_int, c_float_p, C.c_int, c_float_p, c_float_p, C.c_int, c_float_p, c_float_p]
     d.odt_op_stem.argtypes = [C.c_int, c_float_p] + [C.c_int] * 3 + [c_float_p, c_float_p, C.c_int, C.c_int, c_float_p]
     d.odt_op_conv_choice.argtypes = [c_int_p, C.c_int, C.c_int, c_int_p, C.c_char_p, C.c_int]
     d.odt_op_preprocess.argtypes = [C.c_int, C.c_void_p] + [C.c_int] * 8 + [c_float_p]
diff --git a/object_detection_tracking_amd/csrc/conv_h2.hip b/object_detection_tracking_amd/csrc/conv_h2.hip
--- a/object_detection_tracking_amd/csrc/conv_h2.hip
+++ b/object_detection_tracking_amd/csrc/conv_h2.hip
@@ -337,6 +337,26 @@
   }
 }
 
+__global__ void split_weights_h2g_kernel(const float* __restrict__ wt, int Cout, int K, unsigned short* __restrict__ img,
+                                         const float* __restrict__ chinv) {
+  const long idx = (long)blockIdx.x * blockDim.x + threadIdx.x;
+  const int KG = K >> 3, NB = Cout >> 5;
+  if (idx >= (long)Cout * KG) return;
+  const int n = (int)(idx / KG), kg = (int)(idx - (long)n * KG);
+  const int c = kg >> 2, h = (kg >> 1) & 1, fg = kg & 1, j = n >> 5, fr = n & 31;
+  const float sc = 1.0f / chinv[n];
+  for (int e = 0; e < 8; e += 2) {
+    const int k0 = kg * 8 + e;
+    unsigned piece[2];
+    split2h(wt[(size_t)n * K + k0], wt[(size_t)n * K + k0 + 1], sc, piece[0], piece[1]);
+    for (int q = 0; q < 2; ++q) {
+      const size_t at = ((((((size_t)c * 2 + q) * NB + j) * 2 + h) * 2 + fg) * 32 + fr) * 8 + e;
+      img[at] = (unsigned short)(piece[q] & 0xffffu);
+      img[at + 1] = (unsigned short)(piece[q] >> 16);
+    }
+  }
+}
+
 __global__ void __launch_bounds__(256) tensor_amax_kernel(const float* __restrict__ x, size_t n, unsigned* __restrict__ slot) {
   float m = 0.f;
   for (size_t i = (size_t)blockIdx.x * 256 + threadIdx.x; i < n; i += (size_t)gridDim.x * 256) m = fmaxf(m, fabsf(x[i]));
@@ -378,6 +398,35 @@
                      (unsigned short*)img_dev, chinv);
   ODT_HIP(hipGetLastError());
   return 0;
+}
+
+size_t conv_h2g_weight_bytes(int Cout, int K) { return (size_t)Cout * K * 4 + (size_t)Cout * 4; }
+const float* conv_h2g_chinv(const void* img, int Cout, int K) {
+  return reinterpret_cast<const float*>(reinterpret_cast<const char*>(img) + (size_t)Cout * K * 4);
+}
+int conv_make_h2g_weights(const float* wt, int Cout, int K, void* img_dev, hipStream_t stream) {
+  ODT_CHECK((Cout == 64 || Cout == 128) && K % 32 == 0 && K >= 64, "conv_make_h2g_weights: Cout = 64 / 128 and K % 32 == 0 required");
+  float* chinv = const_cast<float*>(conv_h2g_chinv(img_dev, Cout, K));
+  hipLaunchKernelGGL(h2_rowscale_kernel, dim3((unsigned)Cout), dim3(256), 0, stream, wt, Cout, K, chinv);
+  const long total = (long)Cout * (K >> 3);
+  hipLaunchKernelGGL(split_weights_h2g_kernel, dim3((unsigned)((total + 255) / 256)), dim3(256), 0, stream, wt, Cout, K,
+                     (unsigned short*)img_dev, chinv);
+  ODT_HIP(hipGetLastError());
+  return 0;
+}
+
+bool conv_h2g_fusable(const ConvParams& a, const ConvParams& b) {
+  const ConvKernelRow& ra = conv_variant_row(a.variant);
+  const bool a_ok = a.f_wt != nullptr && (ra.flags & CVF_FTAIL) != 0 && (ra.bn == 64 || ra.bn == 128) && a.g_wt == nullptr &&
+                    a.f_out != nullptr && a.f_cout >= 64 && a.trace == nullptr;
+  const bool b_ok = b.in == a.f_out && b.kh == 1 && b.kw == 1 && b.stride == 1 && b.pad_t == 0 && b.pad_l == 0 && b.Cin == a.f_cout &&
+                    b.in_ldc == a.f_out_ldc && b.in2 == nullptr && b.B == a.B && b.H == a.Ho && b.W == a.Wo && b.Ho == a.Ho &&
+                    b.Wo == a.Wo && b.in_Ha == a.Ho && b.in_Wa == a.Wo && (b.Cout == 128 || (b.Cout == 64 && ra.bn == 64)) &&
+                    b.out_oy == 0 && b.out_ox == 0 && b.out_H == b.Ho && b.out_W == b.Wo && b.out_ldc % 4 == 0 && b.out_ldc >= b.Cout &&
+                    b.res_mode == 0 && b.relu <= 1 && b.nlvl <= 1 && b.head_wt == nullptr && b.splitk <= 1 && b.wt_split != nullptr &&
+                    conv_variant_row(b.variant).family == CF_H2 && b.f_wt == nullptr && b.out != nullptr &&
+                    (double)b.B * b.Ho * b.Wo * b.out_ldc * 4.0 < 2147483648.0;
+  return a_ok && b_ok;
 }
 
 bool conv_h2f_fusable(const ConvParams& a, const ConvParams& b) {
diff --git a/object_detection_tracking_amd/csrc/conv_h2k.hip b/object_detection_tracking_amd/csrc/conv_h2k.hip
--- a/object_detection_tracking_amd/csrc/conv_h2k.hip
+++ b/object_detection_tracking_amd/csrc/conv_h2k.hip
@@ -28,13 +28,14 @@
   static constexpr int LDS0 = RING > CTILE ? RING : CTILE;
   static constexpr int F_KOFF = F_CEND > LDS0 ? F_CEND : LDS0;
   static constexpr int F_K3OFF = F_KOFF + 2048;
-  static constexpr int LDS = FUSE ? F_K3OFF + 8192 : LDS0;
+  static constexpr int G_WOFF = F_K3OFF + 8192;
+  static constexpr int LDS = FUSE ? G_WOFF : LDS0;
   static constexpr int NW = STAGE_B / 1024 / 8;
   static constexpr int RA = (PR + 63) / 64;
   static_assert(LDS <= 160 * 1024 && STAGE_B % 8192 == 0 && (!FUSE || WN == 2), "LDS");
 };
 
-template <int TN, bool TRACE>
+template <int TN, bool TRACE, int GNB>
 __device__ __forceinline__ void h2f_tail(const ConvParams& p, f32x16 (&acc)[2][TN], unsigned char* lds, int m0, int M,
                                          int wave, int wm, int wn, float h2_inv) {
   using G = H2kCfg<TN, true>;
@@ -43,6 +44,8 @@
   const int lane = ODT_LANE_ID();
   const int tid = wave * 64 + lane, fr = lane & 31, fg = lane >> 5;
   const int nch = p.f_cout >> 5;
+  constexpr int GCH = GNB * 4096, GN1 = GNB > 0 ? GNB : 1;
+  f32x16 gacc[GN1];
 
   const float* kc = reinterpret_cast<const float*>(lds + G::F_KOFF);
   const float act2_lo = p.relu == 1 ? 0.f : -__builtin_huge_valf();
@@ -152,6 +155,14 @@
   };
   dma_w(0, 0);
   dma_w(1, 1);
+  const __amdgpu_buffer_rsrc_t rs_g = __builtin_amdgcn_make_buffer_rsrc((void*)(GNB > 0 ? p.g_wt : p.f_wt), 0, (int)((unsigned)nch * (unsigned)GCH), 0x00020000);
+  auto dma_g = [&](int cs, int buf) {
+    const int c = ce(cs);
+#pragma unroll
+    for (int i = 0; i < GCH / 8192; ++i)
+      __builtin_amdgcn_raw_ptr_buffer_load_lds(rs_g, ODT_LDS_PTR(lds + G::G_WOFF + buf * GCH + (i * 8 + wave) * 1024), 16,
+                                               lane * 16 + (i * 8 + wave) * 1024, c * GCH, 0, 0);
+  };
 
   const unsigned mrows = (unsigned)M;
   const __amdgpu_buffer_rsrc_t rs_res = __builtin_amdgcn_make_buffer_rsrc(
@@ -169,11 +180,15 @@
     const unsigned off = has_res && c < nch && m_first + 64u * s2 < mrows ? roff0 + s2 * rstep : kOOB;
     return (f32x4)__builtin_amdgcn_raw_buffer_load_b128(rs_res, (int)off, c * 128, 2);
   };
-  f32x4 ra[4], rb[4];
+  constexpr int RAHEAD = GNB > 0 && TN >= 2 ? 1 : 2;
+  f32x4 ra[4], rb_[RAHEAD == 2 ? 4 : 1];
+  f32x4 (&rb)[4] = *reinterpret_cast<f32x4 (*)[4]>(RAHEAD == 2 ? rb_ : ra);
 #pragma unroll
   for (int s2 = 0; s2 < 4; ++s2) ra[s2] = fetch_res(0, s2);
-#pragma unroll
-  for (int s2 = 0; s2 < 4; ++s2) rb[s2] = fetch_res(1, s2);
+  if constexpr (RAHEAD == 2) {
+#pragma unroll
+    for (int s2 = 0; s2 < 4; ++s2) rb[s2] = fetch_res(1, s2);
+  }
   const unsigned char* wrd = lds + lane * 16;
   float* Cst = reinterpret_cast<float*>(lds + COFF);
   const int cw_at = (wm * 64 + wn * 32 + fr) * CS + 4 * fg;
@@ -193,9 +208,60 @@
     const bool ok = m_first + 64u * s2 < mrows;
     vmax = fmaxf(vmax, ok ? vm : 0.f);
     __builtin_amdgcn_raw_buffer_store_b128((u32x4)v, rs_out, (int)(ok ? ooff0 + s2 * ostep : kOOB), c * 128, 0);
-    rr = fetch_res(cs + 2, s2);
-  };
-  ODT_WAIT_VM_LGKM0(8);
+    rr = fetch_res(cs + RAHEAD, s2);
+    if constexpr (GNB > 0) {
+      ODT_FENCE();
+      float rm = vm;
+      rm = fmaxf(rm, __shfl_xor(rm, 1)); rm = fmaxf(rm, __shfl_xor(rm, 2)); rm = fmaxf(rm, __shfl_xor(rm, 4));
+      const int be = (int)((__float_as_uint(rm) >> 23) & 0xffu);
+      int e = 14 - (be - 127);
+      e = e > 100 ? 100 : (e < -100 ? -100 : e);
+      e = (be == 0) | (be == 255) ? 0 : e;
+      const float rs = pow2f(e);
+      unsigned h0, l0, h1, l1;
+      split2h(v[0], v[1], rs, h0, l0);
+      split2h(v[2], v[3], rs, h1, l1);
+      float* rowp = const_cast<float*>(Cb) + (row0 + 64 * s2) * CS;
+      *reinterpret_cast<u32x2*>(rowp + c4 * 2) = u32x2{h0, h1};
+      *reinterpret_cast<u32x2*>(rowp + 16 + c4 * 2) = u32x2{l0, l1};
+      if (c4 == 0) rowp[32] = pow2f(-e);
+      ODT_FENCE();
+    }
+  };
+  auto g_mma = [&](int cs, auto&& between) {
+    if constexpr (GNB > 0) {
+      const float* rowp = Cst + (cs & 1) * (CBUF / 4) + (wm * 64 + wn * 32 + fr) * CS;
+      f16x8 yh[2], yl[2];
+#pragma unroll
+      for (int h = 0; h < 2; ++h) {
+        yh[h] = *reinterpret_cast<const f16x8*>(rowp + h * 8 + fg * 4);
+        yl[h] = *reinterpret_cast<const f16x8*>(rowp + 16 + h * 8 + fg * 4);
+      }
+      const float sinv = rowp[32];
+      ODT_FENCE();
+      between();
+      const unsigned char* wb = lds + G::G_WOFF + (cs & 1) * GCH + lane * 16;
+#pragma unroll
+      for (int j = 0; j < GNB; ++j) {
+        ODT_FENCE();
+        f32x16 part;
+#pragma unroll
+        for (int r = 0; r < 16; ++r) part[r] = 0.f;
+#pragma unroll
+        for (int h = 0; h < 2; ++h) {
+          const f16x8 whi = *reinterpret_cast<const f16x8*>(wb + (j * 2 + h) * 1024);
+          const f16x8 wlo = *reinterpret_cast<const f16x8*>(wb + ((GNB + j) * 2 + h) * 1024);
+          part = ODT_MFMA_F16(wlo, yh[h], part);
+          part = ODT_MFMA_F16(whi, yl[h], part);
+          part = ODT_MFMA_F16(whi, yh[h], part);
+          if (h == 0) ODT_FENCE();
+        }
+        gacc[j] += part * sinv;
+      }
+      ODT_FENCE();
+    }
+  };
+  ODT_WAIT_VM_LGKM0(4 * RAHEAD);
   __builtin_amdgcn_s_barrier();
   auto chunk = [&](int c, f32x4 (&rprev)[4], auto HP) {
     constexpr bool has_prev = decltype(HP)::value;
@@ -228,19 +294,31 @@
         else row_item(c - 1, u, rprev[u]);
       }
     }
-    float* Cb = Cst + buf * (CBUF / 4) + cw_at;
-#pragma unroll
-    for (int g = 0; g < 4; ++g) {
-      f32x4 a = {co[4 * g], co[4 * g + 1], co[4 * g + 2], co[4 * g + 3]};
-      a = a * yinv_k;
-      *reinterpret_cast<f32x4*>(Cb + 8 * g) = a;
-    }
+    auto store_co = [&]() {
+      float* Cb = Cst + buf * (CBUF / 4) + cw_at;
+#pragma unroll
+      for (int g = 0; g < 4; ++g) {
+        f32x4 a = {co[4 * g], co[4 * g + 1], co[4 * g + 2], co[4 * g + 3]};
+        a = a * yinv_k;
+        *reinterpret_cast<f32x4*>(Cb + 8 * g) = a;
+      }
+    };
+    if constexpr (GNB > 0 && has_prev) { if (c >= 2) g_mma(c - 2, store_co); else store_co(); }
+    else store_co();
     if constexpr (has_prev) ODT_WAIT_VM_LGKM0(8); else ODT_WAIT_VM_LGKM0(0);
     __builtin_amdgcn_s_barrier();
     ODT_FENCE();
     dma_w(c + 2, buf);
+    if constexpr (GNB > 0) dma_g(c, buf);
     ODT_FENCE();
   };
+  if constexpr (GNB > 0) {
+    ODT_FENCE();
+#pragma unroll
+    for (int j = 0; j < GNB; ++j)
+#pragma unroll
+      for (int r = 0; r < 16; ++r) gacc[j][r] = 0.f;
+  }
   chunk(0, ra, std::false_type{});
   int c = 1;
 #pragma unroll 1
@@ -256,17 +334,52 @@
 #pragma unroll
     for (int s2 = 0; s2 < 4; ++s2) row_item(c - 1, s2, ra[s2]);
   }
-  publish_amax_wg<512>(p.f_out_amax, vmax, tid, lds);
+  if constexpr (GNB > 0) {
+    ODT_WAIT_VM_LGKM0(0);
+    __builtin_amdgcn_s_barrier();
+    g_mma(nch - 2, [] {});
+    g_mma(nch - 1, [] {});
+    const unsigned gn = (unsigned)p.g_cout;
+    const __amdgpu_buffer_rsrc_t rs_gs = __builtin_amdgcn_make_buffer_rsrc((void*)p.g_chinv, 0, (int)(gn * 4u), 0x00020000);
+    const __amdgpu_buffer_rsrc_t rs_gb = __builtin_amdgcn_make_buffer_rsrc((void*)p.g_bias, 0, (int)(gn * 4u), 0x00020000);
+    const __amdgpu_buffer_rsrc_t rs_go = __builtin_amdgcn_make_buffer_rsrc((void*)p.g_out, 0, (int)(mrows * (unsigned)p.g_out_ldc * 4u), 0x00020000);
+    const unsigned gm = (unsigned)(m0 + wm * 64 + wn * 32 + fr);
+    const bool gok = gm < mrows;
+    const float gact_lo = p.g_relu == 1 ? 0.f : -__builtin_huge_valf();
+    float gmax = 0.f;
+#pragma unroll
+    for (int j = 0; j < GNB; ++j)
+#pragma unroll
+      for (int g = 0; g < 4; ++g) {
+        const int col = j * 32 + 8 * g + 4 * fg;
+        const f32x4 sc = (f32x4)__builtin_amdgcn_raw_buffer_load_b128(rs_gs, col * 4, 0, 0);
+        const f32x4 bs = (f32x4)__builtin_amdgcn_raw_buffer_load_b128(rs_gb, col * 4, 0, 0);
+        f32x4 v = {gacc[j][4 * g], gacc[j][4 * g + 1], gacc[j][4 * g + 2], gacc[j][4 * g + 3]};
+        v = v * sc;
+        v += bs;
+#pragma unroll
+        for (int e = 0; e < 4; ++e) v[e] = fmaxf(v[e], gact_lo);
+        const float vm = fmaxf(fmaxf(fabsf(v[0]), fabsf(v[1])), fmaxf(fabsf(v[2]), fabsf(v[3])));
+        gmax = fmaxf(gmax, gok ? vm : 0.f);
+        __builtin_amdgcn_raw_buffer_store_b128((u32x4)v, rs_go, (int)(gok ? (gm * (unsigned)p.g_out_ldc + (unsigned)col) * 4u : kOOB), 0, 0);
+        if (g & 1) ODT_FENCE();
+      }
+    publish_amax_wg<512>(p.f_out_amax, vmax, tid, lds);
+    publish_amax_wg<512>(p.g_out_amax, gmax, tid, lds);
+  } else {
+    publish_amax_wg<512>(p.f_out_amax, vmax, tid, lds);
+  }
 }
 
-template <int TN, bool TRACE = false, bool FUSE = false, int WN = 2>
+template <int TN, bool TRACE = false, bool FUSE = false, int WN = 2, int GNB = 0>
 __global__ void __launch_bounds__(512, 2) conv_h2k_kernel(const ConvParams* __restrict__ pp) {
   using G = H2kCfg<TN, FUSE, WN>;
   constexpr int WM = G::WM, KW = 3;
   constexpr int BM = G::BM, BN = G::BN, AKG = G::AKG, APL = G::APL, ABUF = G::ABUF, BKG = G::BKG, BPL = G::BPL;
   constexpr int STAGE_B = G::STAGE_B, BOFF = G::BOFF, NW = G::NW, ZR = G::ZR, RA = G::RA;
   const ConvParams p = *pp;
-  __shared__ __attribute__((aligned(16))) unsigned char lds[G::LDS];
+  static_assert(GNB == 0 || (FUSE && (GNB == 2 || GNB == 4) && G::LDS + 2 * GNB * 4096 <= 160 * 1024), "next conv1");
+  __shared__ __attribute__((aligned(16))) unsigned char lds[G::LDS + 2 * GNB * 4096];
 
   const int tid = threadIdx.x, lane = tid & 63;
   const int wave = __builtin_amdgcn_readfirstlane(tid >> 6);
@@ -513,7 +626,7 @@
   }
 #undef ODT_MF
   stamp(2);
-  if constexpr (FUSE) h2f_tail<TN, TRACE>(p, acc, lds, m0, M, wave, wm, wn, h2_inv);
+  if constexpr (FUSE) h2f_tail<TN, TRACE, GNB>(p, acc, lds, m0, M, wave, wm, wn, h2_inv);
   else split3_epilogue<WM, WN, TN, G::LDS, TRACE>(p, acc, lds, m0, n0, M, HoWo, ks, splitk, tid, wm, wn, fr, fg, h2_inv);
   stamp(5);
 }
@@ -531,4 +644,13 @@
   ODT_CONV_ROW(t, H2K_256x64, CF_H2, 256, 64, 512, CVF_KWR, (conv_h2k_kernel<1, false>));
 }
 
+int launch_conv_h2k_next(const ConvParams& p, const ConvParams* dev, unsigned grid, hipStream_t stream) {
+  const int bn = conv_variant_row(p.variant).bn;
+  if (bn == 64 && p.g_cout == 64) hipLaunchKernelGGL((conv_h2k_kernel<1, false, true, 2, 2>), dim3(grid), dim3(512), 0, stream, dev);
+  else if (bn == 64 && p.g_cout == 128) hipLaunchKernelGGL((conv_h2k_kernel<1, false, true, 2, 4>), dim3(grid), dim3(512), 0, stream, dev);
+  else if (bn == 128 && p.g_cout == 128) hipLaunchKernelGGL((conv_h2k_kernel<2, false, true, 2, 4>), dim3(grid), dim3(512), 0, stream, dev);
+  else ODT_CHECK(false, "conv h2k: no kernel for this tail + next conv1 combination");
+  return 0;
 }
+
+}
diff --git a/object_detection_tracking_amd/csrc/conv_igemm.hip b/object_detection_tracking_amd/csrc/conv_igemm.hip
--- a/object_detection_tracking_amd/csrc/conv_igemm.hip
+++ b/object_detection_tracking_amd/csrc/conv_igemm.hip
@@ -534,7 +534,8 @@
   return 2.0 * (double)p.B * p.Ho * p.Wo * (double)p.Cout *
              (double)(p.kh * p.kw * p.Cin + (p.in2 != nullptr ? p.Cin2 : 0)) +
          (p.head_wt != nullptr ? 2.0 * (double)p.B * p.Ho * p.Wo * (double)p.Cout * 15.0 : 0.0) +
-         (p.f_wt != nullptr ? 2.0 * (double)p.B * p.Ho * p.Wo * (double)p.Cout * (double)p.f_cout : 0.0);
+         (p.f_wt != nullptr ? 2.0 * (double)p.B * p.Ho * p.Wo * (double)p.Cout * (double)p.f_cout : 0.0) +
+         (p.g_wt != nullptr ? 2.0 * (double)p.B * p.Ho * p.Wo * (double)p.f_cout * (double)p.g_cout : 0.0);
 }
 
 int conv_check(const ConvParams& p) {
diff --git a/object_detection_tracking_amd/csrc/conv_split.hip b/object_detection_tracking_amd/csrc/conv_split.hip
--- a/object_detection_tracking_amd/csrc/conv_split.hip
+++ b/object_detection_tracking_amd/csrc/conv_split.hip
@@ -349,6 +349,10 @@
                                       (p.f_res == nullptr || p.f_res_ldc % 4 == 0) && (double)M * p.f_out_ldc * 4.0 < 2147483648.0 &&
                                       (p.f_res == nullptr || (double)M * p.f_res_ldc * 4.0 < 2147483648.0)),
                 "conv h2k: unsupported fused 1x1 tail");
+      ODT_CHECK(p.g_wt == nullptr || (p.f_wt != nullptr && (r.bn == 64 || r.bn == 128) && (p.g_cout == 128 || (p.g_cout == 64 && r.bn == 64)) &&
+                                      p.f_cout >= 64 && p.g_out != nullptr && p.g_chinv != nullptr && p.g_bias != nullptr && p.g_out_ldc % 4 == 0 &&
+                                      p.g_out_ldc >= p.g_cout && p.g_relu <= 1 && p.trace == nullptr && (double)M * p.g_out_ldc * 4.0 < 2147483648.0),
+                "conv h2k: unsupported next conv1 behind the fused tail");
     }
   } else if (r.family == CF_SPLIT3) {
     ODT_CHECK(p.Cin % 16 == 0 && p.kh * p.kw <= 32, "conv split3: unsupported tile / shape");
@@ -373,7 +377,8 @@
     const int ntiles = r.family == CF_F32 ? (p.Cout + r.bn - 1) / r.bn : cout_padded(p.Cout) / r.bn;
     grid = (unsigned)(((M + r.bm - 1) / r.bm) * ntiles * sk);
   }
-  (p.trace != nullptr && r.launch_traced != nullptr ? r.launch_traced : r.launch)(dev, grid, stream);
+  if (p.g_wt != nullptr) { if (launch_conv_h2k_next(p, dev, grid, stream)) return 1; }
+  else (p.trace != nullptr && r.launch_traced != nullptr ? r.launch_traced : r.launch)(dev, grid, stream);
   if (sk > 1) launch_split_reduce(p, dev, stream);
   ODT_HIP(hipGetLastError());
   return 0;
diff --git a/object_detection_tracking_amd/csrc/knobs.hpp b/object_detection_tracking_amd/csrc/knobs.hpp
--- a/object_detection_tracking_amd/csrc/knobs.hpp
+++ b/object_detection_tracking_amd/csrc/knobs.hpp
@@ -10,7 +10,7 @@
   X(CONV_H2_ROT) X(CONV_SPLIT3_FILLDIV) X(CONV_SPLIT3_BM) X(CONV_SPLIT3_SPLITK) X(CONV_SPLIT3_KWR) X(CONV_SPLIT3_KWR_N64)         \
   X(CONV_SPLIT3_FORCE_SPLITK) X(CONV_SPLIT_SRC2) X(CONV_SPLIT_RES2) X(SPLIT_REDUCE_BLOCKS) X(CONV_NT) X(AMAX_PER_WAVE) X(ROI_AMAX)            \
   X(CONV_CHUNK_BYTES) X(CONV_TILE) X(CONV_DEBUG) X(CONV_SMALLK) X(CONV_STAGES) X(CONV_FINE) X(CONV_TRACE)                         \
-  X(FUSE_SHORTCUT) X(FUSE_RPN_HEAD) X(FUSE_BOTTLENECK) X(FUSE_ROT) X(FUSE_STEM) X(STEM_GRID) X(TAIL_OVERLAP)                      \
+  X(FUSE_SHORTCUT) X(FUSE_RPN_HEAD) X(FUSE_BOTTLENECK) X(FUSE_NEXT_CONV1) X(FUSE_ROT) X(FUSE_STEM) X(STEM_GRID) X(TAIL_OVERLAP)                      \
   X(SIDE_STREAM_PRIORITY) X(COSINE_STREAM_PRIORITY) X(TRACKER_TIMING)                                                             \
   X(EFFDET_SPLIT) X(EFFDET_FUSE_MB) X(EFFDET_FUSE_MB_MIN) X(EFFDET_WSCALE) X(EFFDET_MERGE_LEVELS) X(DW_PX) X(DW_SUMCAP) X(DW_XCD)
 
diff --git a/object_detection_tracking_amd/csrc/odt_common.hpp b/object_detection_tracking_amd/csrc/odt_common.hpp
--- a/object_detection_tracking_amd/csrc/odt_common.hpp
+++ b/object_detection_tracking_amd/csrc/odt_common.hpp
@@ -91,8 +91,15 @@
   int f_cout, f_out_ldc, f_res_ldc, f_relu;
   int host_unused1_[5];
   int reduce_blocks;
-};
-static_assert(sizeof(ConvParams) == 432 && offsetof(ConvParams, variant) == 208 && offsetof(ConvParams, splitk) == 224 &&
+  const void* g_wt;
+  const float* g_chinv;
+  const float* g_bias;
+  float* g_out;
+  unsigned* g_out_amax;
+  int g_cout, g_out_ldc, g_relu;
+  int g_pad_;
+};
+static_assert(sizeof(ConvParams) == 488 && offsetof(ConvParams, variant) == 208 && offsetof(ConvParams, splitk) == 224 &&
               offsetof(ConvParams, nlvl) == 240 && offsetof(ConvParams, reduce_blocks) == 428, "ConvParams layout");
 void conv_prepare(ConvParams& p);
 double conv_flops(const ConvParams& p);
@@ -198,6 +205,11 @@
 const float* conv_h2f_chinv(const void* img, int Cout, int K);
 int conv_make_h2f_weights(const float* wt, int Cout, int K, void* img_dev, hipStream_t stream);
 bool conv_h2f_fusable(const ConvParams& a, const ConvParams& b);
+size_t conv_h2g_weight_bytes(int Cout, int K);
+const float* conv_h2g_chinv(const void* img, int Cout, int K);
+int conv_make_h2g_weights(const float* wt, int Cout, int K, void* img_dev, hipStream_t stream);
+bool conv_h2g_fusable(const ConvParams& a, const ConvParams& b);
+int launch_conv_h2k_next(const ConvParams& p, const ConvParams* dev, unsigned grid, hipStream_t stream);
 size_t conv_split_partial_bytes(const ConvParams& p);
 
 int launch_preprocess(const void* frames, int dtype, int B, int H, int W, int pad_t, int pad_l,
diff --git a/object_detection_tracking_amd/csrc/odt_model.hpp b/object_detection_tracking_amd/csrc/odt_model.hpp
--- a/object_detection_tracking_amd/csrc/odt_model.hpp
+++ b/object_detection_tracking_amd/csrc/odt_model.hpp
@@ -103,6 +103,7 @@
   int convs_h2 = 0;
   int stem_fused = 0;
   int convs_h2f = 0;
+  int convs_h2g = 0;
   unsigned* pre_amax = nullptr;
   std::vector<Op> ops;
   int Hp = 0, Wp = 0;
@@ -205,6 +206,7 @@
 int attach_split_weights(odt_model* m);
 int fuse_rpn_heads(odt_model* m);
 int fuse_bottleneck_tails(odt_model* m);
+int fuse_next_conv1(odt_model* m);
 int fuse_stem(odt_model* m);
 void find_overlap_points(odt_model* m);
 int plan_arena(odt_model* m);
@@ -231,7 +233,7 @@
   f(op.in.d); f(op.out.d);
   switch (op.kind) {
     case OP_PRE: case OP_PRE_RGB: f(m->image_pad.d); break;
-    case OP_CONV: { ConvParams& c = m->convs[op.conv].p; f(c.in); f(c.res); f(c.out); f(c.in2); f(c.head_out); f(c.f_res); f(c.f_out); break; }
+    case OP_CONV: { ConvParams& c = m->convs[op.conv].p; f(c.in); f(c.res); f(c.out); f(c.in2); f(c.head_out); f(c.f_res); f(c.f_out); f(c.g_out); break; }
     case OP_PROPOSALS: for (auto& l : m->prop.lvl) f(l.rpn); f(m->prop.props); break;
     case OP_ROI_HEAD: roi(m->roi_head); break;
     case OP_ROI_FINAL: roi(m->roi_final); break;
diff --git a/object_detection_tracking_amd/csrc/op_shims.hip b/object_detection_tracking_amd/csrc/op_shims.hip
--- a/object_detection_tracking_amd/csrc/op_shims.hip
+++ b/object_detection_tracking_amd/csrc/op_shims.hip
@@ -287,9 +287,9 @@
   return dout.get(out, nout);
 }
 
-int odt_op_bottleneck_tail(int device, const float* in, int B, int H, int W, int C, const float* w2_hwio, const float* b2,
-                           int dil, const float* w3_io, const float* b3, int C3, const float* res, int relu3, int fuse,
-                           float* out) {
+static int bottleneck_tail_impl(int device, const float* in, int B, int H, int W, int C, const float* w2_hwio, const float* b2,
+                                int dil, const float* w3_io, const float* b3, int C3, const float* res, int relu3, int fuse,
+                                float* out, const float* w1_io, const float* b1, int N1, float* out1) {
   ODT_CHECK(in && w2_hwio && b2 && w3_io && b3 && out, "odt_op_bottleneck_tail: null argument");
   ODT_CHECK((C == 256 || C == 128 || C == 64) && C3 % 64 == 0 && C3 > 0 && (dil == 1 || dil == 2), "odt_op_bottleneck_tail: C = 64 / 128 / 256, C3 % 64 == 0, dil 1 or 2");
   if (set_dev(device)) return 1;
@@ -335,16 +335,44 @@
     a.f_wt = imgf.d; a.f_chinv = conv_h2f_chinv(imgf.d, C3, C); a.f_bias = db3.d; a.f_res = b.res; a.f_res_ldc = C3;
     a.f_out = dout.d; a.f_out_ldc = C3; a.f_cout = C3; a.f_relu = b.relu; a.f_out_amax = amax.d + 2 * kAmaxWays;
     a.out = nullptr; a.out_amax = nullptr;
+    Tmp<float> dw1, db1, dout1, imgg;
+    if (w1_io != nullptr) {
+      ODT_CHECK(b1 && out1 && (N1 == 64 || N1 == 128), "odt_op_bottleneck_tail_next: bias, output and N1 = 64 / 128 required");
+      std::vector<float> w1((size_t)N1 * C3);
+      for (int i = 0; i < C3; ++i) for (int o = 0; o < N1; ++o) w1[(size_t)o * C3 + i] = w1_io[(size_t)i * N1 + o];
+      if (dw1.alloc(w1.size()) || db1.alloc(N1) || dout1.alloc(M * N1) || dout1.zero() || dw1.put(w1.data()) || db1.put(b1)) return 1;
+      if (imgg.alloc((conv_h2g_weight_bytes(N1, C3) + 3) / 4) || conv_make_h2g_weights(dw1.d, N1, C3, imgg.d, nullptr)) return 1;
+      a.g_wt = imgg.d; a.g_chinv = conv_h2g_chinv(imgg.d, N1, C3); a.g_bias = db1.d; a.g_out = dout1.d; a.g_out_ldc = N1;
+      a.g_cout = N1; a.g_relu = 1; a.g_out_amax = amax.d + 3 * kAmaxWays;
+    }
     ConvParams recs[2] = {a, b};
     if (conv_check(a) || rec.put(recs)) return 1;
     if (launch_conv(a, rec.d, nullptr)) return 1;
+    if (w1_io != nullptr) {
+      ODT_HIP(hipDeviceSynchronize());
+      if (dout1.get(out1, M * N1)) return 1;
+    }
   } else {
+    ODT_CHECK(w1_io == nullptr, "odt_op_bottleneck_tail_next: the next conv1 runs behind the fused tail only");
     ConvParams recs[2] = {a, b};
     if (conv_check(a) || conv_check(b) || rec.put(recs)) return 1;
     if (launch_conv(a, rec.d, nullptr) || launch_conv(b, rec.d + 1, nullptr)) return 1;
   }
   ODT_HIP(hipDeviceSynchronize());
   return dout.get(out, M * C3);
+}
+
+int odt_op_bottleneck_tail(int device, const float* in, int B, int H, int W, int C, const float* w2_hwio, const float* b2,
+                           int dil, const float* w3_io, const float* b3, int C3, const float* res, int relu3, int fuse,
+                           float* out) {
+  return bottleneck_tail_impl(device, in, B, H, W, C, w2_hwio, b2, dil, w3_io, b3, C3, res, relu3, fuse, out, nullptr, nullptr, 0, nullptr);
+}
+
+int odt_op_bottleneck_tail_next(int device, const float* in, int B, int H, int W, int C, const float* w2_hwio, const float* b2,
+                                int dil, const float* w3_io, const float* b3, int C3, const float* res, int relu3,
+                                const float* w1_io, const float* b1, int N1, float* out, float* out1) {
+  ODT_CHECK(w1_io && b1 && out1, "odt_op_bottleneck_tail_next: null argument");
+  return bottleneck_tail_impl(device, in, B, H, W, C, w2_hwio, b2, dil, w3_io, b3, C3, res, relu3, 1, out, w1_io, b1, N1, out1);
 }
 
 int odt_op_stem(int device, const float* frame_pad, int B, int Hp, int Wp, const float* w_hwio, const float* bias, int fuse,
diff --git a/object_detection_tracking_amd/csrc/plan_common.hip b/object_detection_tracking_amd/csrc/plan_common.hip
--- a/object_detection_tracking_amd/csrc/plan_common.hip
+++ b/object_detection_tracking_amd/csrc/plan_common.hip
@@ -419,6 +419,53 @@
   return 0;
 }
 
+int fuse_next_conv1(odt_model* m) {
+  if (m->conv_fused.size() < m->convs.size()) m->conv_fused.resize(m->convs.size(), 0);
+  const KnobVal& kv = m->knobs.get(K_FUSE_NEXT_CONV1);
+  if (kv.set && kv.c0 == '0') return 0;
+  const bool force = kv.set && kv.c0 == 'f';
+  if (m->policy.arith == 0 || m->policy.family != 2 || m->cfg.use_se) return 0;
+  int ncu = 0;
+  if (!force) {
+    int dev_id = 0;
+    hipDeviceProp_t prop;
+    ODT_HIP(hipGetDevice(&dev_id));
+    ODT_HIP(hipGetDeviceProperties(&prop, dev_id));
+    ncu = prop.multiProcessorCount > 0 ? prop.multiProcessorCount : 256;
+  }
+  std::map<const float*, const void*> made;
+  for (size_t oi = 0; oi + 1 < m->ops.size(); ++oi) {
+    Op& oa = m->ops[oi];
+    if (oa.kind != OP_CONV || oa.skip) continue;
+    ConvOp& a = m->convs[oa.conv];
+    if (a.p.f_wt == nullptr) continue;
+    size_t ob_i = oi + 1;
+    while (ob_i < m->ops.size() && m->ops[ob_i].skip) ++ob_i;
+    if (ob_i >= m->ops.size() || m->ops[ob_i].kind != OP_CONV) continue;
+    Op& ob = m->ops[ob_i];
+    ConvOp& b = m->convs[ob.conv];
+    if (!conv_h2g_fusable(a.p, b.p)) continue;
+    const long tiles = ((long)a.p.B * a.p.Ho * a.p.Wo + 255) / 256;
+    if (!force && tiles < ncu) continue;
+    const int K = b.p.Cin;
+    auto it = made.find(b.p.wt);
+    if (it == made.end()) {
+      float* img = m->alloc_f((conv_h2g_weight_bytes(b.p.Cout, K) + 3) / 4, false);
+      ODT_CHECK(img != nullptr, "device allocation failed (next conv1 weights of " + b.name + ")");
+      if (conv_make_h2g_weights(b.p.wt, b.p.Cout, K, img, 0)) return 1;
+      it = made.emplace(b.p.wt, img).first;
+    }
+    ConvParams& ap = a.p;
+    ap.g_wt = it->second; ap.g_chinv = conv_h2g_chinv(it->second, b.p.Cout, K); ap.g_bias = b.p.bias;
+    ap.g_out = b.p.out; ap.g_out_ldc = b.p.out_ldc; ap.g_cout = b.p.Cout; ap.g_relu = b.p.relu; ap.g_out_amax = b.p.out_amax;
+    ob.skip = true;
+    m->conv_fused[ob.conv] = 3;
+    ++m->convs_h2g;
+  }
+  ODT_HIP(hipDeviceSynchronize());
+  return 0;
+}
+
 int fuse_stem(odt_model* m) {
   if (m->knobs.off(K_FUSE_STEM)) return 0;
   if (m->policy.arith == 0 || m->policy.family != 2) return 0;
@@ -528,7 +575,7 @@
     if (op.kind != OP_CONV || op.skip) continue;
     const ConvParams& c = m->convs[op.conv].p;
     for (const void* q : {(const void*)c.in, (const void*)c.res, (const void*)c.out, (const void*)c.in2, (const void*)c.head_out,
-                          (const void*)c.f_res, (const void*)c.f_out})
+                          (const void*)c.f_res, (const void*)c.f_out, (const void*)c.g_out})
       ODT_CHECK(q == nullptr || !m->is_virtual(q), "activation arena: unmapped pointer left in " + m->convs[op.conv].name);
   }
   return 0;
@@ -540,7 +587,8 @@
     return b * p.in_Ha * p.in_Wa * p.in_ldc * 4.0 < limit && b * p.out_H * p.out_W * p.out_ldc * 4.0 < limit &&
            (p.res_mode == 0 || b * p.res_H * p.res_W * p.res_ldc * 4.0 < limit) &&
            (p.in2 == nullptr || b * p.in2_Ha * p.in2_Wa * p.in2_ldc * 4.0 < limit) &&
-           (p.f_wt == nullptr || (b * p.Ho * p.Wo * p.f_out_ldc * 4.0 < limit && (p.f_res == nullptr || b * p.Ho * p.Wo * p.f_res_ldc * 4.0 < limit)));
+           (p.f_wt == nullptr || (b * p.Ho * p.Wo * p.f_out_ldc * 4.0 < limit && (p.f_res == nullptr || b * p.Ho * p.Wo * p.f_res_ldc * 4.0 < limit))) &&
+           (p.g_wt == nullptr || b * p.Ho * p.Wo * p.g_out_ldc * 4.0 < limit);
   };
   for (int n = 1; n <= p.B; ++n)
     if (p.B % n == 0 && fits(n)) return n;
@@ -571,6 +619,7 @@
       if (p.head_out != nullptr) q.head_out = p.head_out + b0 * p.Ho * p.Wo * p.head_ldc;
       if (p.f_out != nullptr) q.f_out = p.f_out + b0 * p.Ho * p.Wo * p.f_out_ldc;
       if (p.f_res != nullptr) q.f_res = p.f_res + b0 * p.Ho * p.Wo * p.f_res_ldc;
+      if (p.g_out != nullptr) q.g_out = p.g_out + b0 * p.Ho * p.Wo * p.g_out_ldc;
       if (launched[ci] && conv_finish(q, m->knobs)) { g_err = c.name + ": " + g_err; return 1; }
       m->conv_recs.push_back(q);
     }
diff --git a/object_detection_tracking_amd/csrc/plan_fpn.hip b/object_detection_tracking_amd/csrc/plan_fpn.hip
--- a/object_detection_tracking_amd/csrc/plan_fpn.hip
+++ b/object_detection_tracking_amd/csrc/plan_fpn.hip
@@ -371,6 +371,7 @@
   if (attach_split_weights(m)) return 1;
   if (fuse_rpn_heads(m)) return 1;
   if (fuse_bottleneck_tails(m)) return 1;
+  if (fuse_next_conv1(m)) return 1;
   if (fuse_stem(m)) return 1;
   if (plan_arena(m)) return 1;
   if (upload_conv_records(m)) return 1;
diff --git a/object_detection_tracking_amd/csrc/runtime.hip b/object_detection_tracking_amd/csrc/runtime.hip
--- a/object_detection_tracking_amd/csrc/runtime.hip
+++ b/object_detection_tracking_amd/csrc/runtime.hip
@@ -651,7 +651,8 @@
   if (name && name_cap > 0) {
     const bool fused = index < (int)h->conv_fused.size() && h->conv_fused[index];
     const ConvKernelRow& row = conv_variant_row(c.p.variant);
-    const std::string nm = c.name + (fused ? "[fused into the producer's epilogue]" : (c.p.head_wt != nullptr ? "+head" : ((row.flags & CVF_FTAIL) ? "+conv3" : ((row.flags & CVF_STEM) ? "+pool0" : "")))) +
+    const int fcode = fused ? h->conv_fused[index] : 0;
+    const std::string nm = c.name + (fused ? (fcode == 3 ? "[fused into the previous block's tail]" : "[fused into the producer's epilogue]") : (c.p.head_wt != nullptr ? "+head" : ((row.flags & CVF_FTAIL) ? (c.p.g_wt != nullptr ? "+conv3+next" : "+conv3") : ((row.flags & CVF_STEM) ? "+pool0" : "")))) +
                            (!fused && c.p.wt_split != nullptr ? (row.family == CF_H2 ? "[fp16x2]" : "[bf16x3]") : "");
     std::strncpy(name, nm.c_str(), name_cap - 1); name[name_cap - 1] = 0;
   }
@@ -663,9 +664,10 @@
 
 int odt_describe(odt_handle h, char* buf, int cap) {
   ODT_CHECK(h != nullptr && buf != nullptr && cap > 0, "odt_describe: null argument");
-  int fam[4] = {0, 0, 0, 0}, nsk = 0, nfused = 0;
+  int fam[4] = {0, 0, 0, 0}, nsk = 0, nfused = 0, nnext = 0;
   for (size_t i = 0; i < h->convs.size(); ++i) {
     const ConvOp& c = h->convs[i];
+    if (i < h->conv_fused.size() && h->conv_fused[i] == 3) { ++nnext; continue; }
     if (i < h->conv_fused.size() && h->conv_fused[i]) { ++nfused; continue; }
     fam[c.p.wt_split != nullptr ? conv_variant_row(c.p.variant).family : CF_F32] += 1;
     if (c.p.wt_split != nullptr && c.p.splitk > 1) ++nsk;
@@ -691,7 +693,7 @@
   char tmp[8192];
   std::snprintf(tmp, sizeof(tmp),
                 "{\"conv_arith\": \"%s\", \"conv_launches\": %d, \"convs_fused_into_epilogues\": %d, \"exact_f32_mfma_launches\": %d, "
-                "\"bf16x3_split_launches\": %d, \"fp16x2_split_launches\": %d, \"bottleneck_tails_fused\": %d, \"stem_fused\": %d, \"mbconv_expand_dw_fused\": %d, \"split_launches_by_family\": {\"split3_8wave_lds_dma\": %d, "
+                "\"bf16x3_split_launches\": %d, \"fp16x2_split_launches\": %d, \"bottleneck_tails_fused\": %d, \"next_conv1_fused\": %d, \"stem_fused\": %d, \"mbconv_expand_dw_fused\": %d, \"split_launches_by_family\": {\"split3_8wave_lds_dma\": %d, "
                 "\"one_stage_bk32\": %d, \"h2_8wave_lds_dma\": %d, \"of_split3_with_split_k\": %d}, \"policy\": {\"family\": %d, \"min_tiles\": %ld, "
                 "\"min_tiles3\": %ld, \"min_k\": %d}, \"env_overrides_applied\": %d, \"env_overrides\": [%s], "
                 "\"memory\": {\"device_bytes\": %zu, \"activation_arena_bytes\": [%zu, %zu], \"arena_tensors\": %zu, "
@@ -699,7 +701,7 @@
                 "\"use_se\": %d, \"se_blocks\": %d, \"se_blocks_conv1_on_fp16x2\": %d}",
                 h->policy.arith != 0 && fam[2] > 0 ? "f32 through fp16x2 / bf16x3 split products"
                     : (h->policy.arith != 0 && fam[1] + fam[3] > 0 ? "f32 through bf16x3 split products" : "exact f32 MFMA"),
-                (int)h->convs.size() - nfused, nfused, fam[0], fam[1] + fam[3], fam[2], h->convs_h2f, h->stem_fused, h->mb_fused, fam[3], fam[1], fam[2], nsk, h->policy.family,
+                (int)h->convs.size() - nfused - nnext, nfused, fam[0], fam[1] + fam[3], fam[2], h->convs_h2f, nnext, h->stem_fused, h->mb_fused, fam[3], fam[1], fam[2], nsk, h->policy.family,
                 h->policy.min_tiles, h->policy.min_tiles3, h->policy.min_k, (int)active.size(), envs.c_str(),
                 dev_bytes, h->arena_bytes[0], h->arena_bytes[1], h->vt.size(), h->virtual_tensor_bytes,
                 h->dedicated_tensor_bytes, h->cfg.keep_taps, h->chunked_convs, h->cfg.use_se != 0 ? 1 : 0, h->se_blocks, se_conv1_h2);
diff --git a/object_detection_tracking_amd/ops.py b/object_detection_tracking_amd/ops.py
--- a/object_detection_tracking_amd/ops.py
+++ b/object_detection_tracking_amd/ops.py
@@ -58,6 +58,21 @@
   lib.check(lib.dll.odt_op_bottleneck_tail(device, fptr(x), B, H, W, Cc, fptr(w2), fptr(b2), dil, fptr(w3), fptr(b3), C3,
                                            fptr(r) if r is not None else None, int(relu3), int(fuse), fptr(out)))
   return out
+
+
+def bottleneck_tail_next(x, w2, b2, w3, b3, w1, b1, res=None, dil=1, relu3=True, lib=None, device=0):
+  lib = _L(lib)
+  x = f32(x); w2 = f32(w2); b2 = f32(b2); w3 = f32(w3); b3 = f32(b3); w1 = f32(w1); b1 = f32(b1)
+  B, H, W, Cc = x.shape
+  C3 = w3.shape[1]
+  N1 = w1.shape[1]
+  r = f32(res) if res is not None else None
+  out = np.zeros((B, H, W, C3), np.float32)
+  out1 = np.zeros((B, H, W, N1), np.float32)
+  lib.check(lib.dll.odt_op_bottleneck_tail_next(device, fptr(x), B, H, W, Cc, fptr(w2), fptr(b2), dil, fptr(w3), fptr(b3), C3,
+                                                fptr(r) if r is not None else None, int(relu3), fptr(w1), fptr(b1), N1,
+                                                fptr(out), fptr(out1)))
+  return out, out1
 
 
 def stem(frame_pad, w_hwio, bias, fuse=True, grid=0, lib=None, device=0):
```

New measurement: 314.5 (median of 6 runs). About the same (+0.7%).
